# ndming/GS-2M

Hardware: AMD Instinct MI355X
Metric: train views/s (fwd+bwd raster) at 1M Gaussians 1080p (higher is better)
Workload: dtype f32; 1 GPU; BASELINE configs[2] (c3): 1000000 synthetic Gaussians (SH deg 3), 1 camera 1920x1080 per GPU, feature_count=9, fwd+bwd at the op boundary; gaussians=1000000, visible=844909, num_rendered=2709460, width=1920, height=1080, feature_count=9, parallelism=view-parallel x1, views_per_rank=1

## Files before the change

### gs-2m_amd/csrc/api.hip

```cpp
#include "common.h"
#include <atomic>
#include <mutex>
#include <chrono>
#include <dlfcn.h>

#define HIP_TRY(expr)                          \
    do {                                       \
        hipError_t e_ = (expr);                \
        if (e_ != hipSuccess) return GS2M_ERR_HIP; \
    } while (0)

namespace {

uint32_t higher_msb(uint32_t n) {
    uint32_t msb = sizeof(n) * 4;
    uint32_t step = msb;
    while (step > 1) {
        step /= 2;
        if (n >> msb) msb += step; else msb -= step;
    }
    if (n >> msb) msb++;
    return msb;
}

constexpr int kLandSlots = 64, kLandWords = 16;
struct LandRing {
    uint32_t* host = nullptr;
    uint32_t* dev = nullptr;
    std::atomic<uint32_t> next{0};
    std::atomic<uint32_t> gen[kLandSlots];
};
LandRing g_land[64];
std::mutex g_land_mutex;
thread_local uint64_t t_last_token = 0;
thread_local long long t_rows_hint = -1;
thread_local long long t_units_hint = -1, t_units_from_token = -1;

static_assert(GS2M_NUM_STAGES == 10, "stage table");
enum Stage { ST_PREPROCESS = 0, ST_UNUSED1, ST_SCAN, ST_EMIT, ST_TILE_SORT, ST_LISTS, ST_BLEND_FWD, ST_UNUSED7,
             ST_BLEND_BWD, ST_GAUSSIAN_BWD, ST_COUNT };
constexpr int kMaxRecords = 8192;
struct Prof {
    std::atomic<int> mode{0};
    int n = 0;
    hipEvent_t ev[kMaxRecords][2];
    int stage[kMaxRecords];
    int created = 0;
    int every = 1;
    int seen3 = 0;
};
Prof g_prof;
std::mutex g_prof_mutex;
std::atomic<int> g_reference_binning{0};
std::atomic<int> g_spin_wait{1};
std::atomic<int> g_debug{0};
std::atomic<int> g_markers{0};

const char* const kStageNames[ST_COUNT] = {"preprocess", "-", "scan", "emit", "tile_sort", "depth_order+quad_lists", "blend_fwd", "-", "blend_bwd", "gaussian_bwd"};

struct Roctx {
    int (*push)(const char*) = nullptr;
    int (*pop)() = nullptr;
    bool tried = false;
    void load() {
        if (tried) return;
        tried = true;
        void* h = dlopen("libroctx64.so", RTLD_NOW | RTLD_GLOBAL);
        if (!h) h = dlopen("libroctx64.so.4", RTLD_NOW | RTLD_GLOBAL);
        if (!h) return;
        push = (int (*)(const char*))dlsym(h, "roctxRangePushA");
        pop = (int (*)())dlsym(h, "roctxRangePop");
    }
};
Roctx g_roctx;

struct StageTimer {
    hipStream_t s;
    int slot = -1;
    int stage;
    int* failed;
    bool marked = false;
    StageTimer(int stage_, hipStream_t s_, int* failed_ = nullptr) : s(s_), stage(stage_), failed(failed_) {
        if (g_markers.load(std::memory_order_relaxed)) {
            g_roctx.load();
            if (g_roctx.push) { g_roctx.push(kStageNames[stage]); marked = true; }
        }
        const bool blend = stage == ST_BLEND_FWD || stage == ST_BLEND_BWD;
        if (g_prof.mode.load(std::memory_order_relaxed) == 0) return;
        {
            std::lock_guard<std::mutex> lock(g_prof_mutex);
            if (g_prof.mode == 0 || (g_prof.mode == 1 && !blend) || (g_prof.mode == 3 && stage != ST_BLEND_BWD) || g_prof.n >= kMaxRecords) return;
            if (g_prof.mode == 3 && (g_prof.seen3++ % g_prof.every) != 0) return;
            slot = g_prof.n++;
            if (slot >= g_prof.created) {
                (void)hipEventCreate(&g_prof.ev[slot][0]);
                (void)hipEventCreate(&g_prof.ev[slot][1]);
                g_prof.created = slot + 1;
            }
            g_prof.stage[slot] = stage;
        }
        (void)hipEventRecord(g_prof.ev[slot][0], s);
    }
    ~StageTimer() {
        if (slot >= 0) (void)hipEventRecord(g_prof.ev[slot][1], s);
        if (failed && g_debug.load(std::memory_order_relaxed) && *failed == 0) {
            hipError_t e = hipGetLastError();
            if (e == hipSuccess) e = hipStreamSynchronize(s);
            if (e != hipSuccess) *failed = stage + 1;
        }
        if (marked && g_roctx.pop) g_roctx.pop();
    }
};
#define DEBUG_CHECK()                                        \
    do {                                                     \
        if (failed_stage) return GS2M_ERR_STAGE(failed_stage - 1); \
    } while (0)

}

extern "C" {

char* gs2m_prealloc_alloc(size_t bytes, void* user) {
    gs2m_prealloc* p = static_cast<gs2m_prealloc*>(user);
    if (!p) return nullptr;
    p->requested = bytes;
    if (p->ptr && bytes <= p->capacity) return p->ptr;
    p->used_fallback = 1;
    return p->fallback ? p->fallback(bytes, p->fallback_user) : nullptr;
}

const char* gs2m_version(void) { return "gs2m_raster 0.5 (gfx950, round 5)"; }

static int forward_impl(gs2m_alloc_fn geometry_alloc, void* geometry_user, gs2m_alloc_fn binning_alloc,
                        void* binning_user, gs2m_alloc_fn image_alloc, void* image_user, int P, int D, int M,
                        const float* background, int width, int height, const float* means3D, const float* shs, const float* shs_rest,
                        const float* colors_precomp, const float* opacities, const float* scales, float scale_modifier,
                        const float* rotations, const float* cov3D_precomp, const float* features,
                        const float* viewmatrix, const float* projmatrix, const float* cam_pos, float tan_fovx,
                        float tan_fovy, int prefiltered, int feature_count, float* out_color, int* out_radii,
                        int* out_observe, float* out_buffer, void* stream_) {
    hipStream_t s = (hipStream_t)stream_;
    const int reference_binning = g_reference_binning.load(), spin_wait = g_spin_wait.load();
    int failed_stage = 0;
    if (P < 0 || width <= 0 || height <= 0 || feature_count < 0 || feature_count > GS2M_NUM_FEATURES) return GS2M_ERR_INVALID_ARG;
    if (!geometry_alloc || !binning_alloc || !image_alloc || !out_color || !out_buffer || !background) return GS2M_ERR_INVALID_ARG;
    if (P > 0 && (!means3D || !opacities || !out_radii || !out_observe || !viewmatrix || !projmatrix)) return GS2M_ERR_INVALID_ARG;
    if (P > 0 && ((shs == nullptr) == (colors_precomp == nullptr))) return GS2M_ERR_INVALID_ARG;
    if (P > 0 && (((scales == nullptr) || (rotations == nullptr)) == (cov3D_precomp == nullptr))) return GS2M_ERR_INVALID_ARG;
    if (P > 0 && shs && (D < 0 || D > 3 || M < (D + 1) * (D + 1) || !cam_pos)) return GS2M_ERR_INVALID_ARG;
    if (shs_rest && (!shs || M != 16 || (((uintptr_t)shs_rest) & 15))) return GS2M_ERR_UNSUPPORTED;
    if (P > 0 && feature_count > 0 && !features) return GS2M_ERR_INVALID_ARG;
    if (width > 16 * 65535 || height > 16 * 65535) return GS2M_ERR_UNSUPPORTED;
    if ((size_t)((width + GS2M_TILE - 1) / GS2M_TILE) * (size_t)((height + GS2M_TILE - 1) / GS2M_TILE) > ((size_t)1 << 28)) return GS2M_ERR_UNSUPPORTED;
    if (P >= (1 << GS2M_GID_BITS)) return GS2M_ERR_UNSUPPORTED;

    const int tiles_x = (width + GS2M_TILE - 1) / GS2M_TILE, tiles_y = (height + GS2M_TILE - 1) / GS2M_TILE;
    const size_t tiles = (size_t)tiles_x * tiles_y, N = (size_t)width * height;
    const float focal_y = height / (2.0f * tan_fovy);
    const float focal_x = width / (2.0f * tan_fovx);

    const size_t Pn = P > 0 ? (size_t)P : 1;
    GeomState gsz = gs2m_carve_geom(nullptr, Pn);
    char* gbase = geometry_alloc(gsz.total_bytes, geometry_user);
    if (!gbase) return GS2M_ERR_ALLOC;
    GeomState g = gs2m_carve_geom(gbase, Pn);

    ImageState isz = gs2m_carve_image(nullptr, N, tiles);
    char* ibase = image_alloc(isz.total_bytes, image_user);
    if (!ibase) return GS2M_ERR_ALLOC;
    ImageState im = gs2m_carve_image(ibase, N, tiles);

    int dev_id = 0;
    HIP_TRY(hipGetDevice(&dev_id));
    if (dev_id < 0 || dev_id >= 64) return GS2M_ERR_UNSUPPORTED;
    LandRing& ring = g_land[dev_id];
    if (!ring.host) {
        std::lock_guard<std::mutex> lock(g_land_mutex);
        if (!ring.host) {
            uint32_t* h = nullptr;
            HIP_TRY(hipHostMalloc((void**)&h, kLandSlots * kLandWords * sizeof(uint32_t), hipHostMallocMapped | hipHostMallocPortable));
            HIP_TRY(hipHostGetDevicePointer((void**)&ring.dev, h, 0));
            for (int k = 0; k < kLandSlots; k++) ring.gen[k] = 0;
            ring.host = h;
        }
    }
    const uint32_t seq = ring.next.fetch_add(1), slot = seq % kLandSlots;
    const uint32_t generation = ring.gen[slot].fetch_add(1) + 1;
    volatile uint32_t* land = ring.host + slot * kLandWords;
    uint32_t* land_dev = ring.dev + slot * kLandWords;
    land[GS2M_LAND_R] = 0xFFFFFFFFu;
    land[GS2M_LAND_HUNITS] = 0xFFFFFFFFu;
    land[GS2M_LAND_PREFILTERED] = 0u;
    land[GS2M_LAND_ROWS] = 0u;
    t_last_token = ((uint64_t)(dev_id + 1) << 40) | ((uint64_t)(generation & 0xFFFFFFFFu) << 8) | slot;

    int R = 0;
    uint32_t U = 0, crowded = GS2M_CROWDED_WAVE;
    if (P > 0) {
        {
            StageTimer t(ST_PREPROCESS, s, &failed_stage);
            ZeroJobs zj = {{g.tile_hist, nullptr, nullptr}, {(size_t)GS2M_HIST_COPIES * GS2M_HIST_COPY_WORDS, 0, 0}};
            gs2m_launch_preprocess(P, D, M, means3D, scales, scale_modifier, rotations, opacities, shs, shs_rest, cov3D_precomp,
                                   colors_precomp, features, viewmatrix, projmatrix, cam_pos, width, height, tan_fovx,
                                   tan_fovy, focal_x, focal_y, tiles_x, tiles_y, out_radii, out_observe, g,
                                   reference_binning ? 0 : 1, zj, s);
        }
        if (prefiltered) gs2m_launch_prefiltered_check(P, means3D, viewmatrix, land_dev + GS2M_LAND_PREFILTERED, s);
        {
            StageTimer t(ST_SCAN, s, &failed_stage);
            gs2m_launch_blockscan(P, g, land_dev, s);
        }
        HIP_TRY(hipGetLastError());
        DEBUG_CHECK();
        if (spin_wait) {
            const auto t0 = std::chrono::steady_clock::now();
            uint32_t spins = 0;
            while (land[GS2M_LAND_R] == 0xFFFFFFFFu || land[GS2M_LAND_HUNITS] == 0xFFFFFFFFu) {
                __builtin_ia32_pause();
                if ((++spins & 0xFFFFu) == 0u && std::chrono::steady_clock::now() - t0 > std::chrono::seconds(2)) break;
            }
        }
        if (land[GS2M_LAND_R] == 0xFFFFFFFFu || land[GS2M_LAND_HUNITS] == 0xFFFFFFFFu) HIP_TRY(hipStreamSynchronize(s));
        if (prefiltered && land[GS2M_LAND_PREFILTERED] != 0u) {
            HIP_TRY(hipStreamSynchronize(s));
            return GS2M_ERR_PREFILTERED;
        }
        if (land[GS2M_LAND_R] >= (1u << 29)) return GS2M_ERR_UNSUPPORTED;
        R = (int)land[GS2M_LAND_R];
        U = land[GS2M_LAND_HUNITS];
        if ((size_t)U * 4 * GS2M_UNIT > (size_t)6 * (size_t)R + 65536) {
            crowded = GS2M_CROWDED_OFF;
            land[GS2M_LAND_R] = 0xFFFFFFFFu;
            land[GS2M_LAND_HUNITS] = 0xFFFFFFFFu;
            gs2m_launch_recount_heavy(P, g, s);
            gs2m_launch_blockscan(P, g, land_dev, s);
            HIP_TRY(hipGetLastError());
            HIP_TRY(hipStreamSynchronize(s));
            if (land[GS2M_LAND_R] != (uint32_t)R) return GS2M_ERR_STAGE(ST_SCAN);
            U = land[GS2M_LAND_HUNITS];
        }
        if (U >= (1u << 22)) return GS2M_ERR_UNSUPPORTED;
    }

    const int tile_bits = (int)higher_msb((uint32_t)tiles);
    const size_t Rn = R > 0 ? (size_t)R : 1;
    const size_t btemp = gs2m_binning_temp_bytes(Rn, tile_bits);
    BinningState bsz = gs2m_carve_binning(nullptr, Rn, btemp, U);
    char* bbase = binning_alloc(bsz.total_bytes, binning_user);
    if (!bbase) return GS2M_ERR_ALLOC;
    BinningState b = gs2m_carve_binning(bbase, Rn, btemp, U);

    if (R > 0) {
        {
            StageTimer t(ST_EMIT, s, &failed_stage);
            ZeroJobs zj = {{nullptr, im.ranges_raw, nullptr}, {0, tiles * 2, 0}};
            gs2m_radix_zero_region(b.temp, (size_t)R, tile_bits, &zj.p[0], &zj.words[0]);
            gs2m_launch_emit(P, width, height, tiles_x, tile_bits, g, b, U, crowded, land_dev, zj, s);
        }
        if (g_debug.load(std::memory_order_relaxed)) {
            uint32_t total = 0;
            HIP_TRY(hipStreamSynchronize(s));
            HIP_TRY(hipMemcpy(&total, g.counters, sizeof(total), hipMemcpyDeviceToHost));
            if (total != (uint32_t)R) return GS2M_ERR_STAGE(ST_EMIT);
        }
        {
            StageTimer t(ST_TILE_SORT, s, &failed_stage);
            HIP_TRY(gs2m_radix_sort_pairs(b.temp, b.temp_bytes, b.keys_unsorted, nullptr, b.sort_keyA, b.sort_valA, b.tile_keys, b.slot_sorted,
                                          (size_t)R, tile_bits, true, s, im.ranges_raw, g.tile_hist));
        }
    } else {
        HIP_TRY(gs2m_zero_async(im.ranges_raw, tiles * 2 * sizeof(uint32_t), s));
        land[GS2M_LAND_ROWS] = 1u;
        if (land[GS2M_LAND_HUNITS] == 0xFFFFFFFFu) land[GS2M_LAND_HUNITS] = 0u;
    }
    DEBUG_CHECK();
    {
        StageTimer t(ST_LISTS, s, &failed_stage);
        gs2m_launch_tile_sort(tiles, tiles_x, tiles_y, (size_t)(R > 0 ? R : 0), b, im, g, s);
    }
    {
        StageTimer t(ST_BLEND_FWD, s, &failed_stage);
        gs2m_launch_blend_fwd_q(width, height, tiles_x, tiles_y, feature_count, background, g, b, im, out_color, out_buffer, out_observe, s);
    }
    DEBUG_CHECK();
    HIP_TRY(hipGetLastError());
    return R;
}

static int backward_impl(int P, int D, int M, int R, const float* background, int width, int height,
                         const float* means3D, const float* shs, const float* shs_rest, const float* colors_precomp, const float* scales,
                         float scale_modifier, const float* rotations, const float* cov3D_precomp,
                         const float* features, const float* viewmatrix, const float* projmatrix, const float* campos,
                         float tan_fovx, float tan_fovy, const int* radii, const float* buffer, char* geom_buffer,
                         char* binning_buffer, char* image_buffer, int feature_count, const float* grad_colors,
                         const float* grad_buffer, float* dL_dmeans2D, float* dL_dconics, float* dL_dopacities,
                         float* dL_dcolors, float* dL_dmeans3D, float* dL_dcov3D, float* dL_dshs, float* dL_dshs_rest, float* dL_dscales,
                         float* dL_drots, float* dL_dfeatures, gs2m_alloc_fn scratch_alloc, void* scratch_user,
                         void* stream_) {
    (void)buffer; (void)features;
    hipStream_t s = (hipStream_t)stream_;
    int failed_stage = 0;
    if (P == 0) return GS2M_OK;
    if (P >= (1 << GS2M_GID_BITS)) return GS2M_ERR_UNSUPPORTED;
    if (P < 0 || R < 0 || width <= 0 || height <= 0 || feature_count < 0 || feature_count > GS2M_NUM_FEATURES) return GS2M_ERR_INVALID_ARG;
    if (!geom_buffer || !binning_buffer || !image_buffer || !scratch_alloc || !grad_colors || !radii) return GS2M_ERR_INVALID_ARG;
    if (feature_count > 0 && !grad_buffer) return GS2M_ERR_INVALID_ARG;
    if (!dL_dmeans2D || !dL_dopacities || !dL_dmeans3D || !dL_dscales || !dL_drots || !dL_dfeatures) return GS2M_ERR_INVALID_ARG;
    if ((colors_precomp && !dL_dcolors) || (cov3D_precomp && !dL_dcov3D)) return GS2M_ERR_INVALID_ARG;
    if (shs_rest && (M != 16 || ((dL_dshs == nullptr) != (dL_dshs_rest == nullptr)) || ((((uintptr_t)shs_rest) | ((uintptr_t)dL_dshs_rest)) & 15))) return GS2M_ERR_UNSUPPORTED;

    const int tiles_x = (width + GS2M_TILE - 1) / GS2M_TILE, tiles_y = (height + GS2M_TILE - 1) / GS2M_TILE;
    const size_t tiles = (size_t)tiles_x * tiles_y, N = (size_t)width * height;
    const size_t Rn = R > 0 ? (size_t)R : 1;
    GeomState g = gs2m_carve_geom(geom_buffer, (size_t)P);
    BinningState b = gs2m_carve_binning(binning_buffer, Rn, gs2m_binning_temp_bytes(Rn, (int)higher_msb((uint32_t)tiles)), 0);
    ImageState im = gs2m_carve_image(image_buffer, N, tiles);

    const int rowf = gs2m_row_floats(feature_count);
    const long long hint = t_rows_hint;
    long long units = hint >= 0 ? t_units_hint : -1;
    t_rows_hint = -1;
    t_units_hint = -1;
    size_t nrows = 0;
    if (hint >= 0 && (size_t)hint <= Rn * 10 + 256) {
        nrows = (size_t)hint;
    } else if (R > 0) {
        uint32_t c[2] = {0u, 0u};
        HIP_TRY(hipStreamSynchronize(s));
        HIP_TRY(hipMemcpy(c, g.counters + GS2M_CNT_ROWS, sizeof(c), hipMemcpyDeviceToHost));
        nrows = c[0];
        units = c[1];
    }
    const size_t rows_bytes = gs2m_align_up((nrows > 0 ? nrows : 1) * (size_t)rowf * sizeof(float));
    char* sbase = scratch_alloc(rows_bytes + 2 * GS2M_ALIGN, scratch_user);
    if (!sbase) return GS2M_ERR_ALLOC;
    float* rows = (float*)gs2m_align_up((size_t)(uintptr_t)sbase);

    if (R > 0) {
        StageTimer t(ST_BLEND_BWD, s, &failed_stage);
        gs2m_launch_blend_bwd_q(width, height, tiles_x, tiles_y, feature_count, background, g, b, im, grad_colors,
                                grad_buffer, rows, s);
    }
    DEBUG_CHECK();
    {
        StageTimer tg(ST_GAUSSIAN_BWD, s, &failed_stage);
        if (R > 0) gs2m_launch_heavy_reduce(rows, rowf, b, g, units, s);
        gs2m_launch_gaussian_bwd(P, D, M, means3D, shs, shs_rest, colors_precomp, scales, scale_modifier, rotations, cov3D_precomp,
                                 viewmatrix, projmatrix, campos, width, height, tan_fovx, tan_fovy, radii, feature_count, g,
                                 rows, rowf, R > 0, dL_dmeans2D, dL_dconics, dL_dopacities, dL_dcolors, dL_dmeans3D,
                                 dL_dcov3D, dL_dshs, dL_dshs_rest, dL_dscales, dL_drots, dL_dfeatures, s);
    }
    DEBUG_CHECK();
    HIP_TRY(hipGetLastError());
    return GS2M_OK;
}

int gs2m_raster_forward(gs2m_alloc_fn geometry_alloc, void* geometry_user, gs2m_alloc_fn binning_alloc,
                        void* binning_user, gs2m_alloc_fn image_alloc, void* image_user, int P, int D, int M,
                        const float* background, int width, int height, const float* means3D, const float* shs,
                        const float* colors_precomp, const float* opacities, const float* scales, float scale_modifier,
                        const float* rotations, const float* cov3D_precomp, const float* features,
                        const float* viewmatrix, const float* projmatrix, const float* cam_pos, float tan_fovx,
                        float tan_fovy, int prefiltered, int feature_count, float* out_color, int* out_radii,
                        int* out_observe, float* out_buffer, void* stream_) {
    return forward_impl(geometry_alloc, geometry_user, binning_alloc, binning_user, image_alloc, image_user, P, D, M, background, width, height, means3D, shs, nullptr, colors_precomp, opacities, scales, scale_modifier, rotations, cov3D_precomp, features, viewmatrix, projmatrix, cam_pos, tan_fovx, tan_fovy, prefiltered, feature_count, out_color, out_radii, out_observe, out_buffer, stream_);
}

int gs2m_raster_forward_split_sh(gs2m_alloc_fn geometry_alloc, void* geometry_user, gs2m_alloc_fn binning_alloc,
                        void* binning_user, gs2m_alloc_fn image_alloc, void* image_user, int P, int D, int M,
                        const float* background, int width, int height, const float* means3D, const float* sh_dc, const float* sh_rest,
                        const float* colors_precomp, const float* opacities, const float* scales, float scale_modifier,
                        const float* rotations, const float* cov3D_precomp, const float* features,
                        const float* viewmatrix, const float* projmatrix, const float* cam_pos, float tan_fovx,
                        float tan_fovy, int prefiltered, int feature_count, float* out_color, int* out_radii,
                        int* out_observe, float* out_buffer, void* stream_) {
    if (!sh_dc || !sh_rest) return GS2M_ERR_INVALID_ARG;
    return forward_impl(geometry_alloc, geometry_user, binning_alloc, binning_user, image_alloc, image_user, P, D, M, background, width, height, means3D, sh_dc, sh_rest, colors_precomp, opacities, scales, scale_modifier, rotations, cov3D_precomp, features, viewmatrix, projmatrix, cam_pos, tan_fovx, tan_fovy, prefiltered, feature_count, out_color, out_radii, out_observe, out_buffer, stream_);
}

int gs2m_raster_backward(int P, int D, int M, int R, const float* background, int width, int height,
                         const float* means3D, const float* shs, const float* colors_precomp, const float* scales,
                         float scale_modifier, const float* rotations, const float* cov3D_precomp,
                         const float* features, const float* viewmatrix, const float* projmatrix, const float* campos,
                         float tan_fovx, float tan_fovy, const int* radii, const float* buffer, char* geom_buffer,
                         char* binning_buffer, char* image_buffer, int feature_count, const float* grad_colors,
                         const float* grad_buffer, float* dL_dmeans2D, float* dL_dconics, float* dL_dopacities,
                         float* dL_dcolors, float* dL_dmeans3D, float* dL_dcov3D, float* dL_dshs, float* dL_dscales,
                         float* dL_drots, float* dL_dfeatures, gs2m_alloc_fn scratch_alloc, void* scratch_user,
                         void* stream_) {
    return backward_impl(P, D, M, R, background, width, height, means3D, shs, nullptr, colors_precomp, scales, scale_modifier, rotations, cov3D_precomp, features, viewmatrix, projmatrix, campos, tan_fovx, tan_fovy, radii, buffer, geom_buffer, binning_buffer, image_buffer, feature_count, grad_colors, grad_buffer, dL_dmeans2D, dL_dconics, dL_dopacities, dL_dcolors, dL_dmeans3D, dL_dcov3D, dL_dshs, nullptr, dL_dscales, dL_drots, dL_dfeatures, scratch_alloc, scratch_user, stream_);
}

int gs2m_raster_backward_split_sh(int P, int D, int M, int R, const float* background, int width, int height,
                         const float* means3D, const float* sh_dc, const float* sh_rest, const float* colors_precomp, const float* scales,
                         float scale_modifier, const float* rotations, const float* cov3D_precomp,
                         const float* features, const float* viewmatrix, const float* projmatrix, const float* campos,
                         float tan_fovx, float tan_fovy, const int* radii, const float* buffer, char* geom_buffer,
                         char* binning_buffer, char* image_buffer, int feature_count, const float* grad_colors,
                         const float* grad_buffer, float* dL_dmeans2D, float* dL_dconics, float* dL_dopacities,
                         float* dL_dcolors, float* dL_dmeans3D, float* dL_dcov3D, float* dL_dsh_dc, float* dL_dsh_rest, float* dL_dscales,
                         float* dL_drots, float* dL_dfeatures, gs2m_alloc_fn scratch_alloc, void* scratch_user,
                         void* stream_) {
    if (!sh_dc || !sh_rest) return GS2M_ERR_INVALID_ARG;
    return backward_impl(P, D, M, R, background, width, height, means3D, sh_dc, sh_rest, colors_precomp, scales, scale_modifier, rotations, cov3D_precomp, features, viewmatrix, projmatrix, campos, tan_fovx, tan_fovy, radii, buffer, geom_buffer, binning_buffer, image_buffer, feature_count, grad_colors, grad_buffer, dL_dmeans2D, dL_dconics, dL_dopacities, dL_dcolors, dL_dmeans3D, dL_dcov3D, dL_dsh_dc, dL_dsh_rest, dL_dscales, dL_drots, dL_dfeatures, scratch_alloc, scratch_user, stream_);
}

int gs2m_raster_mark_visible(int P, const float* means3D, const float* viewmatrix, const float* projmatrix,
                             uint8_t* present, void* stream_) {
    (void)projmatrix;
    if (P < 0) return GS2M_ERR_INVALID_ARG;
    if (P == 0) return GS2M_OK;
    if (!means3D || !viewmatrix || !present) return GS2M_ERR_INVALID_ARG;
    gs2m_launch_mark_visible(P, means3D, viewmatrix, present, (hipStream_t)stream_);
    HIP_TRY(hipGetLastError());
    return GS2M_OK;
}

int gs2m_set_reference_binning(int on) {
    g_reference_binning = on ? 1 : 0;
    return GS2M_OK;
}

int gs2m_set_tile_sort_policy(int policy) {
    if (policy < 0 || policy > 3) return GS2M_ERR_INVALID_ARG;
    gs2m_set_tile_sort_policy_impl(policy);
    return GS2M_OK;
}

int gs2m_set_debug(int on) {
    g_debug = on ? 1 : 0;
    return GS2M_OK;
}

int gs2m_set_markers(int on) {
    g_markers = on ? 1 : 0;
    if (on) {
        g_roctx.load();
        if (!g_roctx.push || !g_roctx.pop) return GS2M_ERR_UNSUPPORTED;
    }
    return GS2M_OK;
}

const char* gs2m_stage_name(int stage) { return stage >= 0 && stage < ST_COUNT ? kStageNames[stage] : "?"; }

int gs2m_set_spin_wait(int on) {
    g_spin_wait = on ? 1 : 0;
    return GS2M_OK;
}

int gs2m_profile_mode(int mode) {
    if (mode < 0 || mode > 3) return GS2M_ERR_INVALID_ARG;
    std::lock_guard<std::mutex> lock(g_prof_mutex);
    g_prof.mode = mode;
    g_prof.n = 0;
    g_prof.seen3 = 0;
    return GS2M_OK;
}

int gs2m_profile_sampling(int every) {
    if (every < 1) return GS2M_ERR_INVALID_ARG;
    std::lock_guard<std::mutex> lock(g_prof_mutex);
    g_prof.every = every;
    return GS2M_OK;
}

int gs2m_profile_collect(float* stage_ms, int* stage_count, int n_stages) {
    if (!stage_ms || !stage_count || n_stages < GS2M_NUM_STAGES) return GS2M_ERR_INVALID_ARG;
    std::lock_guard<std::mutex> lock(g_prof_mutex);
    for (int i = 0; i < n_stages; i++) { stage_ms[i] = 0.f; stage_count[i] = 0; }
    for (int r = 0; r < g_prof.n; r++) {
        float ms = 0.f;
        HIP_TRY(hipEventSynchronize(g_prof.ev[r][1]));
        HIP_TRY(hipEventElapsedTime(&ms, g_prof.ev[r][0], g_prof.ev[r][1]));
        stage_ms[g_prof.stage[r]] += ms;
        stage_count[g_prof.stage[r]] += 1;
    }
    g_prof.n = 0;
    return GS2M_OK;
}

int gs2m_debug_layout(int P, int R, int width, int height, gs2m_layout* out) {
    if (!out || P < 0 || R < 0 || width <= 0 || height <= 0) return GS2M_ERR_INVALID_ARG;
    const int tiles_x = (width + GS2M_TILE - 1) / GS2M_TILE, tiles_y = (height + GS2M_TILE - 1) / GS2M_TILE;
    const size_t tiles = (size_t)tiles_x * tiles_y, N = (size_t)width * height;
    const size_t Pn = P > 0 ? (size_t)P : 1, Rn = R > 0 ? (size_t)R : 1;
    GeomState g = gs2m_carve_geom(nullptr, Pn);
    BinningState b = gs2m_carve_binning(nullptr, Rn, gs2m_binning_temp_bytes(Rn, (int)higher_msb((uint32_t)tiles)), 0);
    ImageState im = gs2m_carve_image(nullptr, N, tiles);
    out->geom_bytes = g.total_bytes;
    out->rec = (uint64_t)(uintptr_t)g.rec;
    out->tiles_touched = (uint64_t)(uintptr_t)g.tiles_touched;
    out->depth_key = (uint64_t)(uintptr_t)g.depth_key;
    out->rect = (uint64_t)(uintptr_t)g.rect;
    out->gauss_rows = (uint64_t)(uintptr_t)g.gauss_rows;
    out->clamped = (uint64_t)(uintptr_t)g.clamped;
    out->wave_rowbase = (uint64_t)(uintptr_t)g.wave_rowbase;
    out->counters = (uint64_t)(uintptr_t)g.counters;
    out->binning_bytes = b.total_bytes;
    out->point_list = (uint64_t)(uintptr_t)b.point_list;
    out->tile_keys = (uint64_t)(uintptr_t)b.tile_keys;
    out->qlist = (uint64_t)(uintptr_t)b.qlist;
    out->qrow = (uint64_t)(uintptr_t)b.qrow;
    out->image_bytes = im.total_bytes;
    out->final_T = (uint64_t)(uintptr_t)im.final_T;
    out->n_contrib = (uint64_t)(uintptr_t)im.n_contrib;
    out->ranges = (uint64_t)(uintptr_t)im.ranges;
    out->qcount = (uint64_t)(uintptr_t)im.qcount;
    return GS2M_OK;
}

unsigned long long gs2m_raster_forward_token(void) { return (unsigned long long)t_last_token; }

long long gs2m_raster_dense_rows(unsigned long long token) {
    if (token == 0ull) return -1;
    const int dev = (int)(token >> 40) - 1;
    const uint32_t slot = (uint32_t)(token & 0xFFull), generation = (uint32_t)((token >> 8) & 0xFFFFFFFFull);
    if (dev < 0 || dev >= 64 || slot >= (uint32_t)kLandSlots || !g_land[dev].host) return -1;
    LandRing& ring = g_land[dev];
    volatile uint32_t* land = ring.host + slot * kLandWords;
    const auto t0 = std::chrono::steady_clock::now();
    uint32_t spins = 0;
    for (;;) {
        if (ring.gen[slot].load() != generation) return -1;
        const uint32_t v = land[GS2M_LAND_ROWS];
        if (v != 0u) {
            t_units_from_token = (long long)land[GS2M_LAND_HUNITS];
            return ring.gen[slot].load() == generation ? (long long)v - 1 : -1;
        }
        __builtin_ia32_pause();
        if ((++spins & 0xFFFFu) == 0u && std::chrono::steady_clock::now() - t0 > std::chrono::seconds(2)) return -1;
    }
}

int gs2m_raster_backward_rows_hint(long long dense_rows) {
    t_rows_hint = dense_rows;
    t_units_hint = dense_rows >= 0 ? t_units_from_token : -1;
    t_units_from_token = -1;
    return GS2M_OK;
}

int gs2m_debug_tile_sort(int tiles, const unsigned* ranges_raw, unsigned* ranges, const unsigned* slot_sorted, const unsigned* e_rec,
                         const unsigned* wave_rowbase, unsigned* point_list, unsigned* row_tmp, unsigned* qlist,
                         unsigned* qrow, unsigned* qcount, void* stream_) {
    if (tiles < 0 || !ranges_raw || !ranges || !slot_sorted || !e_rec || !wave_rowbase || !point_list || !row_tmp || !qlist || !qrow || !qcount) return GS2M_ERR_INVALID_ARG;
    BinningState b = {};
    b.slot_sorted = const_cast<uint32_t*>(slot_sorted); b.e_rec = reinterpret_cast<uint4*>(const_cast<unsigned*>(e_rec));
    b.point_list = point_list; b.sort_valA = row_tmp; b.qlist = reinterpret_cast<uint2*>(qlist); b.qrow = qrow;
    ImageState im = {};
    im.ranges_raw = const_cast<uint32_t*>(ranges_raw);
    im.ranges = reinterpret_cast<uint2*>(ranges);
    im.qcount = qcount;
    GeomState g = {};
    g.wave_rowbase = const_cast<uint32_t*>(wave_rowbase);
    static uint32_t* dbg_counters[64] = {nullptr};
    int dev = 0;
    HIP_TRY(hipGetDevice(&dev));
    if (dev < 0 || dev >= 64) return GS2M_ERR_UNSUPPORTED;
    if (dbg_counters[dev] == nullptr) HIP_TRY(hipMalloc(&dbg_counters[dev], 64 * sizeof(uint32_t)));
    HIP_TRY(hipMemsetAsync(dbg_counters[dev], 0, 64 * sizeof(uint32_t), (hipStream_t)stream_));
    g.counters = dbg_counters[dev];
    gs2m_launch_tile_sort((size_t)tiles, tiles, 1, SIZE_MAX, b, im, g, (hipStream_t)stream_);
    HIP_TRY(hipGetLastError());
    return GS2M_OK;
}

}
```

### gs-2m_amd/csrc/binning.hip

```cpp
#include "common.h"

GeomState gs2m_carve_geom(char* base, size_t P) {
    GeomState g;
    size_t off = base ? (gs2m_align_up((size_t)(uintptr_t)base) - (size_t)(uintptr_t)base) : 0;
    auto take = [&](size_t bytes) {
        char* p = (char*)((uintptr_t)base + off);
        off = gs2m_align_up(off + bytes);
        return p;
    };
    const size_t nb = (P + 255) / 256 + 1, nw = (P + 63) / 64 + 1;
    g.rec = (float4*)take(P * REC_Q * sizeof(float4));
    g.tiles_touched = (uint32_t*)take(P * 4);
    g.rect = (uint2*)take(P * sizeof(uint2));
    g.depth_key = (uint32_t*)take(P * 4);
    g.clamped = (uint8_t*)take(P);
    g.sh_dir = (float*)take(P * 9 * sizeof(float));
    g.counters = (uint32_t*)take(64 * 4);
    g.gauss_rows = (uint32_t*)take(P * 4);
    g.block_tt = (uint32_t*)take(nb * 4);
    g.block_pref = (uint32_t*)take(nb * 4);
    g.block_hu = (uint32_t*)take(nb * 4);
    g.block_hupref = (uint32_t*)take(nb * 4);
    g.wave_rows = (uint32_t*)take(nw * 4);
    g.wave_rowbase = (uint32_t*)take(nw * 4);
    g.tile_hist = (uint32_t*)take(GS2M_HIST_COPIES * GS2M_HIST_COPY_WORDS * 4);
    g.total_bytes = off + GS2M_ALIGN;
    return g;
}

BinningState gs2m_carve_binning(char* base, size_t R, size_t temp_bytes, size_t heavy_units) {
    BinningState b;
    size_t off = base ? (gs2m_align_up((size_t)(uintptr_t)base) - (size_t)(uintptr_t)base) : 0;
    auto take = [&](size_t bytes) {
        char* p = (char*)((uintptr_t)base + off);
        off = gs2m_align_up(off + bytes);
        return p;
    };
    b.keys_unsorted = (uint32_t*)take(R * 4);
    b.e_rec = (uint4*)take(R * sizeof(uint4));
    b.sort_keyA = (uint32_t*)take(R * 4);
    b.sort_valA = (uint32_t*)take(R * 4);
    b.tile_keys = (uint32_t*)take(R * 4);
    b.slot_sorted = (uint32_t*)take(R * 4);
    b.point_list = (uint32_t*)take(R * 4);
    b.qlist = (uint2*)take(R * 4 * sizeof(uint2));
    b.qrow = (uint32_t*)take(R * 4 * 4);
    b.temp = take(temp_bytes);
    b.temp_bytes = temp_bytes;
    b.hrec = (HeavyUnit*)take(heavy_units * sizeof(HeavyUnit));
    b.total_bytes = off + GS2M_ALIGN;
    return b;
}

size_t gs2m_binning_temp_bytes(size_t R, int tile_bits) { return gs2m_align_up(gs2m_radix_temp_bytes(R, tile_bits)) + GS2M_ALIGN; }

ImageState gs2m_carve_image(char* base, size_t N, size_t tiles) {
    ImageState im;
    size_t off = base ? (gs2m_align_up((size_t)(uintptr_t)base) - (size_t)(uintptr_t)base) : 0;
    auto take = [&](size_t bytes) {
        char* p = (char*)((uintptr_t)base + off);
        off = gs2m_align_up(off + bytes);
        return p;
    };
    im.final_T = (float*)take(N * 4);
    im.n_contrib = (uint32_t*)take(N * 4);
    im.ranges = (uint2*)take(tiles * sizeof(uint2));
    im.ranges_raw = (uint32_t*)take(tiles * 2 * sizeof(uint32_t));
    im.qcount = (uint32_t*)take(tiles * 4 * sizeof(uint32_t));
    im.qlast = (uint32_t*)take(tiles * 4 * sizeof(uint32_t));
    im.total_bytes = off + GS2M_ALIGN;
    return im;
}

namespace {

__device__ __forceinline__ void publish(uint32_t* landing, int word, uint32_t v) {
    __hip_atomic_store(landing + word, v, __ATOMIC_RELAXED, __HIP_MEMORY_SCOPE_SYSTEM);
}

__device__ __forceinline__ unsigned long long block_sum_u64(unsigned long long v, unsigned long long* s_part ) {
    const int lane = threadIdx.x & 63, wave = threadIdx.x >> 6, nw = blockDim.x >> 6;
#pragma unroll
    for (int d = 32; d > 0; d >>= 1) v += __shfl_xor(v, d, 64);
    gs2m_sync();
    if (lane == 0) s_part[wave] = v;
    gs2m_sync();
    unsigned long long t = 0;
    for (int w = 0; w < nw; w++) t += s_part[w];
    return t;
}

template <typename F>
__device__ __forceinline__ unsigned long long scan_1024_per_block(const uint32_t* __restrict__ in, size_t n, uint32_t* s_w ,
                                                                  unsigned long long* s_part , F emit) {
    const size_t first = (size_t)blockIdx.x * 1024;
    unsigned long long before = 0;
    for (size_t base = 0; base < first; base += 16 * 1024) {
        uint32_t v[16];
#pragma unroll
        for (int k = 0; k < 16; k++) {
            const size_t i = base + (size_t)k * 1024 + threadIdx.x;
            v[k] = i < first ? in[i] : 0u;
        }
#pragma unroll
        for (int k = 0; k < 16; k++) before += v[k];
    }
    const size_t i = first + threadIdx.x;
    const uint32_t mine = i < n ? in[i] : 0u;
    before = block_sum_u64(before, s_part);
    const int lane = threadIdx.x & 63, wave = threadIdx.x >> 6;
    const uint32_t incl = wave_inclusive_scan_u32(mine, lane);
    if (lane == 63) s_w[wave] = incl;
    gs2m_sync();
    uint32_t run = incl - mine, total = 0;
    for (int w = 0; w < 16; w++) {
        if (w < wave) run += s_w[w];
        total += s_w[w];
    }
    if (i < n) emit(i, (uint32_t)before + run, mine);
    return before + total;
}

template <typename F>
__device__ __forceinline__ void scan2_1024_per_block(const uint32_t* __restrict__ in0, const uint32_t* __restrict__ in1, size_t n, uint32_t* s_w ,
                                                     unsigned long long* s_part , F emit, unsigned long long& total0, unsigned long long& total1) {
    const size_t first = (size_t)blockIdx.x * 1024;
    unsigned long long b0 = 0, b1 = 0;
    for (size_t base = 0; base < first; base += 8 * 1024) {
        uint32_t v[8], w[8];
#pragma unroll
        for (int k = 0; k < 8; k++) {
            const size_t i = base + (size_t)k * 1024 + threadIdx.x;
            v[k] = i < first ? in0[i] : 0u;
            w[k] = i < first ? in1[i] : 0u;
        }
#pragma unroll
        for (int k = 0; k < 8; k++) { b0 += v[k]; b1 += w[k]; }
    }
    const size_t i = first + threadIdx.x;
    const uint32_t m0 = i < n ? in0[i] : 0u, m1 = i < n ? in1[i] : 0u;
    const int lane = threadIdx.x & 63, wave = threadIdx.x >> 6;
#pragma unroll
    for (int d = 32; d > 0; d >>= 1) { b0 += __shfl_xor(b0, d, 64); b1 += __shfl_xor(b1, d, 64); }
    const uint32_t i0 = wave_inclusive_scan_u32(m0, lane), i1 = wave_inclusive_scan_u32(m1, lane);
    if (lane == 0) { s_part[wave] = b0; s_part[16 + wave] = b1; }
    if (lane == 63) { s_w[wave] = i0; s_w[16 + wave] = i1; }
    gs2m_sync();
    unsigned long long f0 = 0, f1 = 0;
    uint32_t r0 = i0 - m0, r1 = i1 - m1, t0 = 0, t1 = 0;
    for (int w = 0; w < 16; w++) {
        f0 += s_part[w]; f1 += s_part[16 + w];
        if (w < wave) { r0 += s_w[w]; r1 += s_w[16 + w]; }
        t0 += s_w[w]; t1 += s_w[16 + w];
    }
    if (i < n) emit(i, (uint32_t)f0 + r0, (uint32_t)f1 + r1);
    total0 = f0 + t0;
    total1 = f1 + t1;
}

__global__ void __launch_bounds__(1024) blockscan_kernel(const uint32_t* __restrict__ block_tt, const uint32_t* __restrict__ block_hu, size_t nblocks,
                                                         uint32_t* __restrict__ block_pref, uint32_t* __restrict__ block_hupref,
                                                         uint32_t* __restrict__ counters, uint32_t* landing) {
    __shared__ uint32_t s_w[32];
    __shared__ unsigned long long s_part[32];
    unsigned long long t = 0, u = 0;
    scan2_1024_per_block(block_tt, block_hu, nblocks, s_w, s_part, [&](size_t b, uint32_t e0, uint32_t e1) { block_pref[b] = e0; block_hupref[b] = e1; }, t, u);
    if (blockIdx.x == gridDim.x - 1 && threadIdx.x == 0) {
        const uint32_t r32 = t > 0xFFFFFFFEull ? 0xFFFFFFFEu : (uint32_t)t, u32 = u > 0xFFFFFFFEull ? 0xFFFFFFFEu : (uint32_t)u;
        __hip_atomic_store(reinterpret_cast<unsigned long long*>(landing + GS2M_LAND_R), (unsigned long long)r32 | ((unsigned long long)u32 << 32),
                           __ATOMIC_RELAXED, __HIP_MEMORY_SCOPE_SYSTEM);
        counters[1] = r32;
        counters[GS2M_CNT_HUNITS] = u32;
        counters[GS2M_CNT_SPAN_MID] = 0u;
        counters[GS2M_CNT_SPAN_LONG] = 0u;
    }
}

__global__ void __launch_bounds__(1024) rowscan_kernel(const uint32_t* __restrict__ wave_rows, size_t nwaves, uint32_t* __restrict__ wave_rowbase,
                                                       uint32_t* __restrict__ counters, uint32_t* landing) {
    __shared__ uint32_t s_w[16];
    __shared__ unsigned long long s_part[16];
    const uint32_t heavy_rows = 4u * GS2M_UNIT * counters[GS2M_CNT_HUNITS];
    const unsigned long long total = heavy_rows + scan_1024_per_block(wave_rows, nwaves, s_w, s_part, [&](size_t w, uint32_t excl, uint32_t) { wave_rowbase[w] = heavy_rows + excl; });
    if (blockIdx.x == gridDim.x - 1 && threadIdx.x == 0) {
        counters[GS2M_CNT_ROWS] = (uint32_t)total;
        publish(landing, GS2M_LAND_ROWS, (uint32_t)total + 1u);
    }
}


__device__ __forceinline__ uint2 expand_instance(uint32_t rmin, uint32_t rwid, uint32_t t, const float4 a , const float2 ct ,
                                                 int W, int H, int tiles_x) {
    const uint32_t ry = t / rwid, rx = t - ry * rwid;
    const uint32_t tx = (rmin & 0xFFFFu) + rx, ty = (rmin >> 16) + ry;
    const int px0 = (int)tx * GS2M_TILE, py0 = (int)ty * GS2M_TILE;
    uint32_t mask = gs2m_reaches_quads(a.x, a.y, a.z, a.w, ct.x, ct.y, (float)px0, (float)py0);
    if (px0 + 8 >= W) mask &= 0x5u;
    if (py0 + 8 >= H) mask &= 0x3u;
    return make_uint2(ty * (uint32_t)tiles_x + tx, mask);
}

__global__ void __launch_bounds__(256) emit_kernel(int P, int W, int H, int tiles_x, const uint2* __restrict__ rect,
                                                   const uint32_t* __restrict__ block_pref, const uint32_t* __restrict__ block_hupref,
                                                   const float4* __restrict__ rec,
                                                   const uint32_t* __restrict__ depth_key, uint32_t* __restrict__ keys_out, uint4* __restrict__ e_rec,
                                                   HeavyUnit* __restrict__ hrec,
                                                   uint32_t* __restrict__ gauss_rows, uint32_t* __restrict__ wave_rows,
                                                   uint32_t* __restrict__ counters, uint32_t* __restrict__ tile_hist, int npass, int4 hbits,
                                                   int4 hshift, uint32_t crowded, ZeroJobs zero) {
    __shared__ uint32_t s_th[4][256];
    __shared__ uint32_t s_pref[4][GS2M_WAVE];
    __shared__ uint32_t s_rmin[4][GS2M_WAVE];
    __shared__ uint32_t s_rw[4][GS2M_WAVE];
    __shared__ uint32_t s_off[4][GS2M_WAVE];
    __shared__ uint32_t s_depth[4][GS2M_WAVE];
    __shared__ float4 s_geo[4][GS2M_WAVE];
    __shared__ float2 s_ct[4][GS2M_WAVE];
    __shared__ uint32_t s_rc[4][GS2M_WAVE];
    __shared__ uint32_t s_wtot[4], s_whu[4];
    const int i = blockIdx.x * 256 + threadIdx.x;
    const int wave = threadIdx.x >> 6, lane = threadIdx.x & 63;
    gs2m_zero_jobs(zero, (size_t)i, (size_t)gridDim.x * 256);
#pragma unroll
    for (int p = 0; p < 4; p++) s_th[p][threadIdx.x] = 0u;
    const int hb[4] = {hbits.x, hbits.y, hbits.z, hbits.w}, hs[4] = {hshift.x, hshift.y, hshift.z, hshift.w};
    uint32_t cnt = 0, rmin = 0, rw = 1;
    if (i < P) {
        const uint2 r = rect[i];
        rmin = r.x;
        rw = r.y & 0xFFFFu;
        cnt = rw * (r.y >> 16);
        if (rw == 0u) rw = 1u;
    }
    const bool heavy = gs2m_heavy(cnt, crowded);
    const uint32_t hu = heavy ? (cnt + GS2M_UNIT - 1u) / GS2M_UNIT : 0u;
    const uint32_t incl_all = wave_inclusive_scan_u32(cnt, lane), incl_hu = wave_inclusive_scan_u32(hu, lane);
    if (lane == 63) { s_wtot[wave] = incl_all; s_whu[wave] = incl_hu; }
    const uint32_t lcnt = heavy ? 0u : cnt;
    if (lcnt > 0) {
        const float4* r = rec + (size_t)i * REC_Q;
        s_geo[wave][lane] = r[REC_GEO0];
        s_ct[wave][lane] = make_float2(r[REC_GEO1].x, r[REC_BIN].w);
        s_depth[wave][lane] = depth_key[i];
    }
    const uint32_t incl = wave_inclusive_scan_u32(lcnt, lane);
    const uint32_t total = __shfl(incl, 63, 64);
    s_pref[wave][lane] = incl - lcnt;
    s_rmin[wave][lane] = rmin;
    s_rw[wave][lane] = rw;
    s_rc[wave][lane] = 0u;
    gs2m_sync();
    uint32_t off = block_pref[blockIdx.x], ustart = block_hupref[blockIdx.x];
#pragma unroll
    for (int w = 0; w < 4; w++)
        if (w < wave) { off += s_wtot[w]; ustart += s_whu[w]; }
    off += incl_all - cnt;
    ustart += incl_hu - hu;
    s_off[wave][lane] = off;
    if (blockIdx.x == gridDim.x - 1 && threadIdx.x == 255) counters[0] = off + cnt;
    if (heavy) {
        gauss_rows[i] = GS2M_ROWS_BIG | ustart;
        for (uint32_t j = 0; j < hu; j++) {
            hrec[ustart + j].gid = (uint32_t)i;
            hrec[ustart + j].off = off;
        }
    }
    const uint32_t gid0 = (uint32_t)blockIdx.x * 256u;
    uint32_t rows_run = 0;
    for (uint32_t k = 0; k < total; k += GS2M_WAVE) {
        const uint32_t j = k + lane;
        uint32_t pc = 0, slot = 0, mask = 0;
        int lo = 0;
        if (j < total) {
#pragma unroll
            for (int step = 32; step > 0; step >>= 1)
                if (s_pref[wave][lo + step] <= j) lo += step;
            const uint32_t t = j - s_pref[wave][lo];
            slot = s_off[wave][lo] + t;
            const uint2 km = expand_instance(s_rmin[wave][lo], s_rw[wave][lo], t, s_geo[wave][lo], s_ct[wave][lo], W, H, tiles_x);
            mask = km.y;
            keys_out[slot] = km.x;
            for (int p = 0; p < npass; p++) atomicAdd(&s_th[p][(km.x >> hs[p]) & ((1u << hb[p]) - 1u)], 1u);
            pc = (uint32_t)__popc(mask);
            if (pc) atomicAdd(&s_rc[wave][lo], pc);
        }
        const uint32_t pin = wave_inclusive_scan_u32(pc, lane);
        if (j < total) e_rec[slot] = make_uint4((gid0 + (uint32_t)(wave * GS2M_WAVE + lo)) | (mask << GS2M_GID_BITS), rows_run + pin - pc, s_depth[wave][lo], 0u);
        rows_run += __shfl(pin, 63, 64);
    }
    if (i < P && !heavy) gauss_rows[i] = s_rc[wave][lane];
    const size_t wave_id = (size_t)blockIdx.x * 4 + wave;
    if (lane == 0 && (size_t)wave_id * GS2M_WAVE < (size_t)P) wave_rows[wave_id] = rows_run;
    gs2m_sync();
    uint32_t* dst = tile_hist + (blockIdx.x & (GS2M_HIST_COPIES - 1)) * GS2M_HIST_COPY_WORDS;
    for (int p = 0; p < npass; p++) {
        const uint32_t c = s_th[p][threadIdx.x];
        if (c) atomicAdd(&dst[p * 256 + threadIdx.x], c);
    }
}

__global__ void __launch_bounds__(256) recount_heavy_kernel(int P, const uint2* __restrict__ rect, uint32_t* __restrict__ block_hu) {
    __shared__ uint32_t s_hu[4];
    const int i = blockIdx.x * 256 + threadIdx.x;
    uint32_t cnt = 0;
    if (i < P) {
        const uint2 r = rect[i];
        cnt = (r.y & 0xFFFFu) * (r.y >> 16);
    }
    uint32_t hu = gs2m_heavy(cnt, GS2M_CROWDED_OFF) ? (cnt + GS2M_UNIT - 1u) / GS2M_UNIT : 0u;
#pragma unroll
    for (int d = 32; d > 0; d >>= 1) hu += (uint32_t)__shfl_xor((int)hu, d, 64);
    if ((threadIdx.x & 63) == 0) s_hu[threadIdx.x >> 6] = hu;
    gs2m_sync();
    if (threadIdx.x == 0) block_hu[blockIdx.x] = s_hu[0] + s_hu[1] + s_hu[2] + s_hu[3];
}

__global__ void __launch_bounds__(256) emit_heavy_kernel(uint32_t units, int W, int H, int tiles_x, const uint2* __restrict__ rect, const float4* __restrict__ rec,
                                                         const uint32_t* __restrict__ depth_key, const uint32_t* __restrict__ gauss_rows,
                                                         uint32_t* __restrict__ keys_out, uint4* __restrict__ e_rec, HeavyUnit* __restrict__ hrec,
                                                         uint32_t* __restrict__ tile_hist, int npass, int4 hbits, int4 hshift) {
    __shared__ uint32_t s_th[4][256];
#pragma unroll
    for (int p = 0; p < 4; p++) s_th[p][threadIdx.x] = 0u;
    gs2m_sync();
    const int hb[4] = {hbits.x, hbits.y, hbits.z, hbits.w}, hs[4] = {hshift.x, hshift.y, hshift.z, hshift.w};
    const int wave = threadIdx.x >> 6, lane = threadIdx.x & 63;
    const uint32_t u = blockIdx.x * 4u + (uint32_t)wave;
    if (u < units) {
        const uint32_t gid = hrec[u].gid, off = hrec[u].off;
        const uint32_t ustart = gauss_rows[gid] & ~GS2M_ROWS_BIG;
        const uint2 r = rect[gid];
        const uint32_t rw = r.y & 0xFFFFu, cnt = rw * (r.y >> 16);
        const float4* rq = rec + (size_t)gid * REC_Q;
        const float4 geo = rq[REC_GEO0];
        const float2 ct = make_float2(rq[REC_GEO1].x, rq[REC_BIN].w);
        const uint32_t dk = depth_key[gid];
        const uint32_t t = (u - ustart) * GS2M_UNIT + (uint32_t)lane;
        uint32_t pc = 0;
        if (t < cnt) {
            const uint2 km = expand_instance(r.x, rw, t, geo, ct, W, H, tiles_x);
            keys_out[off + t] = km.x;
            for (int p = 0; p < npass; p++) atomicAdd(&s_th[p][(km.x >> hs[p]) & ((1u << hb[p]) - 1u)], 1u);
            e_rec[off + t] = make_uint4(gid | (km.y << GS2M_GID_BITS), GS2M_ROWS_BIG | (4u * (u * GS2M_UNIT + (uint32_t)lane)), dk, 0u);
            pc = (uint32_t)__popc(km.y);
        }
        hrec[u].pop[lane] = (uint8_t)pc;
    }
    gs2m_sync();
    uint32_t* dst = tile_hist + (blockIdx.x & (GS2M_HIST_COPIES - 1)) * GS2M_HIST_COPY_WORDS;
    for (int p = 0; p < npass; p++) {
        const uint32_t c = s_th[p][threadIdx.x];
        if (c) atomicAdd(&dst[p * 256 + threadIdx.x], c);
    }
}

}

void gs2m_launch_blockscan(int P, const GeomState& g, uint32_t* landing, hipStream_t s) {
    const size_t nb = (size_t)(P + 255) / 256;
    blockscan_kernel<<<(unsigned)((nb + 1023) / 1024 > 0 ? (nb + 1023) / 1024 : 1), 1024, 0, s>>>(g.block_tt, g.block_hu, nb, g.block_pref, g.block_hupref, g.counters,
                                                                                                  landing);
}

void gs2m_launch_recount_heavy(int P, const GeomState& g, hipStream_t s) {
    recount_heavy_kernel<<<(P + 255) / 256, 256, 0, s>>>(P, g.rect, g.block_hu);
}

void gs2m_launch_emit(int P, int W, int H, int tiles_x, int tile_bits, const GeomState& g, const BinningState& b, uint32_t heavy_units, uint32_t crowded,
                      uint32_t* landing, const ZeroJobs& zero, hipStream_t s) {
    int npass = 0, bits[4], shift[4];
    gs2m_radix_plan(tile_bits, &npass, bits, shift);
    const int4 hbits = make_int4(bits[0], bits[1], bits[2], bits[3]), hshift = make_int4(shift[0], shift[1], shift[2], shift[3]);
    emit_kernel<<<(P + 255) / 256, 256, 0, s>>>(P, W, H, tiles_x, g.rect, g.block_pref, g.block_hupref, g.rec, g.depth_key, b.keys_unsorted, b.e_rec, b.hrec,
                                                g.gauss_rows, g.wave_rows, g.counters, g.tile_hist, npass, hbits, hshift, crowded, zero);
    if (heavy_units > 0u)
        emit_heavy_kernel<<<(heavy_units + 3u) / 4u, 256, 0, s>>>(heavy_units, W, H, tiles_x, g.rect, g.rec, g.depth_key, g.gauss_rows, b.keys_unsorted, b.e_rec,
                                                                  b.hrec, g.tile_hist, npass, hbits, hshift);
    const size_t nw = (size_t)(P + 63) / 64;
    rowscan_kernel<<<(unsigned)((nw + 1023) / 1024 > 0 ? (nw + 1023) / 1024 : 1), 1024, 0, s>>>(g.wave_rows, nw, g.wave_rowbase, g.counters, landing);
}

__global__ void zero_kernel(uint32_t* __restrict__ p, size_t words) {
    const size_t i = (size_t)blockIdx.x * blockDim.x + threadIdx.x;
    const size_t head = (4 - (((uintptr_t)p >> 2) & 3)) & 3;
    const size_t quads = words > head ? (words - head) >> 2 : 0;
    if (i < quads) reinterpret_cast<uint4*>(p + head)[i] = make_uint4(0u, 0u, 0u, 0u);
    if (i < head && i < words) p[i] = 0u;
    const size_t tail = head + 4 * quads;
    if (i < words - min(words, tail)) p[tail + i] = 0u;
}
hipError_t gs2m_zero_async(void* p, size_t bytes, hipStream_t s) {
    if (bytes == 0) return hipSuccess;
    if ((bytes & 3) || ((uintptr_t)p & 3)) return hipMemsetAsync(p, 0, bytes, s);
    const size_t words = bytes >> 2, threads = (words >> 2) + 4;
    zero_kernel<<<(unsigned)((threads + 255) / 256), 256, 0, s>>>((uint32_t*)p, words);
    return hipGetLastError();
}
```

### gs-2m_amd/csrc/common.h

```cpp
#pragma once
#include <hip/hip_runtime.h>
#include <stdint.h>
#include <stddef.h>
#include "../../include/gs2m_raster.h"

typedef float gs2m_v4f __attribute__((ext_vector_type(4)));
template <typename T> __device__ __forceinline__ T gs2m_ldnt(const T* p) { return __builtin_nontemporal_load(p); }
__device__ __forceinline__ float4 gs2m_ldnt(const float4* p) {
    const gs2m_v4f t = __builtin_nontemporal_load(reinterpret_cast<const gs2m_v4f*>(p));
    return make_float4(t.x, t.y, t.z, t.w);
}
template <typename T> __device__ __forceinline__ void gs2m_stnt(T* p, T v) { __builtin_nontemporal_store(v, p); }
__device__ __forceinline__ void gs2m_stnt(float4* p, float4 v) {
    const gs2m_v4f t = {v.x, v.y, v.z, v.w};
    __builtin_nontemporal_store(t, reinterpret_cast<gs2m_v4f*>(p));
}

#define GS2M_ALIGN 256
#define GS2M_WAVE 64

#define REC_Q 8
#define REC_GEO0 0
#define REC_GEO1 1
#define REC_BIN 2
#define REC_CH 3
#define REC_AUX 7
#define GS2M_GID_BITS 28
#define GS2M_GID_MASK 0x0FFFFFFFu
#define GS2M_HEAVY_TILES 40u
#define GS2M_HEAVY_TILES_CROWDED 8u
#define GS2M_CROWDED_WAVE 320u
#define GS2M_ROWS_BIG 0x80000000u
#define GS2M_UNIT 64u
struct HeavyUnit {
    uint32_t gid;
    uint32_t off;
    uint32_t pad[2];
    uint8_t pop[GS2M_UNIT];
};

#define ROW_GEOM 8
#define ROW_COL 8
#define ROW_FEAT 11

static inline size_t gs2m_align_up(size_t x, size_t a = GS2M_ALIGN) { return (x + a - 1) & ~(a - 1); }
static inline int gs2m_status(hipError_t e) { return e == hipSuccess ? GS2M_OK : GS2M_ERR_HIP; }

struct GeomState {
    float4* rec;
    uint32_t* tiles_touched;
    uint2* rect;
    uint32_t* depth_key;
    uint8_t* clamped;
    float* sh_dir;
    uint32_t* counters;
    uint32_t* gauss_rows;
    uint32_t* block_tt;
    uint32_t* block_pref;
    uint32_t* block_hu;
    uint32_t* block_hupref;
    uint32_t* wave_rows;
    uint32_t* wave_rowbase;
    uint32_t* tile_hist;
    size_t total_bytes;
};
struct BinningState {
    uint32_t* keys_unsorted;
    uint4* e_rec;
    uint32_t* sort_keyA;
    uint32_t* sort_valA;
    uint32_t* tile_keys;
    uint32_t* slot_sorted;
    uint32_t* point_list;
    uint2* qlist;
    uint32_t* qrow;
    char* temp;
    size_t temp_bytes;
    HeavyUnit* hrec;
    size_t total_bytes;
};
struct ImageState {
    float* final_T;
    uint32_t* n_contrib;
    uint2* ranges;
    uint32_t* ranges_raw;
    uint32_t* qcount;
    uint32_t* qlast;
    size_t total_bytes;
};

struct ZeroJobs {
    uint32_t* p[3];
    size_t words[3];
};
#ifdef __HIPCC__
__device__ __forceinline__ void gs2m_zero_jobs(const ZeroJobs& z, size_t thread, size_t threads) {
#pragma unroll
    for (int k = 0; k < 3; k++)
        for (size_t i = thread; i < z.words[k]; i += threads) z.p[k][i] = 0u;
}
#endif

#ifdef __HIPCC__
__device__ __forceinline__ void gs2m_stage_sh(const float* __restrict__ shs, const float* __restrict__ rest, int P,
                                              float* __restrict__ s_sh) {
    const int tid = threadIdx.x;
    if (rest == nullptr) {
        const size_t base4 = (size_t)blockIdx.x * 256 * 12, lim4 = (size_t)P * 12;
        const float4* g4 = reinterpret_cast<const float4*>(shs);
        float4 t[12];
#pragma unroll
        for (int i = 0; i < 12; i++) {
            const size_t k = base4 + tid + 256 * i;
            t[i] = k < lim4 ? gs2m_ldnt(g4 + k) : make_float4(0.f, 0.f, 0.f, 0.f);
        }
#pragma unroll
        for (int i = 0; i < 12; i++) {
            const int e = 4 * (tid + 256 * i);
            const int row = e / 48, col = e - row * 48;
            float* d = s_sh + row * 49 + col;
            d[0] = t[i].x; d[1] = t[i].y; d[2] = t[i].z; d[3] = t[i].w;
        }
    } else {
        const size_t dbase = (size_t)blockIdx.x * 768, dlim = (size_t)P * 3;
#pragma unroll
        for (int i = 0; i < 3; i++) {
            const int e = tid + 256 * i;
            const float v = dbase + e < dlim ? shs[dbase + e] : 0.f;
            s_sh[(e / 3) * 49 + (e % 3)] = v;
        }
        const size_t rbase = (size_t)blockIdx.x * 11520, rlim = (size_t)P * 45;
        const bool full = rbase + 11520 <= rlim;
        float4 t[12];
        if (full) {
            const float4* g4 = reinterpret_cast<const float4*>(rest + rbase);
#pragma unroll
            for (int i = 0; i < 11; i++) t[i] = gs2m_ldnt(g4 + tid + 256 * i);
            t[11] = tid < 64 ? gs2m_ldnt(g4 + tid + 2816) : make_float4(0.f, 0.f, 0.f, 0.f);
        } else {
#pragma unroll
            for (int i = 0; i < 12; i++) {
                const int k4 = tid + 256 * i;
                const size_t ge = rbase + 4 * (size_t)k4;
                t[i] = make_float4(0.f, 0.f, 0.f, 0.f);
                if (k4 < 2880) {
                    if (ge + 3 < rlim) {
                        t[i] = *reinterpret_cast<const float4*>(rest + ge);
                    } else {
                        if (ge < rlim) t[i].x = rest[ge];
                        if (ge + 1 < rlim) t[i].y = rest[ge + 1];
                        if (ge + 2 < rlim) t[i].z = rest[ge + 2];
                    }
                }
            }
        }
        int row = (4 * tid) / 45, col = 4 * tid - 45 * row;
#pragma unroll
        for (int i = 0; i < 12; i++) {
            if (i < 11 || tid < 64) {
                const float v[4] = {t[i].x, t[i].y, t[i].z, t[i].w};
                int a = row * 49 + 3 + col, left = 45 - col;
#pragma unroll
                for (int c = 0; c < 4; c++) s_sh[a + c + (c >= left ? 4 : 0)] = v[c];
            }
            row += 22; col += 34;
            if (col >= 45) { col -= 45; row += 1; }
        }
    }
}
#endif

GeomState gs2m_carve_geom(char* base, size_t P);
BinningState gs2m_carve_binning(char* base, size_t R, size_t temp_bytes, size_t heavy_units);
size_t gs2m_binning_temp_bytes(size_t R, int tile_bits);
ImageState gs2m_carve_image(char* base, size_t N, size_t tiles);

size_t gs2m_radix_temp_bytes(size_t n, int total_bits);
hipError_t gs2m_radix_sort_pairs(void* temp, size_t temp_bytes, const uint32_t* kin, const uint32_t* vin, uint32_t* kA,
                                 uint32_t* vA, uint32_t* kB, uint32_t* vB, size_t n, int total_bits, bool prezeroed, hipStream_t s,
                                 uint32_t* range_raw = nullptr, const uint32_t* ext_hist = nullptr);
#define GS2M_HIST_COPIES 8
#define GS2M_HIST_COPY_WORDS 1024
void gs2m_radix_plan(int total_bits, int* npass, int bits[4], int shift[4]);
void gs2m_radix_zero_region(void* temp, size_t n, int total_bits, uint32_t** ptr, size_t* words);

#define GS2M_LAND_R 0
#define GS2M_LAND_HUNITS 1
#define GS2M_LAND_PREFILTERED 2
#define GS2M_LAND_ROWS 3
#define GS2M_CNT_ROWS 2
#define GS2M_CNT_HUNITS 3
#define GS2M_CNT_SPAN_MID 4
#define GS2M_CNT_SPAN_LONG 5

void gs2m_launch_preprocess(int P, int D, int M, const float* means3D, const float* scales, float scale_modifier,
                            const float* rotations, const float* opacities, const float* shs, const float* shs_rest,
                            const float* cov3D_precomp, const float* colors_precomp, const float* features,
                            const float* viewmatrix, const float* projmatrix, const float* cam_pos, int W, int H,
                            float tan_fovx, float tan_fovy, float focal_x, float focal_y, int tiles_x, int tiles_y,
                            int* radii, int* observe_zero, const GeomState& g, int shrink, const ZeroJobs& zero, hipStream_t s);
void gs2m_launch_blockscan(int P, const GeomState& g, uint32_t* landing, hipStream_t s);
void gs2m_launch_emit(int P, int W, int H, int tiles_x, int tile_bits, const GeomState& g, const BinningState& b, uint32_t heavy_units,
                      uint32_t crowded, uint32_t* landing, const ZeroJobs& zero, hipStream_t s);
void gs2m_launch_recount_heavy(int P, const GeomState& g, hipStream_t s);
void gs2m_launch_heavy_reduce(float* rows, int rowf, const BinningState& b, const GeomState& g, long long heavy_units, hipStream_t s);
void gs2m_set_tile_sort_policy_impl(int policy);
void gs2m_launch_tile_sort(size_t tiles, int tiles_x, int tiles_y, size_t R, const BinningState& b, const ImageState& im, const GeomState& g, hipStream_t s);
hipError_t gs2m_zero_async(void* p, size_t bytes, hipStream_t s);

void gs2m_launch_blend_fwd_q(int W, int H, int tiles_x, int tiles_y, int fc, const float* bg, const GeomState& g,
                             const BinningState& b, const ImageState& im, float* out_color, float* out_buffer,
                             int* out_observe, hipStream_t s);
void gs2m_launch_blend_bwd_q(int W, int H, int tiles_x, int tiles_y, int fc, const float* bg, const GeomState& g,
                             const BinningState& b, const ImageState& im, const float* grad_color,
                             const float* grad_buffer, float* rows, hipStream_t s);
int gs2m_row_floats(int fc);
void gs2m_launch_gaussian_bwd(int P, int D, int M, const float* means3D, const float* shs, const float* shs_rest,
                              const float* colors_precomp,
                              const float* scales, float scale_modifier, const float* rotations,
                              const float* cov3D_precomp, const float* viewmatrix, const float* projmatrix,
                              const float* campos, int W, int H, float tan_fovx, float tan_fovy, const int* radii,
                              int fc, const GeomState& g, const float* rows, int rowf, bool have_rows,
                              float* dL_dmeans2D, float* dL_dconics, float* dL_dopacities, float* dL_dcolors,
                              float* dL_dmeans3D, float* dL_dcov3D, float* dL_dshs, float* dL_dshs_rest, float* dL_dscales,
                              float* dL_drots, float* dL_dfeatures, hipStream_t s);
void gs2m_launch_prefiltered_check(int P, const float* means3D, const float* viewmatrix, uint32_t* flag, hipStream_t s);
void gs2m_launch_mark_visible(int P, const float* means3D, const float* viewmatrix, uint8_t* present, hipStream_t s);

#ifdef __HIPCC__
__device__ __forceinline__ float u2f(uint32_t u) { return __uint_as_float(u); }
__device__ __forceinline__ uint32_t f2u(float f) { return __float_as_uint(f); }

#define DPP_QUAD_PERM(a, b, c, d) ((a) | ((b) << 2) | ((c) << 4) | ((d) << 6))
#define DPP_ROW_HALF_MIRROR 0x141
#define DPP_ROW_MIRROR 0x140

__device__ __forceinline__ void gs2m_sync() {
    asm volatile("s_waitcnt lgkmcnt(0)" ::: "memory");
    __syncthreads();
}
__device__ __forceinline__ int gs2m_sync_or(bool pred) {
    asm volatile("s_waitcnt lgkmcnt(0)" ::: "memory");
    return __syncthreads_or(pred);
}

#define GS2M_CROWDED_OFF 0xFFFFFFFFu
__device__ __forceinline__ bool gs2m_heavy(uint32_t cnt, uint32_t crowded) {
    uint32_t light = cnt < GS2M_HEAVY_TILES ? cnt : 0u;
#pragma unroll
    for (int d = 32; d > 0; d >>= 1) light += (uint32_t)__shfl_xor((int)light, d, 64);
    return cnt >= (light > crowded ? GS2M_HEAVY_TILES_CROWDED : GS2M_HEAVY_TILES) && cnt < (1u << 29);
}

template <typename T>
__device__ __forceinline__ T gs2m_wave_inclusive_scan(T v, int lane) {
#pragma unroll
    for (int d = 1; d < 64; d <<= 1) {
        const T t = __shfl_up(v, d, 64);
        if (lane >= d) v += t;
    }
    return v;
}
__device__ __forceinline__ uint32_t wave_inclusive_scan_u32(uint32_t v, int lane) { return gs2m_wave_inclusive_scan(v, lane); }

template <typename T>
__device__ __forceinline__ T gs2m_wg_exclusive_scan(T v, T* s_w, T* total) {
    const int lane = threadIdx.x & 63, w = threadIdx.x >> 6;
    const T inc = gs2m_wave_inclusive_scan(v, lane);
    if (lane == 63) s_w[w] = inc;
    __syncthreads();
    T off = 0, tot = 0;
#pragma unroll
    for (int k = 0; k < 4; k++) {
        const T x = s_w[k];
        off += k < w ? x : T(0);
        tot += x;
    }
    __syncthreads();
    *total = tot;
    return off + inc - v;
}

#define GS2M_LOG2E 1.4426950408889634f
__device__ __forceinline__ float gs2m_power(float dx, float dy, float A, float B, float C) {
    const float t1 = (A * dx) * dx;
    const float t2 = (C * dy) * dy;
    const float t3 = (B * dx) * dy;
    return (-0.5f * (t1 + t2)) - t3;
}
__device__ __forceinline__ uint32_t gs2m_reaches_quads(float gx, float gy, float A, float B, float C, float t2, float x0, float y0) {
    const float b2 = B + B;
    const float nhrC = -0.5f * __builtin_amdgcn_rcpf(C), nhrA = -0.5f * __builtin_amdgcn_rcpf(A);
    float xl[4], yl[4], blx[4], bly[4], basex[4], basey[4], mx[4], my[4];
#pragma unroll
    for (int i = 0; i < 4; i++) {
        const float o = (float)((i >> 1) * 8 + (i & 1) * 7);
        xl[i] = (x0 + o) - gx; yl[i] = (y0 + o) - gy;
        blx[i] = b2 * xl[i]; bly[i] = b2 * yl[i];
        basex[i] = (A * xl[i]) * xl[i]; basey[i] = (C * yl[i]) * yl[i];
        mx[i] = blx[i] * nhrC;
        my[i] = bly[i] * nhrA;
    }
    uint32_t mask = 0;
#pragma unroll
    for (int q = 0; q < 4; q++) {
        const int qx = q & 1, qy = q >> 1;
        const float lx = xl[2 * qx], ux = xl[2 * qx + 1], ly = yl[2 * qy], uy = yl[2 * qy + 1];
        const bool inside = lx <= 0.f && ux >= 0.f && ly <= 0.f && uy >= 0.f;
        float qe[2];
#pragma unroll
        for (int e = 0; e < 2; e++) {
            const int i = 2 * qx + e;
            const float fm = __builtin_amdgcn_fmed3f(mx[i], ly, uy);
            qe[e] = __builtin_fmaf(__builtin_fmaf(C, fm, blx[i]), fm, basex[i]);
        }
        const float qv = fminf(qe[0], qe[1]);
#pragma unroll
        for (int e = 0; e < 2; e++) {
            const int k = 2 * qy + e;
            const float fm = __builtin_amdgcn_fmed3f(my[k], lx, ux);
            qe[e] = __builtin_fmaf(__builtin_fmaf(A, fm, bly[k]), fm, basey[k]);
        }
        const float qmin = fminf(qv, fminf(qe[0], qe[1]));
        const bool hit = !(t2 < 3.0e38f) || inside || qmin <= __builtin_fmaf(1.0e-3f, fabsf(qmin), t2);
        mask |= hit ? (1u << q) : 0u;
    }
    return mask;
}

__device__ __forceinline__ float gs2m_exp(float x) { return __builtin_amdgcn_exp2f(x * GS2M_LOG2E); }
#endif
```

### gs-2m_amd/csrc/radix_sort.hip

```cpp
#include "common.h"
#include <stdlib.h>
#include <atomic>

static std::atomic<int> g_sort_tickets{0};
extern "C" int gs2m_set_sort_tickets(int on) {
    g_sort_tickets = on ? 1 : 0;
    return GS2M_OK;
}

namespace {
constexpr int RS_LB2_WIN = 16;
constexpr int RS_THREADS = 256;
constexpr int RS_ITEMS = 16;
constexpr int RS_TILE = RS_THREADS * RS_ITEMS;
constexpr int RS_MAXPASS = 4;
int resident_tiles() {
    static int cached[64] = {0};
    int dev = 0;
    if (hipGetDevice(&dev) != hipSuccess || dev < 0 || dev >= 64) return 0;
    if (cached[dev] == 0) {
        int cus = 0;
        cached[dev] = hipDeviceGetAttribute(&cus, hipDeviceAttributeMultiprocessorCount, dev) == hipSuccess && cus > 0 ? 4 * cus : -1;
    }
    return cached[dev] > 0 ? cached[dev] : 0;
}
constexpr uint32_t FLAG_AGG = 1u << 30, FLAG_PFX = 2u << 30, VAL_MASK = (1u << 30) - 1;

struct SortPlan {
    int npass;
    int bits[RS_MAXPASS];
    int shift[RS_MAXPASS];
};

SortPlan make_plan(int total_bits) {
    SortPlan p;
    if (total_bits < 1) total_bits = 1;
    p.npass = total_bits <= 16 ? 2 : 4;
    const int per = (total_bits + p.npass - 1) / p.npass;
    int s = 0;
    for (int i = 0; i < p.npass; i++) {
        int b = total_bits - s;
        if (b > per) b = per;
        if (b < 0) b = 0;
        p.bits[i] = b;
        p.shift[i] = s;
        s += b;
    }
    return p;
}

constexpr int RS_HIST_WGS = 512;
constexpr int RS_HIST_REP = 16;
__global__ void __launch_bounds__(RS_THREADS) rs_hist_kernel(const uint32_t* __restrict__ keys, uint32_t n, int npass,
                                                             int4 bits, int4 shift, uint32_t* __restrict__ ghist, int tiles,
                                                             int workers) {
    __shared__ uint32_t s_h[RS_MAXPASS][256][RS_HIST_REP];
    const int tid = threadIdx.x, lane = tid & 63;
    for (int i = tid; i < RS_MAXPASS * 256 * RS_HIST_REP; i += RS_THREADS) (&s_h[0][0][0])[i] = 0;
    gs2m_sync();
    const int b[4] = {bits.x, bits.y, bits.z, bits.w}, sh[4] = {shift.x, shift.y, shift.z, shift.w};
    const int rep = lane & (RS_HIST_REP - 1);
    for (int tile = blockIdx.x; tile < tiles; tile += workers) {
        const uint32_t base = (uint32_t)tile * RS_TILE;
        uint32_t key[RS_ITEMS];
#pragma unroll
        for (int k = 0; k < RS_ITEMS; k++) {
            const uint32_t i = base + k * RS_THREADS + tid;
            key[k] = i < n ? keys[i] : 0u;
        }
#pragma unroll
        for (int k = 0; k < RS_ITEMS; k++) {
            const uint32_t i = base + k * RS_THREADS + tid;
            if (i < n)
                for (int p = 0; p < npass; p++) atomicAdd(&s_h[p][(key[k] >> sh[p]) & ((1u << b[p]) - 1u)][rep], 1u);
        }
    }
    gs2m_sync();
    for (int p = 0; p < npass; p++) {
        const uint4* r4 = reinterpret_cast<const uint4*>(&s_h[p][tid][0]);
        uint32_t c = 0;
#pragma unroll
        for (int q = 0; q < RS_HIST_REP / 4; q++) {
            const uint4 v = r4[q];
            c += v.x + v.y + v.z + v.w;
        }
        if (c) atomicAdd(&ghist[p * 256 + tid], c);
    }
}

template <int BITS>
__global__ void __launch_bounds__(RS_THREADS) rs_onesweep_kernel(
    const uint32_t* __restrict__ keys_in, const uint32_t* __restrict__ vals_in, uint32_t* __restrict__ keys_out,
    uint32_t* __restrict__ vals_out, uint32_t n, int shift, const uint32_t* __restrict__ ghist, uint32_t* ticket,
    uint32_t* status , uint32_t* range_raw, int hist_copies ) {
    constexpr int BINS = 1 << BITS;
    __shared__ uint32_t s_cnt[4][BINS];
    __shared__ uint32_t s_gbase[256];
    __shared__ uint32_t s_w[2][4];
    __shared__ uint32_t s_tile;
    __shared__ uint32_t s_key[RS_TILE], s_val[RS_TILE];
    const int tid = threadIdx.x, wave = tid >> 6, lane = tid & 63;
    if (tid == 0) s_tile = ticket != nullptr ? atomicAdd(ticket, 1u) : blockIdx.x;
    for (int i = tid; i < 4 * BINS; i += RS_THREADS) (&s_cnt[0][0])[i] = 0;
    gs2m_sync();
    const uint32_t tile = s_tile;
    const uint32_t tile_base = tile * RS_TILE;
    const uint32_t tile_count = min((uint32_t)RS_TILE, n - tile_base);
    const uint32_t segbase = tile_base + wave * (64 * RS_ITEMS);

    uint32_t key[RS_ITEMS], val[RS_ITEMS], rank[RS_ITEMS];
#pragma unroll
    for (int k = 0; k < RS_ITEMS; k++) {
        const uint32_t i = segbase + k * 64 + lane;
        key[k] = i < n ? keys_in[i] : 0xFFFFFFFFu;
        val[k] = i < n ? (vals_in ? vals_in[i] : i) : 0u;
    }
    const unsigned long long lt = (1ull << lane) - 1ull;
#pragma unroll
    for (int k = 0; k < RS_ITEMS; k++) {
        const bool valid = segbase + k * 64 + lane < n;
        const uint32_t d = (key[k] >> shift) & (BINS - 1);
        unsigned long long peers = __builtin_amdgcn_ballot_w64(valid);
#pragma unroll
        for (int b = 0; b < BITS; b++) {
            const bool bit = (d >> b) & 1u;
            const unsigned long long bal = __builtin_amdgcn_ballot_w64(bit);
            peers &= bit ? bal : ~bal;
        }
        const uint32_t old = s_cnt[wave][d];
        const unsigned long long below = peers & lt;
        rank[k] = old + (uint32_t)__popcll(below);
        if (valid && below == 0ull) s_cnt[wave][d] = old + (uint32_t)__popcll(peers);
    }
    gs2m_sync();

    uint32_t tot = 0, c0 = 0, c1 = 0, c2 = 0, gh = 0;
    if (tid < BINS) {
        c0 = s_cnt[0][tid]; c1 = s_cnt[1][tid]; c2 = s_cnt[2][tid];
        tot = c0 + c1 + c2 + s_cnt[3][tid];
        for (int c = 0; c < hist_copies; c++) gh += ghist[c * GS2M_HIST_COPY_WORDS + tid];
    }
    const uint32_t inclA = wave_inclusive_scan_u32(tot, lane), inclB = wave_inclusive_scan_u32(gh, lane);
    if (lane == 63) {
        s_w[0][wave] = inclA;
        s_w[1][wave] = inclB;
    }
    gs2m_sync();
    uint32_t tile_excl = inclA - tot, digit_base = inclB - gh;
#pragma unroll
    for (int w = 0; w < 4; w++)
        if (w < wave) {
            tile_excl += s_w[0][w];
            digit_base += s_w[1][w];
        }
    if (tid < BINS) {
        __hip_atomic_store(status + (size_t)tile * 256 + tid, FLAG_AGG | tot, __ATOMIC_RELAXED, __HIP_MEMORY_SCOPE_AGENT);
        s_cnt[0][tid] = tile_excl;
        s_cnt[1][tid] = tile_excl + c0;
        s_cnt[2][tid] = tile_excl + c0 + c1;
        s_cnt[3][tid] = tile_excl + c0 + c1 + c2;
    }
    gs2m_sync();
#pragma unroll
    for (int k = 0; k < RS_ITEMS; k++) {
        if (segbase + k * 64 + lane < n) {
            const uint32_t d = (key[k] >> shift) & (BINS - 1);
            const uint32_t lp = s_cnt[wave][d] + rank[k];
            s_key[lp] = key[k];
            s_val[lp] = val[k];
        }
    }
    if (tid < BINS) {
        const uint32_t grp = tile >> 5, r = tile & 31u;
        uint32_t* const lvl2 = status + (size_t)gridDim.x * 256;
        const bool leader = r == 31u;
        uint32_t insum = 0;
#pragma unroll
        for (int h = 0; h < 2; h++) {
            uint32_t w[16];
#pragma unroll
            for (int k = 0; k < 16; k++) {
                const uint32_t back = (uint32_t)(16 * h + k) + 1u;
                w[k] = back <= r ? __hip_atomic_load(status + (size_t)(tile - back) * 256 + tid, __ATOMIC_RELAXED, __HIP_MEMORY_SCOPE_AGENT) : FLAG_AGG;
            }
#pragma unroll
            for (int k = 0; k < 16; k++) {
                const uint32_t back = (uint32_t)(16 * h + k) + 1u;
                while ((w[k] & ~VAL_MASK) == 0u) {
                    __builtin_amdgcn_s_sleep(1);
                    w[k] = __hip_atomic_load(status + (size_t)(tile - back) * 256 + tid, __ATOMIC_RELAXED, __HIP_MEMORY_SCOPE_AGENT);
                }
                insum += w[k] & VAL_MASK;
            }
        }
        uint32_t* const my2 = lvl2 + (size_t)grp * 256 + tid;
        const uint32_t gagg = insum + tot;
        if (leader) __hip_atomic_store(my2, (grp == 0 ? FLAG_PFX : FLAG_AGG) | gagg, __ATOMIC_RELAXED, __HIP_MEMORY_SCOPE_AGENT);
        uint32_t excl2 = 0;
        {
            int p = (int)grp - 1;
            bool found = p < 0;
            while (!found) {
                uint32_t w[RS_LB2_WIN];
#pragma unroll
                for (int k = 0; k < RS_LB2_WIN; k++)
                    w[k] = p - k >= 0 ? __hip_atomic_load(lvl2 + (size_t)(p - k) * 256 + tid, __ATOMIC_RELAXED, __HIP_MEMORY_SCOPE_AGENT)
                                      : FLAG_PFX;
                bool stalled = false;
#pragma unroll
                for (int k = 0; k < RS_LB2_WIN; k++) {
                    const uint32_t f = w[k] & ~VAL_MASK;
                    if (!found && !stalled) {
                        if (f == 0u) {
                            stalled = true;
                        } else {
                            excl2 += w[k] & VAL_MASK;
                            p--;
                            found = f == FLAG_PFX;
                        }
                    }
                }
                if (stalled) __builtin_amdgcn_s_sleep(1);
            }
        }
        if (leader && grp > 0) __hip_atomic_store(my2, FLAG_PFX | (excl2 + gagg), __ATOMIC_RELAXED, __HIP_MEMORY_SCOPE_AGENT);
        const uint32_t excl = excl2 + insum;
        s_gbase[tid] = digit_base + excl - tile_excl;
    }
    gs2m_sync();
#pragma unroll
    for (int k = 0; k < RS_ITEMS; k++) {
        const uint32_t i = k * RS_THREADS + tid;
        if (i < tile_count) {
            const uint32_t kk = s_key[i];
            const uint32_t pos = s_gbase[(kk >> shift) & (BINS - 1)] + i;
            keys_out[pos] = kk;
            vals_out[pos] = s_val[i];
            if (range_raw != nullptr) {
                if (i == 0 || s_key[i - 1] != kk) atomicMax(&range_raw[2 * kk], ~pos);
                if (i + 1 == tile_count || s_key[i + 1] != kk) atomicMax(&range_raw[2 * kk + 1], pos + 1u);
            }
        }
    }
}

template <int BITS>
void launch_pass(const uint32_t* ki, const uint32_t* vi, uint32_t* ko, uint32_t* vo, uint32_t n, int shift,
                 const uint32_t* ghist, uint32_t* ticket, uint32_t* status, int tiles, hipStream_t s, uint32_t* range_raw, int hist_copies) {
    static const bool env_tickets = getenv("GS2M_SORT_TICKETS") && atoi(getenv("GS2M_SORT_TICKETS")) != 0;
    const bool force_tickets = env_tickets || g_sort_tickets.load(std::memory_order_relaxed) != 0;
    rs_onesweep_kernel<BITS><<<tiles, RS_THREADS, 0, s>>>(ki, vi, ko, vo, n, shift, ghist,
                                                          (!force_tickets && tiles <= resident_tiles()) ? nullptr : ticket, status, range_raw, hist_copies);
}

}

void gs2m_radix_plan(int total_bits, int* npass, int bits[4], int shift[4]) {
    const SortPlan p = make_plan(total_bits);
    *npass = p.npass;
    for (int i = 0; i < RS_MAXPASS; i++) { bits[i] = i < p.npass ? p.bits[i] : 0; shift[i] = i < p.npass ? p.shift[i] : 0; }
}

static size_t status_rows(size_t tiles) { return tiles + (tiles + 31) / 32; }
size_t gs2m_radix_temp_bytes(size_t n, int total_bits) {
    const SortPlan p = make_plan(total_bits);
    const size_t tiles = (n + RS_TILE - 1) / RS_TILE;
    return gs2m_align_up(RS_MAXPASS * 256 * 4) + GS2M_ALIGN + (size_t)p.npass * status_rows(tiles) * 256 * 4 + 2 * GS2M_ALIGN;
}

void gs2m_radix_zero_region(void* temp, size_t n, int total_bits, uint32_t** ptr, size_t* words) {
    const SortPlan p = make_plan(total_bits);
    const size_t tiles = (n + RS_TILE - 1) / RS_TILE;
    *ptr = (uint32_t*)gs2m_align_up((size_t)(uintptr_t)temp);
    *words = (gs2m_align_up(RS_MAXPASS * 256 * 4) + GS2M_ALIGN + (size_t)p.npass * status_rows(tiles) * 256 * 4) / 4;
}

hipError_t gs2m_radix_sort_pairs(void* temp, size_t temp_bytes, const uint32_t* kin, const uint32_t* vin, uint32_t* kA,
                                 uint32_t* vA, uint32_t* kB, uint32_t* vB, size_t n, int total_bits, bool prezeroed, hipStream_t s,
                                 uint32_t* range_raw, const uint32_t* ext_hist) {
    if (n == 0) return hipSuccess;
    const SortPlan p = make_plan(total_bits);
    const int tiles = (int)((n + RS_TILE - 1) / RS_TILE);
    if (temp_bytes < gs2m_radix_temp_bytes(n, total_bits)) return hipErrorInvalidValue;
    char* base = (char*)gs2m_align_up((size_t)(uintptr_t)temp);
    uint32_t* ghist = (uint32_t*)base;
    uint32_t* tickets = (uint32_t*)(base + gs2m_align_up(RS_MAXPASS * 256 * 4));
    uint32_t* status = (uint32_t*)(base + gs2m_align_up(RS_MAXPASS * 256 * 4) + GS2M_ALIGN);
    const size_t zero_bytes = gs2m_align_up(RS_MAXPASS * 256 * 4) + GS2M_ALIGN + (size_t)p.npass * status_rows((size_t)tiles) * 256 * 4;
    hipError_t e = prezeroed ? hipSuccess : gs2m_zero_async(base, zero_bytes, s);
    if (e != hipSuccess) return e;
    const int workers = tiles < RS_HIST_WGS ? tiles : RS_HIST_WGS;
    if (ext_hist == nullptr)
        rs_hist_kernel<<<workers, RS_THREADS, 0, s>>>(kin, (uint32_t)n, p.npass, make_int4(p.bits[0], p.bits[1], p.bits[2], p.bits[3]),
                                                      make_int4(p.shift[0], p.shift[1], p.shift[2], p.shift[3]), ghist, tiles, workers);
    const uint32_t *ki = kin, *vi = vin;
    for (int i = 0; i < p.npass; i++) {
        uint32_t* ko = (i & 1) ? kB : kA;
        uint32_t* vo = (i & 1) ? vB : vA;
        uint32_t* st = status + (size_t)i * status_rows((size_t)tiles) * 256;
        const uint32_t* gh = (ext_hist ? ext_hist : ghist) + i * 256;
        const int hc = ext_hist ? GS2M_HIST_COPIES : 1;
        uint32_t* const rr = i == p.npass - 1 ? range_raw : nullptr;
        switch (p.bits[i]) {
#define RS_CASE(B) case B: launch_pass<B>(ki, vi, ko, vo, (uint32_t)n, p.shift[i], gh, tickets + i, st, tiles, s, rr, hc); break;
            RS_CASE(1) RS_CASE(2) RS_CASE(3) RS_CASE(4) RS_CASE(5) RS_CASE(6) RS_CASE(7) RS_CASE(8)
#undef RS_CASE
            default: launch_pass<1>(ki, vi, ko, vo, (uint32_t)n, 31, gh, tickets + i, st, tiles, s, rr, hc); break;
        }
        ki = ko;
        vi = vo;
    }
    return hipGetLastError();
}
```

### gs-2m_amd/csrc/tile_sort.hip

```cpp
#include "common.h"
#include <atomic>
#include <cstdlib>
#include <type_traits>

namespace {

template <int CTRL, int ROW_MASK = 0xF, int BANK_MASK = 0xF>
__device__ __forceinline__ uint32_t dpp_u32(uint32_t old, uint32_t v) {
    return (uint32_t)__builtin_amdgcn_update_dpp((int)old, (int)v, CTRL, ROW_MASK, BANK_MASK, false);
}
template <int CTRL>
__device__ __forceinline__ uint32_t dpp_perm(uint32_t v) {
    return (uint32_t)__builtin_amdgcn_update_dpp(0, (int)v, CTRL, 0xF, 0xF, true);
}
template <int B>
__device__ __forceinline__ uint32_t lane_xor(uint32_t v, int lane) {
    if constexpr (B == 0) return dpp_perm<DPP_QUAD_PERM(1, 0, 3, 2)>(v);
    else if constexpr (B == 1) return dpp_perm<DPP_QUAD_PERM(2, 3, 0, 1)>(v);
    else if constexpr (B == 2) {
        const uint32_t t = dpp_u32<0x104 , 0xF, 0x5>(v, v);
        return dpp_u32<0x114 , 0xF, 0xA>(t, v);
    } else if constexpr (B == 3) return dpp_perm<0x128 >(v);
    else return (uint32_t)__builtin_amdgcn_ds_bpermute((lane ^ (1 << B)) << 2, (int)v);
}
template <int T>
__device__ __forceinline__ uint32_t lane_flip(uint32_t v, int lane) {
    if constexpr (T == 1) return dpp_perm<DPP_QUAD_PERM(1, 0, 3, 2)>(v);
    else if constexpr (T == 2) return dpp_perm<DPP_QUAD_PERM(3, 2, 1, 0)>(v);
    else if constexpr (T == 3) return dpp_perm<DPP_ROW_HALF_MIRROR>(v);
    else if constexpr (T == 4) return dpp_perm<DPP_ROW_MIRROR>(v);
    else return (uint32_t)__builtin_amdgcn_ds_bpermute((lane ^ ((1 << T) - 1)) << 2, (int)v);
}

template <int I, int N, typename F>
__device__ __forceinline__ void static_for(F&& f) {
    if constexpr (I < N) {
        f(std::integral_constant<int, I>{});
        static_for<I + 1, N>(f);
    }
}
template <int E, int a, int b>
__device__ __forceinline__ void ce(uint32_t (&k)[E], uint32_t (&x)[E]) {
    const bool sw = k[b] < k[a];
    const uint32_t mn = min(k[a], k[b]), mx = max(k[a], k[b]);
    const uint32_t xa = sw ? x[b] : x[a], xb = sw ? x[a] : x[b];
    k[a] = mn; k[b] = mx; x[a] = xa; x[b] = xb;
}
template <int E, int KB>
__device__ __forceinline__ void inlane_flip(uint32_t (&k)[E], uint32_t (&x)[E]) {
    static_for<0, E>([&](auto ec) {
        constexpr int e = decltype(ec)::value;
        if constexpr (((e >> (KB - 1)) & 1) == 0) ce<E, e, (e ^ ((1 << KB) - 1))>(k, x);
    });
}
template <int E, int JB>
__device__ __forceinline__ void inlane_xor(uint32_t (&k)[E], uint32_t (&x)[E]) {
    static_for<0, E>([&](auto ec) {
        constexpr int e = decltype(ec)::value;
        if constexpr (((e >> JB) & 1) == 0) ce<E, e, (e | (1 << JB))>(k, x);
    });
}
template <int E, int T>
__device__ __forceinline__ void cross_flip(uint32_t (&k)[E], uint32_t (&x)[E], int lane) {
    const bool lower = ((lane >> (T - 1)) & 1) == 0;
    uint32_t nk[E], nx[E];
#pragma unroll
    for (int e = 0; e < E; e++) {
        const uint32_t ok = lane_flip<T>(k[E - 1 - e], lane), ox = lane_flip<T>(x[E - 1 - e], lane);
        const uint32_t mn = min(k[e], ok), mx = max(k[e], ok);
        nk[e] = lower ? mn : mx;
        nx[e] = nk[e] == k[e] ? x[e] : ox;
    }
#pragma unroll
    for (int e = 0; e < E; e++) { k[e] = nk[e]; x[e] = nx[e]; }
}
template <int E, int B>
__device__ __forceinline__ void cross_xor(uint32_t (&k)[E], uint32_t (&x)[E], int lane) {
    const bool lower = ((lane >> B) & 1) == 0;
#pragma unroll
    for (int e = 0; e < E; e++) {
        const uint32_t ok = lane_xor<B>(k[e], lane), ox = lane_xor<B>(x[e], lane);
        const uint32_t mn = min(k[e], ok), mx = max(k[e], ok);
        const uint32_t nk = lower ? mn : mx;
        x[e] = nk == k[e] ? x[e] : ox;
        k[e] = nk;
    }
}
template <int E, int LE, int JB>
__device__ __forceinline__ void xor_steps(uint32_t (&k)[E], uint32_t (&x)[E], int lane) {
    if constexpr (JB >= 0) {
        if constexpr (JB >= LE) cross_xor<E, JB - LE>(k, x, lane);
        else inlane_xor<E, JB>(k, x);
        xor_steps<E, LE, JB - 1>(k, x, lane);
    }
}
template <int E, int LE, int KB>
__device__ __forceinline__ void levels(uint32_t (&k)[E], uint32_t (&x)[E], int lane, uint32_t n) {
    if constexpr (KB <= LE + 6) {
        if (n > (1u << (KB - 1))) {
            if constexpr (KB <= LE) inlane_flip<E, KB>(k, x);
            else cross_flip<E, KB - LE>(k, x, lane);
            xor_steps<E, LE, KB - 2>(k, x, lane);
        }
        levels<E, LE, KB + 1>(k, x, lane, n);
    }
}

__device__ __forceinline__ int skew(int p) { return p + (p >> 5); }

template <int E>
__device__ __forceinline__ void tie_positions(const uint32_t (&key)[E], const uint32_t (&idx)[E], uint32_t (&pos)[E], const int t, const uint32_t n,
                                              const uint32_t* s_k, const uint32_t* s_i) {
#pragma unroll
    for (int e = 0; e < E; e++) {
        const uint32_t i = (uint32_t)(t * E + e);
        pos[e] = i;
        if (i >= n) continue;
        const uint32_t K = key[e], X = idx[e];
        uint32_t a = i, cnt = 0;
        for (uint32_t j = i; j > 0u;) {
            j--;
            if (s_k[skew((int)j)] != K) break;
            a = j;
            cnt += s_i[skew((int)j)] < X ? 1u : 0u;
        }
        for (uint32_t j = i + 1u; j < n; j++) {
            if (s_k[skew((int)j)] != K) break;
            cnt += s_i[skew((int)j)] < X ? 1u : 0u;
        }
        pos[e] = a + cnt;
    }
}

template <int E, int LE>
__device__ __forceinline__ void sort_tile_wave(const int tile, const uint32_t start, const uint32_t n, const uint32_t* __restrict__ slot_sorted,
                                               const uint4* __restrict__ e_rec, const uint32_t* __restrict__ wave_rowbase,
                                               uint32_t* __restrict__ point_list, uint2* __restrict__ qlist, uint32_t* __restrict__ qrow,
                                               uint32_t* __restrict__ qcount, uint32_t* s_v, uint32_t* s_r, const int lane) {
    uint32_t key[E], idx[E], rb[E];
    static_for<0, E / 8>([&](auto bc) {
        constexpr int e0 = 8 * decltype(bc)::value;
        uint32_t slot[8];
#pragma unroll
        for (int e = 0; e < 8; e++) {
            const uint32_t p = (uint32_t)((e0 + e) * GS2M_WAVE + lane);
            slot[e] = p < n ? slot_sorted[start + p] : 0u;
        }
        uint4 rc[8];
#pragma unroll
        for (int e = 0; e < 8; e++) rc[e] = (uint32_t)((e0 + e) * GS2M_WAVE + lane) < n ? e_rec[slot[e]] : make_uint4(0u, 0u, 0xFFFFFFFFu, 0u);
        static_for<0, 8>([&](auto ec) {
            constexpr int e = decltype(ec)::value;
            const uint32_t p = (uint32_t)((e0 + e) * GS2M_WAVE + lane);
            key[e0 + e] = rc[e].z;
            idx[e0 + e] = p;
            s_v[skew((int)p)] = rc[e].x;
            s_r[skew((int)p)] = rc[e].y & ~GS2M_ROWS_BIG;
            rb[e0 + e] = p < n && (rc[e].y & GS2M_ROWS_BIG) == 0u ? wave_rowbase[(rc[e].x & GS2M_GID_MASK) >> 6] : 0u;
        });
        asm volatile("" ::: "memory");
    });
    levels<E, LE, 1>(key, idx, lane, 0xFFFFFFFFu);
#pragma unroll
    for (int e = 0; e < E; e++) s_r[skew(e * GS2M_WAVE + lane)] += rb[e];
    asm volatile("s_waitcnt lgkmcnt(0)" ::: "memory");
    uint32_t sv[E], sr[E];
    auto pick_up = [&]() {
#pragma unroll
        for (int e = 0; e < E; e++) {
            const bool real = (uint32_t)(lane * E + e) < n;
            sv[e] = real ? s_v[skew((int)idx[e])] : 0u;
            sr[e] = real ? s_r[skew((int)idx[e])] : 0u;
        }
        asm volatile("s_waitcnt lgkmcnt(0)" ::: "memory");
    };
    auto park = [&]() {
#pragma unroll
        for (int e = 0; e < E; e++) {
            s_v[skew(lane * E + e)] = sv[e];
            s_r[skew(lane * E + e)] = sr[e];
        }
    };
    pick_up();
    bool tie = false;
#pragma unroll
    for (int e = 0; e + 1 < E; e++) tie |= (uint32_t)(lane * E + e + 1) < n && key[e] == key[e + 1];
    {
        const uint32_t nxt = (uint32_t)__shfl_down((int)key[0], 1, 64);
        tie |= lane < 63 && (uint32_t)(lane * E + E) < n && key[E - 1] == nxt;
    }
    if (__builtin_amdgcn_ballot_w64(tie) != 0ull) {
#pragma unroll
        for (int e = 0; e < E; e++) {
            s_v[skew(lane * E + e)] = key[e];
            s_r[skew(lane * E + e)] = idx[e];
        }
        asm volatile("s_waitcnt lgkmcnt(0)" ::: "memory");
        uint32_t pos[E];
        tie_positions<E>(key, idx, pos, lane, n, s_v, s_r);
        asm volatile("s_waitcnt lgkmcnt(0)" ::: "memory");
#pragma unroll
        for (int e = 0; e < E; e++) {
            s_v[skew((int)pos[e])] = sv[e];
            s_r[skew((int)pos[e])] = sr[e];
        }
    } else {
        park();
    }
    asm volatile("s_waitcnt lgkmcnt(0)" ::: "memory");
    uint2* out = qlist + (size_t)4 * start;
    uint32_t* orow = qrow + (size_t)4 * start;
    uint32_t run[4] = {0u, 0u, 0u, 0u};
    const unsigned long long lt = lane == 0 ? 0ull : (~0ull >> (64 - lane));
    for (uint32_t base = 0; base < n; base += GS2M_WAVE) {
        const uint32_t k = base + (uint32_t)lane;
        uint32_t v = 0, r = 0;
        if (k < n) {
            v = s_v[skew((int)k)];
            r = s_r[skew((int)k)];
            point_list[start + k] = v;
        }
        const uint32_t mask = v >> GS2M_GID_BITS;
#pragma unroll
        for (int q = 0; q < 4; q++) {
            const bool hit = ((mask >> q) & 1u) != 0u;
            const unsigned long long m = __builtin_amdgcn_ballot_w64(hit);
            if (hit) {
                const size_t o = (size_t)q * n + run[q] + (uint32_t)__popcll(m & lt);
                out[o] = make_uint2(v, k);
                orow[o] = r + (uint32_t)__popc(mask & ((1u << q) - 1u));
            }
            run[q] += (uint32_t)__popcll(m);
        }
    }
    if (lane < 4) qcount[tile * 4 + lane] = lane == 0 ? run[0] : (lane == 1 ? run[1] : (lane == 2 ? run[2] : run[3]));
    asm volatile("s_waitcnt lgkmcnt(0)" ::: "memory");
}

#ifndef GS2M_TS_SUPER_LOG
#define GS2M_TS_SUPER_LOG 2
#endif
__device__ __forceinline__ int tile_of_block(int b, int tiles_x, int tiles_y) {
    constexpr int L = GS2M_TS_SUPER_LOG, SIDE = 1 << L, PER = SIDE * SIDE;
    const int xcd = b & 7, j = b >> 3, sub = j & (PER - 1);
    const int stx = (tiles_x + SIDE - 1) >> L, nsuper = stx * ((tiles_y + SIDE - 1) >> L);
    const int S = (j >> (2 * L)) * 8 + xcd;
    if (S >= nsuper) return -1;
    const int tx = SIDE * (S % stx) + (sub & (SIDE - 1)), ty = SIDE * (S / stx) + (sub >> L);
    if (tx >= tiles_x || ty >= tiles_y) return -1;
    return ty * tiles_x + tx;
}
__host__ __device__ inline unsigned tile_grid(int tiles_x, int tiles_y) {
    constexpr int L = GS2M_TS_SUPER_LOG, SIDE = 1 << L;
    const size_t nsuper = (size_t)((tiles_x + SIDE - 1) >> L) * ((tiles_y + SIDE - 1) >> L);
    return (unsigned)(((nsuper + 7) / 8) * 8 * SIDE * SIDE);
}

__device__ __forceinline__ uint2 tile_range(const uint32_t* __restrict__ ranges_raw, uint2* __restrict__ ranges, int tile, int lane) {
    const uint2 raw = reinterpret_cast<const uint2*>(ranges_raw)[tile];
    const uint2 range = raw.y != 0u ? make_uint2(~raw.x, raw.y) : make_uint2(0u, 0u);
    if (lane == 0) ranges[tile] = range;
    return range;
}

__global__ void __launch_bounds__(64) tile_sort_wave_kernel(const uint32_t* __restrict__ ranges_raw, uint2* __restrict__ ranges,
                                                            const uint32_t* __restrict__ slot_sorted, const uint4* __restrict__ e_rec,
                                                            const uint32_t* __restrict__ wave_rowbase,
                                                            uint32_t* __restrict__ point_list, uint2* __restrict__ qlist,
                                                            uint32_t* __restrict__ qrow, uint32_t* __restrict__ qcount, int tiles_x, int tiles_y,
                                                            uint32_t wave_max , uint32_t* __restrict__ counters) {
    constexpr int M = 64 * 8;
    __shared__ uint32_t s_v[M + M / 32], s_r[M + M / 32];
    const int lane = threadIdx.x;
    const int tile = tile_of_block(blockIdx.x, tiles_x, tiles_y);
    if (tile < 0) return;
    const uint2 range = tile_range(ranges_raw, ranges, tile, lane);
    const uint32_t n = range.y - range.x;
    if (n == 0u) {
        if (lane < 4) qcount[tile * 4 + lane] = 0u;
    } else if (n <= wave_max) {
        sort_tile_wave<8, 3>(tile, range.x, n, slot_sorted, e_rec, wave_rowbase, point_list, qlist, qrow, qcount, s_v, s_r, lane);
    } else if (lane == 0) {
        counters[n <= 1024u ? GS2M_CNT_SPAN_MID : GS2M_CNT_SPAN_LONG] = 1u;
    }
}

__global__ void __launch_bounds__(64) __attribute__((amdgpu_waves_per_eu(4, 8)))
tile_sort_wave16_kernel(const uint32_t* __restrict__ ranges_raw, const uint32_t* __restrict__ slot_sorted, const uint4* __restrict__ e_rec,
                        const uint32_t* __restrict__ wave_rowbase, uint32_t* __restrict__ point_list, uint2* __restrict__ qlist,
                        uint32_t* __restrict__ qrow, uint32_t* __restrict__ qcount, int tiles_x, int tiles_y, const uint32_t* __restrict__ counters) {
    constexpr int M16 = 64 * 16, W16 = M16 + M16 / 32;
    __shared__ uint32_t s_v[W16], s_r[W16];
    if (counters[GS2M_CNT_SPAN_MID] == 0u) return;
    const int lane = threadIdx.x;
    const int tile = tile_of_block(blockIdx.x, tiles_x, tiles_y);
    if (tile < 0) return;
    const uint2 raw = reinterpret_cast<const uint2*>(ranges_raw)[tile];
    const uint32_t start = ~raw.x, n = raw.y != 0u ? raw.y - start : 0u;
    if (n <= 512u || n > 1024u) return;
    sort_tile_wave<16, 4>(tile, start, n, slot_sorted, e_rec, wave_rowbase, point_list, qlist, qrow, qcount, s_v, s_r, lane);
}

template <int E>
__device__ __forceinline__ void cross_wave(uint32_t (&k)[E], uint32_t (&x)[E], const int tid, const int partner, const bool mirrored, const bool lower,
                                           uint32_t* s_x) {
    uint32_t ok[E], ox[E];
#pragma unroll
    for (int e = 0; e < E; e++) s_x[skew(tid * E + e)] = k[e];
    gs2m_sync();
#pragma unroll
    for (int e = 0; e < E; e++) ok[e] = s_x[skew(partner * E + (mirrored ? E - 1 - e : e))];
    gs2m_sync();
#pragma unroll
    for (int e = 0; e < E; e++) s_x[skew(tid * E + e)] = x[e];
    gs2m_sync();
#pragma unroll
    for (int e = 0; e < E; e++) ox[e] = s_x[skew(partner * E + (mirrored ? E - 1 - e : e))];
    gs2m_sync();
#pragma unroll
    for (int e = 0; e < E; e++) {
        const uint32_t mn = min(k[e], ok[e]), mx = max(k[e], ok[e]);
        const uint32_t nk = lower ? mn : mx;
        x[e] = nk == k[e] ? x[e] : ox[e];
        k[e] = nk;
    }
}
template <int E, int LE>
__device__ __forceinline__ void network_wg(uint32_t (&k)[E], uint32_t (&x)[E], const int tid, uint32_t* s_x) {
    const int lane = tid & 63, wave = tid >> 6;
    levels<E, LE, 1>(k, x, lane, 0xFFFFFFFFu);
    cross_wave<E>(k, x, tid, tid ^ 127, true, (wave & 1) == 0, s_x);
    xor_steps<E, LE, LE + 5>(k, x, lane);
    cross_wave<E>(k, x, tid, tid ^ 255, true, wave < 2, s_x);
    cross_wave<E>(k, x, tid, tid ^ 64, false, (wave & 1) == 0, s_x);
    xor_steps<E, LE, LE + 5>(k, x, lane);
}

constexpr int WG_MAX = 4096;
template <int E, int LE>
__device__ __forceinline__ void sort_tile_wg(const int tile, const uint32_t start, const uint32_t n, const uint32_t* __restrict__ slot_sorted,
                                             const uint4* __restrict__ e_rec, const uint32_t* __restrict__ wave_rowbase,
                                             uint32_t* __restrict__ point_list, uint2* __restrict__ qlist, uint32_t* __restrict__ qrow,
                                             uint32_t* __restrict__ qcount, uint32_t* s_v, uint32_t* s_r, uint32_t* s_x, const int tid,
                                             uint32_t* __restrict__ clk = nullptr) {
    const int lane = tid & 63, wave = tid >> 6;
#ifdef GS2M_TS_CLOCK
    const unsigned long long c0 = wall_clock64();
    int cphase = 0;
#define TS_CLK() do { if (tid == 0 && clk) clk[16 * tile + (cphase++)] = (uint32_t)(wall_clock64() - c0); } while (0)
#else
#define TS_CLK() do {} while (0)
#endif
    uint32_t key[E], idx[E], rb[E];
    constexpr int BATCH = E < 8 ? E : 8;
    static_for<0, E / BATCH>([&](auto bc) {
        constexpr int e0 = BATCH * decltype(bc)::value;
        uint32_t slot[BATCH];
#pragma unroll
        for (int e = 0; e < BATCH; e++) {
            const uint32_t p = (uint32_t)((e0 + e) * 256 + tid);
            slot[e] = p < n ? slot_sorted[start + p] : 0u;
        }
        uint4 rc[BATCH];
#pragma unroll
        for (int e = 0; e < BATCH; e++) rc[e] = (uint32_t)((e0 + e) * 256 + tid) < n ? e_rec[slot[e]] : make_uint4(0u, 0u, 0xFFFFFFFFu, 0u);
        static_for<0, BATCH>([&](auto ec) {
            constexpr int e = decltype(ec)::value;
            const uint32_t p = (uint32_t)((e0 + e) * 256 + tid);
            key[e0 + e] = rc[e].z;
            idx[e0 + e] = p;
            s_v[skew((int)p)] = rc[e].x;
            s_r[skew((int)p)] = rc[e].y & ~GS2M_ROWS_BIG;
            rb[e0 + e] = p < n && (rc[e].y & GS2M_ROWS_BIG) == 0u ? wave_rowbase[(rc[e].x & GS2M_GID_MASK) >> 6] : 0u;
        });
        asm volatile("" ::: "memory");
    });
    TS_CLK();
    network_wg<E, LE>(key, idx, tid, s_x);
    TS_CLK();
#pragma unroll
    for (int e = 0; e < E; e++) s_r[skew(e * 256 + tid)] += rb[e];
    uint32_t sv[E], sr[E];
    auto pick_up = [&]() {
#pragma unroll
        for (int e = 0; e < E; e++) {
            const bool real = (uint32_t)(tid * E + e) < n;
            sv[e] = real ? s_v[skew((int)idx[e])] : 0u;
            sr[e] = real ? s_r[skew((int)idx[e])] : 0u;
        }
    };
    auto park = [&]() {
#pragma unroll
        for (int e = 0; e < E; e++) {
            s_v[skew(tid * E + e)] = sv[e];
            s_r[skew(tid * E + e)] = sr[e];
        }
    };
    gs2m_sync();
    pick_up();
    bool tie = false;
#pragma unroll
    for (int e = 0; e + 1 < E; e++) tie |= (uint32_t)(tid * E + e + 1) < n && key[e] == key[e + 1];
    s_x[tid] = key[0];
    gs2m_sync();
    tie |= tid < 255 && (uint32_t)(tid * E + E) < n && key[E - 1] == s_x[tid + 1];
    if (gs2m_sync_or(tie) != 0) {
#pragma unroll
        for (int e = 0; e < E; e++) {
            s_v[skew(tid * E + e)] = key[e];
            s_r[skew(tid * E + e)] = idx[e];
        }
        gs2m_sync();
        uint32_t pos[E];
        tie_positions<E>(key, idx, pos, tid, n, s_v, s_r);
        gs2m_sync();
#pragma unroll
        for (int e = 0; e < E; e++) {
            s_v[skew((int)pos[e])] = sv[e];
            s_r[skew((int)pos[e])] = sr[e];
        }
    } else {
        park();
    }
    TS_CLK();
    gs2m_sync();
    TS_CLK();
    for (uint32_t k = (uint32_t)tid; k < n; k += 256) point_list[start + k] = s_v[skew((int)k)];
    const int q = wave;
    uint2* out = qlist + (size_t)4 * start + (size_t)q * n;
    uint32_t* orow = qrow + (size_t)4 * start + (size_t)q * n;
    uint32_t run = 0;
    const unsigned long long lt = lane == 0 ? 0ull : (~0ull >> (64 - lane));
    for (uint32_t base = 0; base < n; base += GS2M_WAVE) {
        const uint32_t k = base + (uint32_t)lane;
        uint32_t v = 0, r = 0;
        if (k < n) { v = s_v[skew((int)k)]; r = s_r[skew((int)k)]; }
        const uint32_t mask = v >> GS2M_GID_BITS;
        const bool hit = ((mask >> q) & 1u) != 0u;
        const unsigned long long m = __builtin_amdgcn_ballot_w64(hit);
        if (hit) {
            const uint32_t o = run + (uint32_t)__popcll(m & lt);
            out[o] = make_uint2(v, k);
            orow[o] = r + (uint32_t)__popc(mask & ((1u << q) - 1u));
        }
        run += (uint32_t)__popcll(m);
    }
    if (lane == 0) qcount[tile * 4 + q] = run;
    TS_CLK();
#ifdef GS2M_TS_CLOCK
    if (tid == 0 && clk) { clk[16 * tile + 14] = n; clk[16 * tile + 15] = (uint32_t)(c0 & 0xFFFFFFFFull); }
#endif
}

constexpr int BIG_CHUNK = 4096;
__device__ __forceinline__ void sort_tile_big(const int tile, const uint32_t start, const uint32_t n, const uint32_t* __restrict__ slot_sorted,
                                              const uint4* __restrict__ e_rec, const uint32_t* __restrict__ wave_rowbase, uint32_t* __restrict__ point_list,
                                              uint32_t* __restrict__ row_tmp ,
                                              uint2* __restrict__ qlist, uint32_t* __restrict__ qrow, uint32_t* __restrict__ qcount,
                                              uint32_t* s_x ) {
    const int tid = threadIdx.x, wave = tid >> 6, lane = tid & 63;
    uint32_t* const K = reinterpret_cast<uint32_t*>(qlist + (size_t)4 * start);
    uint32_t* const I = K + n;
    auto barrier = [&]() {
        __threadfence_block();
        gs2m_sync();
    };
    constexpr int E = 16, LE = 4;
    for (uint32_t base = 0; base < n; base += BIG_CHUNK) {
        uint32_t key[E], idx[E];
        static_for<0, E / 8>([&](auto bc) {
            constexpr int e0 = 8 * decltype(bc)::value;
            uint32_t slot[8];
#pragma unroll
            for (int e = 0; e < 8; e++) {
                const uint32_t p = base + (uint32_t)((e0 + e) * 256 + tid);
                slot[e] = p < n ? slot_sorted[start + p] : 0u;
            }
            static_for<0, 8>([&](auto ec) {
                constexpr int e = decltype(ec)::value;
                const uint32_t p = base + (uint32_t)((e0 + e) * 256 + tid);
                key[e0 + e] = p < n ? e_rec[slot[e]].z : 0xFFFFFFFFu;
                idx[e0 + e] = p;
            });
        });
        network_wg<E, LE>(key, idx, tid, s_x);
#pragma unroll
        for (int e = 0; e < E; e++) {
            const uint32_t i = base + (uint32_t)(tid * E + e);
            if (i < n) { K[i] = key[e]; I[i] = idx[e]; }
        }
    }
    barrier();
    auto cex = [&](uint32_t i, uint32_t p) {
        const uint32_t a = K[i], b = K[p];
        if (b < a) {
            const uint32_t xa = I[i], xb = I[p];
            K[i] = b; K[p] = a; I[i] = xb; I[p] = xa;
        }
    };
    for (int kb = 13; (1u << (kb - 1)) < n; kb++) {
        const uint32_t half = 1u << (kb - 1), mask = (1u << kb) - 1u;
        for (uint32_t q = tid;; q += 256) {
            const uint32_t i = ((q >> (kb - 1)) << kb) | (q & (half - 1u));
            if (i >= n) break;
            const uint32_t p = i ^ mask;
            if (p < n) cex(i, p);
        }
        barrier();
        for (int jb = kb - 2; jb >= 12; jb--) {
            const uint32_t j = 1u << jb;
            for (uint32_t q = tid;; q += 256) {
                const uint32_t i = ((q >> jb) << (jb + 1)) | (q & (j - 1u));
                if (i >= n) break;
                const uint32_t p = i | j;
                if (p < n) cex(i, p);
            }
            barrier();
        }
        for (uint32_t base = 0; base < n; base += BIG_CHUNK) {
            uint32_t key[E], idx[E];
#pragma unroll
            for (int e = 0; e < E; e++) {
                const uint32_t i = base + (uint32_t)(tid * E + e);
                key[e] = i < n ? K[i] : 0xFFFFFFFFu;
                idx[e] = i < n ? I[i] : i;
            }
            cross_wave<E>(key, idx, tid, tid ^ 128, false, (wave & 2) == 0, s_x);
            cross_wave<E>(key, idx, tid, tid ^ 64, false, (wave & 1) == 0, s_x);
            xor_steps<E, LE, LE + 5>(key, idx, lane);
#pragma unroll
            for (int e = 0; e < E; e++) {
                const uint32_t i = base + (uint32_t)(tid * E + e);
                if (i < n) { K[i] = key[e]; I[i] = idx[e]; }
            }
        }
        barrier();
    }
    uint32_t* const I2 = I + n;
    for (uint32_t p = tid; p < n; p += 256) {
        const uint32_t Kp = K[p], X = I[p];
        uint32_t a = p, cnt = 0;
        for (uint32_t j = p; j > 0u;) {
            j--;
            if (K[j] != Kp) break;
            a = j;
            cnt += I[j] < X ? 1u : 0u;
        }
        for (uint32_t j = p + 1u; j < n; j++) {
            if (K[j] != Kp) break;
            cnt += I[j] < X ? 1u : 0u;
        }
        I2[a + cnt] = X;
    }
    barrier();
    for (uint32_t p = tid; p < n; p += 256) {
        const uint4 rc = e_rec[slot_sorted[start + I2[p]]];
        point_list[start + p] = rc.x;
        row_tmp[start + p] = (rc.y & GS2M_ROWS_BIG) != 0u ? (rc.y & ~GS2M_ROWS_BIG) : rc.y + wave_rowbase[(rc.x & GS2M_GID_MASK) >> 6];
    }
    barrier();
    const int q = wave;
    uint2* out = qlist + (size_t)4 * start + (size_t)q * n;
    uint32_t* orow = qrow + (size_t)4 * start + (size_t)q * n;
    uint32_t run = 0;
    const unsigned long long lt = lane == 0 ? 0ull : (~0ull >> (64 - lane));
    for (uint32_t base = 0; base < n; base += GS2M_WAVE) {
        const uint32_t k = base + (uint32_t)lane;
        uint32_t v = 0, r = 0;
        if (k < n) { v = point_list[start + k]; r = row_tmp[start + k]; }
        const uint32_t mask = v >> GS2M_GID_BITS;
        const bool hit = ((mask >> q) & 1u) != 0u;
        const unsigned long long m = __builtin_amdgcn_ballot_w64(hit);
        if (hit) {
            const uint32_t o = run + (uint32_t)__popcll(m & lt);
            out[o] = make_uint2(v, k);
            orow[o] = r + (uint32_t)__popc(mask & ((1u << q) - 1u));
        }
        run += (uint32_t)__popcll(m);
    }
    if (lane == 0) qcount[tile * 4 + q] = run;
}

#ifndef GS2M_TS_WG_OCC
#define GS2M_TS_WG_OCC 6
#endif
template <int MAXE>
struct WgCfg {
    static constexpr int kMax = 256 * MAXE, kWords = kMax + kMax / 32;
    static constexpr int kLds = 3 * kWords;
};
template <int MAXE>
__global__ void __launch_bounds__(256) __attribute__((amdgpu_waves_per_eu(MAXE >= 8 ? 3 : GS2M_TS_WG_OCC, 8)))
tile_sort_wg_kernel(const uint32_t* __restrict__ ranges_raw, uint2* __restrict__ ranges, const uint32_t* __restrict__ slot_sorted,
                    const uint4* __restrict__ e_rec, const uint32_t* __restrict__ wave_rowbase, uint32_t* __restrict__ point_list,
                    uint32_t* __restrict__ row_tmp, uint2* __restrict__ qlist, uint32_t* __restrict__ qrow, uint32_t* __restrict__ qcount,
                    int tiles_x, int tiles_y, uint32_t nblocks, uint32_t* __restrict__ counters, int take_mid) {
    constexpr int WORDS = WgCfg<MAXE>::kWords;
    __shared__ uint32_t s_all[WgCfg<MAXE>::kLds];
    if constexpr (MAXE >= 8) {
        if (counters[GS2M_CNT_SPAN_LONG] == 0u && !(take_mid && counters[GS2M_CNT_SPAN_MID] != 0u)) return;
    }
    uint32_t* const s_v = s_all, * const s_r = s_all + WORDS, * const s_x = s_all + 2 * WORDS;
    const int tid = threadIdx.x;
    for (uint32_t blk = blockIdx.x; blk < nblocks; blk += gridDim.x) {
        const int tile = tile_of_block((int)blk, tiles_x, tiles_y);
        if (tile < 0) continue;
        const uint2 raw = reinterpret_cast<const uint2*>(ranges_raw)[tile];
        const uint32_t start = raw.y != 0u ? ~raw.x : 0u, n = raw.y != 0u ? raw.y - start : 0u;
        if constexpr (MAXE < 8) {
            if (ranges != nullptr) {
                if (tid == 0) ranges[tile] = raw.y != 0u ? make_uint2(start, raw.y) : make_uint2(0u, 0u);
                if (n == 0u && tid < 4) qcount[tile * 4 + tid] = 0u;
            }
            if (n > 1024u && tid == 0) counters[GS2M_CNT_SPAN_LONG] = 1u;
            if (n == 0u || n > 1024u) continue;
            if (n <= 256u) sort_tile_wg<1, 0>(tile, start, n, slot_sorted, e_rec, wave_rowbase, point_list, qlist, qrow, qcount, s_v, s_r, s_x, tid, row_tmp);
            else if (n <= 512u) sort_tile_wg<2, 1>(tile, start, n, slot_sorted, e_rec, wave_rowbase, point_list, qlist, qrow, qcount, s_v, s_r, s_x, tid, row_tmp);
            else sort_tile_wg<4, 2>(tile, start, n, slot_sorted, e_rec, wave_rowbase, point_list, qlist, qrow, qcount, s_v, s_r, s_x, tid, row_tmp);
        } else {
            if (n <= 512u || (n <= 1024u && !take_mid)) continue;
            if (n <= 1024u) sort_tile_wg<4, 2>(tile, start, n, slot_sorted, e_rec, wave_rowbase, point_list, qlist, qrow, qcount, s_v, s_r, s_x, tid, row_tmp);
            else if (n <= 2048u) sort_tile_wg<8, 3>(tile, start, n, slot_sorted, e_rec, wave_rowbase, point_list, qlist, qrow, qcount, s_v, s_r, s_x, tid, row_tmp);
            else if (n <= (uint32_t)WG_MAX) sort_tile_wg<16, 4>(tile, start, n, slot_sorted, e_rec, wave_rowbase, point_list, qlist, qrow, qcount, s_v, s_r, s_x, tid, row_tmp);
            else sort_tile_big(tile, start, n, slot_sorted, e_rec, wave_rowbase, point_list, row_tmp, qlist, qrow, qcount, s_all);
        }
        gs2m_sync();
    }
}

}

static std::atomic<int> g_ts_policy{0};
void gs2m_set_tile_sort_policy_impl(int policy) { g_ts_policy = policy; }

void gs2m_launch_tile_sort(size_t tiles, int tiles_x, int tiles_y, size_t R , const BinningState& b, const ImageState& im,
                           const GeomState& g, hipStream_t s) {
    if (tiles == 0) return;
    const unsigned grid = tile_grid(tiles_x, tiles_y);
    static const int env_policy = getenv("GS2M_TS_POLICY") ? atoi(getenv("GS2M_TS_POLICY")) : 0;
    const int set_policy = g_ts_policy.load(std::memory_order_relaxed), policy = set_policy != 0 ? set_policy : env_policy;
    const bool waves = policy == 2 || policy == 3 || (policy == 0 && tiles >= 2560);
    const bool mid_own_kernel = policy != 3 && (R == SIZE_MAX || R > (size_t)400 * tiles);
    const unsigned wg_grid = grid < 2048u ? grid : 2048u;
    if (waves) {
        tile_sort_wave_kernel<<<grid, 64, 0, s>>>(im.ranges_raw, im.ranges, b.slot_sorted, b.e_rec, g.wave_rowbase, b.point_list, b.qlist, b.qrow, im.qcount,
                                                  tiles_x, tiles_y, 512u, g.counters);
        if (mid_own_kernel)
            tile_sort_wave16_kernel<<<grid, 64, 0, s>>>(im.ranges_raw, b.slot_sorted, b.e_rec, g.wave_rowbase, b.point_list, b.qlist, b.qrow, im.qcount, tiles_x, tiles_y, g.counters);
    } else {
        tile_sort_wg_kernel<4><<<wg_grid, 256, 0, s>>>(im.ranges_raw, im.ranges, b.slot_sorted, b.e_rec, g.wave_rowbase, b.point_list, b.sort_valA, b.qlist, b.qrow,
                                                       im.qcount, tiles_x, tiles_y, grid, g.counters, 0);
    }
    tile_sort_wg_kernel<16><<<wg_grid < 768u ? wg_grid : 768u , 256, 0, s>>>(im.ranges_raw, nullptr, b.slot_sorted, b.e_rec, g.wave_rowbase, b.point_list, b.sort_valA,
                                                                             b.qlist, b.qrow, im.qcount, tiles_x, tiles_y, grid, g.counters, waves && !mid_own_kernel ? 1 : 0);
}
```

### gs-2m_amd/diff_gaussian_rasterization/__init__.py

```python
from typing import NamedTuple

import ctypes as C
import functools
import os
import threading

import torch
import torch.nn as nn

import gs2m_arena as _arena
import gs2m_native as _native

NUM_CHANNELS = 3
NUM_FEATURES = 10


_ptr = _native.ptr
_f32c = functools.partial(_native.f32, who="gs2m rasterizer", optional=True)


class _Alloc:

    def __init__(self, device):
        self.device = device
        self.tensor = None
        self.cb = _native.ALLOC_FN(self._alloc)

    _pool = threading.local()

    @classmethod
    def three(cls, device):
        pool = cls._pool.__dict__.setdefault("by_device", {})
        key = torch.device(device).index
        a = pool.get(key)
        if a is None:
            a = pool[key] = (cls(device), cls(device), cls(device))
        for x in a:
            x.tensor = None
        return a

    def take(self):
        t, self.tensor = self.tensor, None
        return t if t is not None else torch.empty(0, dtype=torch.uint8, device=self.device)

    def _alloc(self, nbytes, _user):
        try:
            self.tensor = torch.empty(int(nbytes), dtype=torch.uint8, device=self.device)
            return self.tensor.data_ptr()
        except Exception:
            return 0


class _ScratchCache(_Alloc):
    SHRINK_AFTER = 32
    _cache = {}
    _cache_lock = threading.Lock()

    @classmethod
    def get(cls, device, stream):
        key = (torch.device(device).index, stream)
        with cls._cache_lock:
            a = cls._cache.get(key)
            if a is None:
                a = cls._cache[key] = cls(device)
        return a

    @classmethod
    def release(cls):
        with cls._cache_lock:
            cls._cache.clear()

    recent_max = 0
    window = 0

    def _alloc(self, nbytes, _user):
        nbytes = int(nbytes)
        self.recent_max = max(self.recent_max, nbytes)
        self.window += 1
        if self.window >= self.SHRINK_AFTER:
            if self.tensor is not None and self.tensor.numel() > 2 * self.recent_max + (1 << 20):
                self.tensor = None
            self.recent_max, self.window = nbytes, 0
        if self.tensor is not None and self.tensor.numel() >= nbytes:
            return self.tensor.data_ptr()
        self.tensor = None
        return super()._alloc(nbytes + nbytes // 10, _user)


BINNING_CACHE_STATS = {"calls": 0, "busy": 0, "grown": 0}


class _BinningLease:

    def __init__(self):
        self.node = None
        self.ended = False

    def attach(self, ctx):
        import weakref
        self.node = weakref.ref(ctx)

    def over(self):
        if self.ended:
            return True
        if self.node is None:
            return False
        ctx = self.node()
        if ctx is None:
            return True
        try:
            ctx.saved_tensors
        except RuntimeError:
            return True
        except Exception:
            return False
        return False


class _BinningCache:
    _cache = {}
    _lock = threading.RLock()
    SHRINK_AFTER = 32

    def __init__(self):
        self.tensor = None
        self.owner = None
        self.recent_max = 0
        self.window = 0

    @classmethod
    def acquire(cls, device, stream):
        key = (torch.device(device).index, stream)
        lease = _BinningLease()
        with cls._lock:
            e = cls._cache.get(key)
            if e is None:
                e = cls._cache[key] = cls()
            if e.owner is not None and not e.owner.over():
                return e, None
            e.owner = lease
        return e, lease

    def note_request(self, nbytes):
        self.recent_max = max(self.recent_max, int(nbytes))
        self.window += 1
        if self.window >= self.SHRINK_AFTER:
            if self.tensor is not None and self.tensor.numel() > 2 * max(self.recent_max, 1) + 8192:
                self.tensor = None
            self.recent_max, self.window = 0, 0

    @classmethod
    def release(cls):
        with cls._lock:
            cls._cache.clear()


class _CModule:
    _prealloc_cb = None

    @staticmethod
    def rasterize_gaussians(background, means3D, colors, opacities, scales, rotations, scale_modifier, cov3D_precomp,
                            features, viewmatrix, projmatrix, tan_fovx, tan_fovy, image_height, image_width, sh, degree,
                            campos, prefiltered, featureCount, sh_rest=None, _cached_binning=False, _lease_out=None):
        if means3D.dim() != 2 or means3D.size(1) != 3:
            raise RuntimeError("means3D must have dimensions (num_points, 3)")
        means3D = _f32c(means3D, "means3D")
        device = means3D.device
        background = _f32c(background, "bg"); colors = _f32c(colors, "colors_precomp")
        opacities = _f32c(opacities, "opacities"); scales = _f32c(scales, "scales")
        rotations = _f32c(rotations, "rotations"); cov3D_precomp = _f32c(cov3D_precomp, "cov3D_precomp")
        features = _f32c(features, "features"); viewmatrix = _f32c(viewmatrix, "viewmatrix")
        projmatrix = _f32c(projmatrix, "projmatrix"); sh = _f32c(sh, "shs"); campos = _f32c(campos, "campos")
        P, H, W = means3D.size(0), int(image_height), int(image_width)
        M = sh.size(1) if (sh is not None and sh.numel() != 0) else 0
        split = sh_rest is not None and sh_rest.numel() != 0
        if split:
            sh_rest = _f32c(sh_rest, "shs_rest")
            if sh_rest.data_ptr() % 16:
                sh_rest = sh_rest.clone()
            M = 1 + sh_rest.size(1)
        out_color = torch.empty((NUM_CHANNELS, H, W), dtype=torch.float32, device=device)
        out_buffer = torch.empty((NUM_FEATURES, H, W), dtype=torch.float32, device=device)
        radii = torch.empty((P,), dtype=torch.int32, device=device)
        observe = torch.empty((P,), dtype=torch.int32, device=device)
        geom, binning, img = _Alloc.three(device)
        cache, lease = _BinningCache.acquire(device, _native.stream_ptr(device)) if _cached_binning else (None, None)
        pre = None
        if lease is not None and cache.tensor is not None:
            pre = _native.Prealloc(cache.tensor.data_ptr(), cache.tensor.numel(), binning.cb, None, 0, 0)
            if _CModule._prealloc_cb is None:
                _CModule._prealloc_cb = C.cast(_native.lib().gs2m_prealloc_alloc, _native.ALLOC_FN)
            bin_cb, bin_user = _CModule._prealloc_cb, C.byref(pre)
        else:
            bin_cb, bin_user = binning.cb, None
        sh_args = (_ptr(sh), _ptr(sh_rest)) if split else (_ptr(sh),)
        rendered = _native.launch(
            "gs2m_raster_forward_split_sh" if split else "gs2m_raster_forward", device,
            geom.cb, None, bin_cb, bin_user, img.cb, None, P, int(degree), int(M), _ptr(background), W, H,
            _ptr(means3D), *sh_args, _ptr(colors), _ptr(opacities), _ptr(scales), float(scale_modifier),
            _ptr(rotations), _ptr(cov3D_precomp), _ptr(features), _ptr(viewmatrix), _ptr(projmatrix), _ptr(campos),
            float(tan_fovx), float(tan_fovy), int(bool(prefiltered)), int(featureCount), _ptr(out_color),
            _ptr(radii), _ptr(observe), _ptr(out_buffer))
        if _cached_binning:
            BINNING_CACHE_STATS["calls"] += 1
            if lease is None:
                BINNING_CACHE_STATS["busy"] += 1
            elif pre is None or pre.used_fallback:
                BINNING_CACHE_STATS["grown"] += 1
        if pre is not None and not pre.used_fallback:
            bin_tensor = cache.tensor
            cache.note_request(pre.requested)
            if _lease_out is not None:
                _lease_out.append(lease)
            else:
                lease.ended = True
        else:
            bin_tensor = binning.take()
            if lease is not None:
                cache.tensor = torch.empty(int(bin_tensor.numel() * 1.25) + 4096, dtype=torch.uint8, device=device)
                cache.recent_max, cache.window = 0, 0
                lease.ended = True
        return rendered, out_color, radii, observe, out_buffer, geom.take(), bin_tensor, img.take()

    @staticmethod
    def rasterize_gaussians_backward(background, means3D, radii, buffer, colors, scales, rotations, scale_modifier,
                                     cov3D_precomp, features, viewmatrix, projmatrix, tan_fovx, tan_fovy, grad_colors,
                                     grad_buffer, sh, degree, campos, geomBuffer, R, binningBuffer, imageBuffer,
                                     featureCount, return_conics=False, sh_rest=None, unused_input_grads=True, want_sh_grad=True):
        device = means3D.device
        means3D = _f32c(means3D, "means3D")
        P = means3D.size(0)
        H, W = grad_colors.size(1), grad_colors.size(2)
        M = sh.size(1) if (sh is not None and sh.numel() != 0) else 0
        split = sh_rest is not None and sh_rest.numel() != 0
        if split:
            sh_rest = _f32c(sh_rest, "shs_rest")
            if sh_rest.data_ptr() % 16:
                sh_rest = sh_rest.clone()
            M = 1 + sh_rest.size(1)
        grad_colors = _f32c(grad_colors, "grad_colors"); grad_buffer = _f32c(grad_buffer, "grad_buffer")
        background = _f32c(background, "bg"); colors = _f32c(colors, "colors_precomp")
        scales = _f32c(scales, "scales"); rotations = _f32c(rotations, "rotations")
        cov3D_precomp = _f32c(cov3D_precomp, "cov3D_precomp"); features = _f32c(features, "features")
        viewmatrix = _f32c(viewmatrix, "viewmatrix"); projmatrix = _f32c(projmatrix, "projmatrix")
        sh = _f32c(sh, "shs"); campos = _f32c(campos, "campos"); buffer = _f32c(buffer, "buffer")
        radii = radii.contiguous()
        entries = [("means3D", (P, 3)), ("opacities", (P, 1)), ("scales", (P, 3)), ("rotations", (P, 4)),
                   ("features", (P, NUM_FEATURES))]
        if want_sh_grad:
            entries.append(("shs", (P, 1 if split else M, 3)))
            if split:
                entries.append(("shs_rest", (P, M - 1, 3)))
        want_colors = unused_input_grads or (colors is not None and colors.numel() != 0)
        want_cov3D = unused_input_grads or (cov3D_precomp is not None and cov3D_precomp.numel() != 0)
        entries += [("means2D", (P, 4))] + ([("colors", (P, NUM_CHANNELS))] if want_colors else []) + ([("cov3D", (P, 6))] if want_cov3D else [])
        if return_conics:
            entries.append(("conics", (P, 2, 2)))
        arena = _arena.GradArena(device, entries, zero=(P == 0), key="rasterizer")
        dL_dmeans3D = arena["means3D"]; dL_dmeans2D = arena["means2D"]; dL_dcolors = arena.get("colors")
        dL_dfeatures = arena["features"]; dL_dopacities = arena["opacities"]; dL_dcov3D = arena.get("cov3D")
        dL_dshs = arena.get("shs"); dL_dscales = arena["scales"]; dL_drotations = arena["rotations"]
        dL_dshs_rest = arena.get("shs_rest")
        dL_dconics = arena.get("conics")
        scratch = _ScratchCache.get(device, _native.stream_ptr(device))
        sh_args = (_ptr(sh), _ptr(sh_rest)) if split else (_ptr(sh),)
        dsh_args = (_ptr(dL_dshs), _ptr(dL_dshs_rest)) if split else (_ptr(dL_dshs),)
        _native.launch(
            "gs2m_raster_backward_split_sh" if split else "gs2m_raster_backward", device,
            P, int(degree), int(M), int(R), _ptr(background), W, H, _ptr(means3D), *sh_args, _ptr(colors),
            _ptr(scales), float(scale_modifier), _ptr(rotations), _ptr(cov3D_precomp), _ptr(features),
            _ptr(viewmatrix), _ptr(projmatrix), _ptr(campos), float(tan_fovx), float(tan_fovy), _ptr(radii),
            _ptr(buffer), _ptr(geomBuffer), _ptr(binningBuffer), _ptr(imageBuffer), int(featureCount),
            _ptr(grad_colors), _ptr(grad_buffer), _ptr(dL_dmeans2D), _ptr(dL_dconics), _ptr(dL_dopacities),
            _ptr(dL_dcolors), _ptr(dL_dmeans3D), _ptr(dL_dcov3D), *dsh_args, _ptr(dL_dscales),
            _ptr(dL_drotations), _ptr(dL_dfeatures), scratch.cb, None)
        out = (dL_dmeans2D, dL_dcolors, dL_dopacities, dL_dmeans3D, dL_dcov3D, dL_dshs, dL_dscales, dL_drotations,
               dL_dfeatures)
        if split:
            out = out + (dL_dshs_rest,)
        return out + (dL_dconics,) if return_conics else out

    @staticmethod
    def mark_visible(means3D, viewmatrix, projmatrix):
        means3D = _f32c(means3D, "means3D")
        P = means3D.size(0)
        present = torch.zeros((P,), dtype=torch.bool, device=means3D.device)
        if P != 0:
            _native.launch("gs2m_raster_mark_visible", means3D.device, P, _ptr(means3D), _ptr(_f32c(viewmatrix, "viewmatrix")),
                           _ptr(_f32c(projmatrix, "projmatrix")), present.data_ptr())
        return present


_C = _CModule()


def release_scratch():
    _ScratchCache.release()
    _BinningCache.release()
    _arena.release()


def rasterize_gaussians(means3D, means2D, shs, colors_precomp, opacities, scales, rotations, cov3Ds_precomp, features,
                        raster_settings, shs_rest=None):
    if shs_rest is None:
        shs_rest = torch.Tensor([])
    return _RasterizeGaussians.apply(means3D, means2D, shs, colors_precomp, opacities, scales, rotations,
                                     cov3Ds_precomp, features, raster_settings, shs_rest)


_zero_image_cache = {}


def _zero_image(buffer):
    key = (buffer.device, buffer.shape[1], buffer.shape[2])
    z = _zero_image_cache.get(key)
    if z is None:
        if len(_zero_image_cache) > 8:
            _zero_image_cache.clear()
        z = _zero_image_cache[key] = torch.zeros((NUM_CHANNELS, buffer.shape[1], buffer.shape[2]), dtype=torch.float32, device=buffer.device)
    return z


class _RasterizeGaussians(torch.autograd.Function):
    @staticmethod
    def forward(ctx, means3D, means2D, shs, colors_precomp, opacities, scales, rotations, cov3Ds_precomp, features,
                raster_settings, shs_rest):
        args = (raster_settings.bg, means3D, colors_precomp, opacities, scales, rotations,
                raster_settings.scale_modifier, cov3Ds_precomp, features, raster_settings.viewmatrix,
                raster_settings.projmatrix, raster_settings.tanfovx, raster_settings.tanfovy,
                raster_settings.image_height, raster_settings.image_width, shs, raster_settings.sh_degree,
                raster_settings.campos, raster_settings.prefiltered, raster_settings.feature_count)
        lease = []
        num_rendered, color, radii, observe, buffer, geomBuffer, binningBuffer, imgBuffer = _C.rasterize_gaussians(
            *args, sh_rest=shs_rest, _cached_binning=True, _lease_out=lease)
        ctx.forward_token = _native.lib().gs2m_raster_forward_token()
        ctx.binning_lease = lease[0] if lease else None
        if lease:
            lease[0].attach(ctx)
        ctx.raster_settings = raster_settings
        ctx.num_rendered = num_rendered
        ctx.set_materialize_grads(False)
        ctx.save_for_backward(buffer, features, colors_precomp, means3D, scales, rotations, cov3Ds_precomp, radii, shs,
                              geomBuffer, binningBuffer, imgBuffer, shs_rest)
        ctx.mark_non_differentiable(radii, observe)
        return color, radii, observe, buffer

    @staticmethod
    def backward(ctx, grad_out_color, grad_out_radii, grad_out_observe, grad_out_buffer):
        num_rendered = ctx.num_rendered
        raster_settings = ctx.raster_settings
        (buffer, features, colors_precomp, means3D, scales, rotations, cov3Ds_precomp, radii, shs, geomBuffer,
         binningBuffer, imgBuffer, shs_rest) = ctx.saved_tensors
        color_dead = grad_out_color is None and os.environ.get("GS2M_KEEP_DEAD_SH") is None
        if grad_out_color is None:
            grad_out_color = _zero_image(buffer)
        if grad_out_buffer is None:
            grad_out_buffer = torch.zeros_like(buffer)
        args = (raster_settings.bg, means3D, radii, buffer, colors_precomp, scales, rotations,
                raster_settings.scale_modifier, cov3Ds_precomp, features, raster_settings.viewmatrix,
                raster_settings.projmatrix, raster_settings.tanfovx, raster_settings.tanfovy, grad_out_color,
                grad_out_buffer, shs, raster_settings.sh_degree, raster_settings.campos, geomBuffer, num_rendered,
                binningBuffer, imgBuffer, raster_settings.feature_count)
        L = _native.lib()
        dense_rows = L.gs2m_raster_dense_rows(ctx.forward_token)
        if dense_rows >= 0:
            L.gs2m_raster_backward_rows_hint(dense_rows)
        res = _C.rasterize_gaussians_backward(*args, sh_rest=shs_rest, unused_input_grads=False, want_sh_grad=not color_dead)
        (grad_means2D, grad_colors_precomp, grad_opacities, grad_means3D, grad_cov3Ds_precomp, grad_sh, grad_scales,
         grad_rotations, grad_features) = res[:9]
        grad_sh_rest = res[9] if len(res) > 9 else None

        def opt(g, x):
            return g if (x is not None and x.numel() != 0) else None

        return (grad_means3D, grad_means2D, opt(grad_sh, shs), opt(grad_colors_precomp, colors_precomp), grad_opacities,
                opt(grad_scales, scales), opt(grad_rotations, rotations), opt(grad_cov3Ds_precomp, cov3Ds_precomp),
                opt(grad_features, features), None, grad_sh_rest)


class GaussianRasterizationSettings(NamedTuple):
    image_height: int
    image_width: int
    tanfovx: float
    tanfovy: float
    bg: torch.Tensor
    scale_modifier: float
    viewmatrix: torch.Tensor
    projmatrix: torch.Tensor
    sh_degree: int
    campos: torch.Tensor
    prefiltered: bool
    feature_count: int


class GaussianRasterizer(nn.Module):
    def __init__(self, raster_settings):
        super().__init__()
        self.raster_settings = raster_settings

    def markVisible(self, positions):
        with torch.no_grad():
            raster_settings = self.raster_settings
            visible = _C.mark_visible(positions, raster_settings.viewmatrix, raster_settings.projmatrix)
        return visible

    def forward(self, means3D, means2D, opacities, shs=None, colors_precomp=None, scales=None, rotations=None,
                cov3D_precomp=None, features=None, shs_rest=None):
        raster_settings = self.raster_settings

        if (shs is None and colors_precomp is None) or (shs is not None and colors_precomp is not None):
            raise Exception('Please provide excatly one of either SHs or precomputed colors!')

        if ((scales is None or rotations is None) and cov3D_precomp is None) or \
                ((scales is not None or rotations is not None) and cov3D_precomp is not None):
            raise Exception('Please provide exactly one of either scale/rotation pair or precomputed 3D covariance!')

        if shs is None:
            shs = torch.Tensor([])
        if colors_precomp is None:
            colors_precomp = torch.Tensor([])
        if scales is None:
            scales = torch.Tensor([])
        if rotations is None:
            rotations = torch.Tensor([])
        if cov3D_precomp is None:
            cov3D_precomp = torch.Tensor([])
        if features is None:
            features = torch.Tensor([])

        return rasterize_gaussians(means3D, means2D, shs, colors_precomp, opacities, scales, rotations, cov3D_precomp,
                                   features, raster_settings, shs_rest=shs_rest)
```

### gs-2m_amd/gs2m_native.py

```python
import ctypes as C
import os
import subprocess

_HERE = os.path.dirname(os.path.abspath(__file__))
CSRC = os.path.join(_HERE, "csrc")
LIB_PATH = os.environ.get("GS2M_LIB", os.path.join(CSRC, "libgs2m_raster.so"))

ALLOC_FN = C.CFUNCTYPE(C.c_void_p, C.c_size_t, C.c_void_p)


class Prealloc(C.Structure):
    _fields_ = [("ptr", C.c_void_p), ("capacity", C.c_size_t), ("fallback", ALLOC_FN), ("fallback_user", C.c_void_p),
                ("used_fallback", C.c_int), ("requested", C.c_size_t)]


class Layout(C.Structure):
    _fields_ = [(n, C.c_uint64) for n in (
        "geom_bytes", "rec", "tiles_touched", "depth_key", "rect", "gauss_rows", "clamped", "wave_rowbase", "counters",
        "binning_bytes", "point_list", "tile_keys", "qlist", "qrow",
        "image_bytes", "final_T", "n_contrib", "ranges", "qcount")]


class STREAM(C.c_void_p):
    """`void* stream` as an entry point's LAST parameter: the function enqueues GPU work (call it through `launch`)."""


p, i, f, d, ll, ull, A, s = C.c_void_p, C.c_int, C.c_float, C.c_double, C.c_longlong, C.c_ulonglong, ALLOC_FN, STREAM
SIGNATURES = {
    "gs2m_raster_forward": (i, [A, p, A, p, A, p, i, i, i, p, i, i, p, p, p, p, p, f, p, p, p, p, p, p, f, f, i, i, p,
                                p, p, p, s]),
    "gs2m_raster_backward": (i, [i, i, i, i, p, i, i, p, p, p, p, f, p, p, p, p, p, p, f, f, p, p, p, p, p, i, p, p, p,
                                 p, p, p, p, p, p, p, p, p, A, p, s]),
    "gs2m_raster_mark_visible": (i, [i, p, p, p, p, s]),
    "gs2m_knn_dist2": (i, [i, p, p, A, p, s]),
    "gs2m_debug_layout": (i, [i, i, i, i, C.POINTER(Layout)]),
    "gs2m_set_reference_binning": (i, [i]),
    "gs2m_raster_forward_split_sh": (i, [A, p, A, p, A, p, i, i, i, p, i, i, p, p, p, p, p, p, f, p, p, p, p, p, p, f,
                                         f, i, i, p, p, p, p, s]),
    "gs2m_raster_backward_split_sh": (i, [i, i, i, i, p, i, i, p, p, p, p, p, f, p, p, p, p, p, p, f, f, p, p, p, p, p,
                                          i, p, p, p, p, p, p, p, p, p, p, p, p, p, A, p, s]),
    "gs2m_pack_features_forward": (i, [i, p, p, p, p, p, p, p, p, i, i, p, s]),
    "gs2m_pack_features_backward": (i, [i, p, p, p, p, p, i, i, p, p, p, p, p, p, s]),
    "gs2m_gbuffer_post_forward": (i, [i, i, p, p, p, i, p, p, p, s]),
    "gs2m_gbuffer_post_backward": (i, [i, i, p, p, p, i, p, p, p, s]),
    "gs2m_gbuffer_maps_backward": (i, [i, i, p, p, p, i, p, p, p, p, p, p, p, p, p, s]),
    "gs2m_sobel_normal_forward": (i, [i, i, p, p, p, p, f, f, f, f, p, s]),
    "gs2m_sobel_normal_backward": (i, [i, i, p, p, p, p, f, f, f, f, p, p, p, s]),
    "gs2m_activate_forward": (i, [i, p, p, p, p, p, p, p, p, p, p, p, p, s]),
    "gs2m_activate_backward": (i, [i, p, p, p, p, p, p, p, p, p, p, p, p, p, p, p, p, p, p, s]),
    "gs2m_set_spin_wait": (i, [i]),
    "gs2m_set_sort_tickets": (i, [i]),
    "gs2m_set_tile_sort_policy": (i, [i]),
    "gs2m_prealloc_alloc": (p, [C.c_size_t, p]),
    "gs2m_set_debug": (i, [i]),
    "gs2m_set_markers": (i, [i]),
    "gs2m_stage_name": (C.c_char_p, [i]),
    "gs2m_raster_forward_token": (ull, []),
    "gs2m_raster_dense_rows": (ll, [ull]),
    "gs2m_raster_backward_rows_hint": (i, [ll]),
    "gs2m_debug_tile_sort": (i, [i, p, p, p, p, p, p, p, p, p, p, s]),
    "gs2m_profile_mode": (i, [i]),
    "gs2m_profile_sampling": (i, [i]),
    "gs2m_profile_collect": (i, [C.POINTER(C.c_float), C.POINTER(C.c_int), i]),
    "gs2m_version": (C.c_char_p, []),
    "gs2m_texture_cube_forward": (i, [i, i, i, p, p, p, p, p, s]),
    "gs2m_texture_cube_backward": (i, [i, i, i, p, p, p, p, p, i, s]),
    "gs2m_texture_2d_clamp_forward": (i, [i, i, i, i, p, p, p, s]),
    "gs2m_texture_2d_clamp_backward": (i, [i, i, i, i, p, p, p, s]),
    "gs2m_diffuse_cubemap_forward": (i, [i, p, p, s]),
    "gs2m_diffuse_cubemap_backward": (i, [i, p, p, s]),
    "gs2m_cubemap_texel_table": (i, [i, p, s]),
    "gs2m_specular_cubemap_forward": (i, [i, f, f, p, p, p, s]),
    "gs2m_specular_cubemap_backward": (i, [i, f, f, p, p, p, s]),
    "gs2m_specular_cubemap_normalized_forward": (i, [i, f, f, p, p, p, p, s]),
    "gs2m_specular_cubemap_normalized_backward": (i, [i, f, f, p, p, p, p, p, s]),
    "gs2m_pbr_shade_forward": (i, [i, p, p, p, p, p, p, i, i, p, i, i, p, p, f, f, p, p, p, p, s]),
    "gs2m_pbr_shade_backward": (i, [i, p, p, p, p, p, p, i, i, p, i, i, p, p, f, f, p, p, p, p, p, i, s]),
    "gs2m_pbr_inputs_forward": (i, [i, i, p, p, p, p, p, f, f, p, p, p, p, s]),
    "gs2m_pbr_inputs_backward": (i, [i, i, p, p, p, s]),
    "gs2m_patch_ncc_forward": (i, [i, p, p, p, p, p, i, i, p, p, p, f, i, p, s]),
    "gs2m_patch_ncc_backward": (i, [i, p, p, p, p, p, i, i, p, p, p, f, i, p, p, p, s]),
    "gs2m_patch_ncc_roughness": (i, [i, p, p, p, p, p, i, i, p, p, p, f, i, p, p, p, s]),
    "gs2m_mvs_set_deterministic": (None, [i]),
    "gs2m_mvs_get_deterministic": (i, []),
    "gs2m_grid_sample_border_forward": (i, [i, i, i, i, p, p, p, s]),
    "gs2m_grid_sample_border_backward": (i, [i, i, i, i, p, p, p, p, p, s]),
    "gs2m_mv_geo_forward": (i, [i, i, i, i, p, p, p, p, p, p, p, p, p, p, f, p, p, p, s]),
    "gs2m_mv_geo_backward": (i, [i, i, i, i, p, p, p, p, p, p, p, p, p, p, f, p, p, p, p, p, p, s]),
    "gs2m_adam_step": (i, [i, p, d, d, d, s]),
    "gs2m_ssim_forward": (i, [i, i, i, i, f, f, p, p, p, p, p, p, s]),
    "gs2m_ssim_backward": (i, [i, i, i, i, p, p, p, p, p, p, p, s]),
    "gs2m_ssim_backward_uniform": (i, [i, i, i, i, p, p, p, f, f, p, p, p, p, s]),
    "gs2m_loss_workspace_bytes": (i, []),
    "gs2m_edge_gradient": (i, [i, i, p, p, p, p, s]),
    "gs2m_image_loss_forward": (i, [i, i, p, i, p, p, p, p, p, p, p, p, f, f, p, p, p, s]),
    "gs2m_image_loss_backward": (i, [i, i, p, i, p, p, p, p, p, p, p, f, f, p, p, p, p, p, s]),
    "gs2m_tv_loss_forward": (i, [i, i, i, p, p, p, i, f, p, p, s]),
    "gs2m_tv_loss_backward": (i, [i, i, i, p, p, p, i, f, p, p, s]),
    "gs2m_mv_geo_loss_forward": (i, [i, p, p, p, f, f, f, f, p, p, p, p, s]),
    "gs2m_mv_geo_loss_backward": (i, [i, p, p, p, f, f, f, f, p, p, p, p, s]),
    "gs2m_mv_take_forward": (i, [i, p, i, i, p, p, p, p, p, p, p, s]),
    "gs2m_mv_take_backward": (i, [i, p, i, i, p, p, p, p, s]),
    "gs2m_ncc_tail_forward": (i, [i, p, p, p, p, s]),
    "gs2m_ncc_tail_backward": (i, [i, p, p, p, p, p, s]),
    "gs2m_subset_thin": (i, [i, p, i, ull, p, i, p, p, s]),
    "gs2m_subset_remove": (i, [i, i, ull, p, p, s]),
    "gs2m_affine_mean": (i, [ll, p, f, f, p, p, s]),
    "gs2m_plane_loss_forward": (i, [i, p, i, p, f, p, p, s]),
    "gs2m_plane_loss_backward": (i, [i, p, i, p, f, p, p, p, s]),
    "gs2m_densification_stats": (i, [i, p, p, p, p, p, p, p, p, s]),
    "gs2m_tsdf_workspace_bytes": (i, [p, i, p, p]),
    "gs2m_tsdf_points_aabb": (i, [i, i, p, f, f, f, f, f, p, p, s]),
    "gs2m_tsdf_touch": (i, [p, f, f, i, i, p, f, f, f, f, f, p, i, p, p, p, p, p, p, s]),
    "gs2m_tsdf_integrate": (i, [f, f, i, i, p, p, f, f, f, f, f, p, i, p, p, p, p, p, s]),
    "gs2m_tsdf_mesh_count": (i, [p, i, p, p, p, p, p, p, s]),
    "gs2m_tsdf_mesh_emit": (i, [p, f, i, p, p, p, p, p, ll, ll, p, p, p, s]),
    "gs2m_tsdf_block_coords": (i, [i, p, p, s]),
    "gs2m_mesh_post_workspace_bytes": (i, [ll, ll, p, p]),
    "gs2m_mesh_cluster_triangles": (i, [ll, ll, p, p, p, p, p, s]),
    "gs2m_mesh_keep_clusters": (i, [ll, p, p, i, p, s]),
    "gs2m_mesh_compact": (i, [ll, ll, p, p, p, p, p, p, p, p, p, s]),
    "gs2m_eval_transform": (i, [ll, p, d, p, p, s]),
    "gs2m_eval_sample_workspace_bytes": (i, [ll, ll, p, p]),
    "gs2m_eval_sample_rows": (i, [ll, p, ll, p, d, p, p, s]),
    "gs2m_eval_sample_count": (i, [ll, ll, p, p, p, s]),
    "gs2m_eval_sample_emit": (i, [ll, p, ll, p, ll, p, p, ll, p, s]),
    "gs2m_eval_gather": (i, [ll, p, p, p, s]),
    "gs2m_eval_grid_bytes": (i, [ll, p, p]),
    "gs2m_eval_grid_build": (i, [ll, p, d, p, p, s]),
    "gs2m_eval_thin_workspace_bytes": (i, [ll, p]),
    "gs2m_eval_thin": (i, [ll, p, p, d, p, p, p, s]),
    "gs2m_eval_filter": (i, [ll, p, p, p, p, d, p, p, p, s]),
    "gs2m_eval_above_plane": (i, [ll, p, p, p, s]),
    "gs2m_eval_scan_workspace_bytes": (i, [ll, p]),
    "gs2m_eval_compact": (i, [ll, p, p, i, p, p, p, s]),
    "gs2m_eval_nearest": (i, [ll, p, ll, d, p, d, p, s]),
    "gs2m_eval_nearest_index": (i, [ll, p, ll, d, p, d, p, p, s]),
    "gs2m_eval_masked_mean": (i, [ll, p, d, p, p, p, s]),
    "gs2m_tnt_mesh_points": (i, [ll, p, ll, p, p, p, s]),
    "gs2m_tnt_transform": (i, [ll, p, p, p, s]),
    "gs2m_tnt_crop_flags": (i, [ll, p, i, d, d, i, p, p, s]),
    "gs2m_tnt_voxel_workspace_bytes": (i, [ll, p]),
    "gs2m_tnt_voxel_downsample": (i, [ll, p, d, p, p, p, s]),
    "gs2m_tnt_stride_gather": (i, [ll, p, ll, p, s]),
    "gs2m_tnt_icp_workspace_bytes": (i, [p]),
    "gs2m_tnt_icp_moments": (i, [ll, p, ll, p, p, p, p, p, s]),
    "gs2m_tnt_histogram": (i, [ll, p, i, p, p, s]),
}
del p, i, f, d, ll, ull, A, s
EXPORTS = tuple(SIGNATURES)

STAGES = ("preprocess", "unused1", "scan", "emit", "tile_sort", "lists", "blend_fwd", "unused7", "blend_bwd",
          "gaussian_bwd")

_lib = None


def build(jobs=8, force=False):
    cmd = ["make", "-C", CSRC, "-j", str(jobs)]
    if force:
        cmd.append("-B")
    subprocess.check_call(cmd, stdout=subprocess.DEVNULL)
    return LIB_PATH


def lib():
    global _lib
    if _lib is not None:
        return _lib
    if not os.path.exists(LIB_PATH):
        raise RuntimeError(
            f"gs2m: HIP extension not built: {LIB_PATH} is missing. Run `python -c 'import __graft_entry__ as g; "
            f"g.build()'` (needs hipcc, --offload-arch=gfx950). There is no CPU fallback.")
    L = C.CDLL(LIB_PATH)
    for name, (restype, argtypes) in SIGNATURES.items():
        fn = getattr(L, name)
        fn.restype, fn.argtypes = restype, argtypes
    _lib = L
    return L


ERRORS = {-1: "invalid argument", -2: "HIP runtime error", -3: "scratch allocation failed", -4: "unsupported size",
          -5: "Point culled! This point should have been prefiltered (prefiltered=True and a Gaussian has view z <= 0.2; the reference traps the device here, cuda_rasterizer/auxiliary.h:155-158)"}


class _NoGuard:
    def __enter__(self):
        return None

    def __exit__(self, *exc):
        return False


_NO_GUARD = _NoGuard()


def device_guard(device):
    import torch
    idx = device.index if hasattr(device, "index") else device
    if idx is None or idx == torch.cuda.current_device():
        return _NO_GUARD
    return torch.cuda.device(device)


def stream_ptr(device=None):
    import torch
    idx = None if device is None else (device.index if hasattr(device, "index") else device)
    if idx is None:
        idx = torch.cuda.current_device()
    return torch._C._cuda_getCurrentRawStream(idx)


def check(rc, what):
    if rc <= -100:
        raise RuntimeError(f"gs2m: {what} failed in stage `{lib().gs2m_stage_name(-100 - rc).decode()}` (debug mode)")
    if rc < 0:
        raise RuntimeError(f"gs2m: {what} failed: {ERRORS.get(rc, rc)}")
    return rc


def launch(name, device, *args):
    fn = getattr(lib(), name)
    if fn.argtypes[-1] is not STREAM:
        raise TypeError(f"gs2m: {name} takes no stream: call it as check(lib().{name}(...), ...)")
    with device_guard(device):
        return check(fn(*args, stream_ptr(device)), name)


def ptr(t):
    return None if t is None or t.numel() == 0 else t.data_ptr()


def f32(t, name, shape=None, *, who, optional=False):
    import torch
    if optional and (t is None or t.numel() == 0):
        return t
    if not isinstance(t, torch.Tensor) or not t.is_cuda:
        raise RuntimeError(f"{who}: `{name}` must be a CUDA tensor on a HIP device; there is no CPU path")
    if t.dtype != torch.float32:
        raise RuntimeError(f"{who}: `{name}` must be float32, got {t.dtype}")
    if shape is not None and tuple(t.shape) != tuple(shape):
        raise RuntimeError(f"{who}: `{name}` must have shape {tuple(shape)}, got {tuple(t.shape)}")
    return t.contiguous()


def set_debug(on):
    check(lib().gs2m_set_debug(int(bool(on))), "gs2m_set_debug")


def set_markers(on):
    check(lib().gs2m_set_markers(int(bool(on))), "gs2m_set_markers")


def reset_modes():
    L = lib()
    L.gs2m_set_reference_binning(0); L.gs2m_set_spin_wait(1); L.gs2m_set_debug(0); L.gs2m_set_sort_tickets(0); L.gs2m_set_tile_sort_policy(0)
    L.gs2m_set_markers(0); L.gs2m_profile_mode(0)


def debug_layout(P, R, W, H):
    lay = Layout()
    check(lib().gs2m_debug_layout(P, R, W, H, C.byref(lay)), "gs2m_debug_layout")
    return lay


def set_sort_tickets(on):
    check(lib().gs2m_set_sort_tickets(int(bool(on))), "gs2m_set_sort_tickets")


def set_tile_sort_policy(policy):
    check(lib().gs2m_set_tile_sort_policy(int(policy)), "gs2m_set_tile_sort_policy")


def set_spin_wait(on):
    check(lib().gs2m_set_spin_wait(int(bool(on))), "gs2m_set_spin_wait")


def profile_mode(mode, every=1):
    check(lib().gs2m_profile_sampling(int(every)), "gs2m_profile_sampling")
    check(lib().gs2m_profile_mode(int(mode)), "gs2m_profile_mode")


def profile_collect():
    n = len(STAGES)
    ms = (C.c_float * n)()
    cnt = (C.c_int * n)()
    check(lib().gs2m_profile_collect(ms, cnt, n), "gs2m_profile_collect")
    return {STAGES[k]: (float(ms[k]), int(cnt[k])) for k in range(n)}


def set_reference_binning(on):
    check(lib().gs2m_set_reference_binning(1 if on else 0), "gs2m_set_reference_binning")
```

### include/gs2m_raster.h

```cpp
#ifndef GS2M_RASTER_H
#define GS2M_RASTER_H

#include <stddef.h>
#include <stdint.h>

#ifdef __cplusplus
extern "C" {
#endif

#define GS2M_NUM_CHANNELS 3
#define GS2M_NUM_FEATURES 10
#define GS2M_TILE 16

#define GS2M_OK 0
#define GS2M_ERR_INVALID_ARG (-1)
#define GS2M_ERR_HIP (-2)
#define GS2M_ERR_ALLOC (-3)
#define GS2M_ERR_UNSUPPORTED (-4)
#define GS2M_ERR_PREFILTERED (-5)
#define GS2M_ERR_STAGE(st) (-100 - (st))

typedef char* (*gs2m_alloc_fn)(size_t bytes, void* user);

int gs2m_raster_forward(
    gs2m_alloc_fn geometry_alloc, void* geometry_user,
    gs2m_alloc_fn binning_alloc, void* binning_user,
    gs2m_alloc_fn image_alloc, void* image_user,
    int P, int D, int M,
    const float* background,
    int width, int height,
    const float* means3D,
    const float* shs,
    const float* colors_precomp,
    const float* opacities,
    const float* scales,
    float scale_modifier,
    const float* rotations,
    const float* cov3D_precomp,
    const float* features,
    const float* viewmatrix,
    const float* projmatrix,
    const float* cam_pos,
    float tan_fovx, float tan_fovy,
    int prefiltered,
    int feature_count,
    float* out_color,
    int* out_radii,
    int* out_observe,
    float* out_buffer,
    void* stream);

int gs2m_raster_backward(
    int P, int D, int M, int R,
    const float* background,
    int width, int height,
    const float* means3D,
    const float* shs,
    const float* colors_precomp,
    const float* scales,
    float scale_modifier,
    const float* rotations,
    const float* cov3D_precomp,
    const float* features,
    const float* viewmatrix,
    const float* projmatrix,
    const float* campos,
    float tan_fovx, float tan_fovy,
    const int* radii,
    const float* buffer,
    char* geom_buffer,
    char* binning_buffer,
    char* image_buffer,
    int feature_count,
    const float* grad_colors,
    const float* grad_buffer,
    float* dL_dmeans2D,
    float* dL_dconics,
    float* dL_dopacities,
    float* dL_dcolors,
    float* dL_dmeans3D,
    float* dL_dcov3D,
    float* dL_dshs,
    float* dL_dscales,
    float* dL_drots,
    float* dL_dfeatures,
    gs2m_alloc_fn scratch_alloc, void* scratch_user,
    void* stream);

int gs2m_raster_mark_visible(int P, const float* means3D, const float* viewmatrix,
                             const float* projmatrix, uint8_t* present, void* stream);

int gs2m_knn_dist2(int P, const float* points, float* mean_dists,
                   gs2m_alloc_fn scratch_alloc, void* scratch_user, void* stream);


typedef struct gs2m_layout {
    uint64_t geom_bytes;
    uint64_t rec;
    uint64_t tiles_touched;
    uint64_t depth_key;
    uint64_t rect;
    uint64_t gauss_rows;
    uint64_t clamped;
    uint64_t wave_rowbase;
    uint64_t counters;
    uint64_t binning_bytes;
    uint64_t point_list;
    uint64_t tile_keys;
    uint64_t qlist;
    uint64_t qrow;
    uint64_t image_bytes;
    uint64_t final_T;
    uint64_t n_contrib;
    uint64_t ranges;
    uint64_t qcount;
} gs2m_layout;

int gs2m_debug_layout(int P, int R, int width, int height, gs2m_layout* out);

int gs2m_set_reference_binning(int on);

int gs2m_raster_forward_split_sh(gs2m_alloc_fn geometry_alloc, void* geometry_user, gs2m_alloc_fn binning_alloc,
                        void* binning_user, gs2m_alloc_fn image_alloc, void* image_user, int P, int D, int M,
                        const float* background, int width, int height, const float* means3D, const float* sh_dc, const float* sh_rest,
                        const float* colors_precomp, const float* opacities, const float* scales, float scale_modifier,
                        const float* rotations, const float* cov3D_precomp, const float* features,
                        const float* viewmatrix, const float* projmatrix, const float* cam_pos, float tan_fovx,
                        float tan_fovy, int prefiltered, int feature_count, float* out_color, int* out_radii,
                        int* out_observe, float* out_buffer, void* stream_);
int gs2m_raster_backward_split_sh(int P, int D, int M, int R, const float* background, int width, int height,
                         const float* means3D, const float* sh_dc, const float* sh_rest, const float* colors_precomp, const float* scales,
                         float scale_modifier, const float* rotations, const float* cov3D_precomp,
                         const float* features, const float* viewmatrix, const float* projmatrix, const float* campos,
                         float tan_fovx, float tan_fovy, const int* radii, const float* buffer, char* geom_buffer,
                         char* binning_buffer, char* image_buffer, int feature_count, const float* grad_colors,
                         const float* grad_buffer, float* dL_dmeans2D, float* dL_dconics, float* dL_dopacities,
                         float* dL_dcolors, float* dL_dmeans3D, float* dL_dcov3D, float* dL_dsh_dc, float* dL_dsh_rest, float* dL_dscales,
                         float* dL_drots, float* dL_dfeatures, gs2m_alloc_fn scratch_alloc, void* scratch_user,
                         void* stream_);

int gs2m_pack_features_forward(int P, const float* xyz, const float* scales, const float* rotations, const float* albedo,
                               const float* roughness, const float* metallic, const float* campos, const float* view,
                               int z_depth, int blend_metallic, float* features, void* stream);
int gs2m_pack_features_backward(int P, const float* xyz, const float* scales, const float* rotations, const float* campos,
                                const float* view, int z_depth, int blend_metallic, const float* dL_dfeatures,
                                float* dL_dxyz, float* dL_drotations, float* dL_dalbedo, float* dL_droughness,
                                float* dL_dmetallic, void* stream);
int gs2m_gbuffer_post_forward(int width, int height, const float* buffer, const float* rays, const float* view, int z_depth,
                              uint8_t* normal_mask, float* local_normal_map, float* depth_map, void* stream);
int gs2m_gbuffer_post_backward(int width, int height, const float* buffer, const float* rays, const float* view,
                               int z_depth, const float* dL_dlocal_normal, const float* dL_ddepth, float* dL_dbuffer,
                               void* stream);

int gs2m_gbuffer_maps_backward(int width, int height, const float* buffer, const float* rays, const float* view,
                               int z_depth, const float* dL_dlocal_normal, const float* dL_ddepth, const float* dL_dalpha,
                               const float* dL_ddistance, const float* dL_dnormal, const float* dL_dalbedo,
                               const float* dL_droughness, const float* dL_dmetallic, float* dL_dbuffer, void* stream);

int gs2m_sobel_normal_forward(int width, int height, const float* depth, const float* alpha, const float* bg,
                              const float* view, float fx, float fy, float cx, float cy, float* sobel_map, void* stream);
int gs2m_sobel_normal_backward(int width, int height, const float* depth, const float* alpha, const float* bg,
                               const float* view, float fx, float fy, float cx, float cy, const float* dL_dsobel,
                               float* dL_ddepth, float* dL_dalpha, void* stream);

int gs2m_activate_forward(int P, const float* scaling, const float* rotation, const float* opacity, const float* albedo,
                          const float* roughness, const float* metallic, float* scales, float* rotations, float* opacities,
                          float* albedo_a, float* roughness_a, float* metallic_a, void* stream);
int gs2m_activate_backward(int P, const float* rotation, const float* scales, const float* opacities, const float* albedo_a,
                           const float* roughness_a, const float* metallic_a, const float* dL_dscales,
                           const float* dL_drotations, const float* dL_dopacities, const float* dL_dalbedo_a,
                           const float* dL_droughness_a, const float* dL_dmetallic_a, float* dL_dscaling, float* dL_drotation,
                           float* dL_dopacity, float* dL_dalbedo, float* dL_droughness, float* dL_dmetallic, void* stream);

int gs2m_set_spin_wait(int on);

int gs2m_set_sort_tickets(int on);

int gs2m_set_tile_sort_policy(int policy);

typedef struct gs2m_prealloc {
    char* ptr;
    size_t capacity;
    gs2m_alloc_fn fallback;
    void* fallback_user;
    int used_fallback;
    size_t requested;
} gs2m_prealloc;
char* gs2m_prealloc_alloc(size_t bytes, void* user);

int gs2m_set_debug(int on);
int gs2m_set_markers(int on);
const char* gs2m_stage_name(int stage);


unsigned long long gs2m_raster_forward_token(void);
long long gs2m_raster_dense_rows(unsigned long long token);
int gs2m_raster_backward_rows_hint(long long dense_rows);

int gs2m_debug_tile_sort(int tiles, const unsigned* ranges_raw, unsigned* ranges, const unsigned* slot_sorted, const unsigned* e_rec,
                         const unsigned* wave_rowbase, unsigned* point_list, unsigned* row_tmp,
                         unsigned* qlist, unsigned* qrow, unsigned* qcount, void* stream);

#define GS2M_NUM_STAGES 10
int gs2m_profile_mode(int mode);
int gs2m_profile_sampling(int every);
int gs2m_profile_collect(float* stage_ms, int* stage_count, int n_stages);

const char* gs2m_version(void);

#ifdef __cplusplus
}
#endif
#endif
```

Baseline: 853.2 views/s.

## Queue forward emit/sort/blend speculatively before host learns instance count

When a cached binning buffer is available, the forward pass sizes the binning layout from the cached capacity and enqueues emit, tile sort, list building and blending right after the scan. It does this before spinning on the host for the rendered-instance count. Device kernels check a spec-fail flag and read the count from device counters, so the GPU does not sit idle during the host round trip. If the guess overflows, the host falls back to the exact path using the fallback allocator. The backward pass gets a carve hint so it uses the same buffer layout. This adds device-side flag checks, oversized buffers and a costly rerun when the speculation fails.

```diff
diff --git a/gs-2m_amd/csrc/api.hip b/gs-2m_amd/csrc/api.hip
--- a/gs-2m_amd/csrc/api.hip
+++ b/gs-2m_amd/csrc/api.hip
@@ -35,6 +35,7 @@
 thread_local uint64_t t_last_token = 0;
 thread_local long long t_rows_hint = -1;
 thread_local long long t_units_hint = -1, t_units_from_token = -1;
+thread_local long long t_last_carved = 0, t_carve_hint = -1;
 
 static_assert(GS2M_NUM_STAGES == 10, "stage table");
 enum Stage { ST_PREPROCESS = 0, ST_UNUSED1, ST_SCAN, ST_EMIT, ST_TILE_SORT, ST_LISTS, ST_BLEND_FWD, ST_UNUSED7,
@@ -55,6 +56,23 @@
 std::atomic<int> g_spin_wait{1};
 std::atomic<int> g_debug{0};
 std::atomic<int> g_markers{0};
+std::atomic<int> g_speculative{1};
+
+uint32_t fit_instances(size_t capacity, uint32_t ucap, int tile_bits) {
+    thread_local size_t m_capacity = 0;
+    thread_local uint32_t m_ucap = 0, m_rcap = 0;
+    thread_local int m_bits = -1;
+    if (capacity == m_capacity && ucap == m_ucap && tile_bits == m_bits) return m_rcap;
+    auto fits = [&](size_t r) { return gs2m_carve_binning(nullptr, r, gs2m_binning_temp_bytes(r, tile_bits), ucap).total_bytes <= capacity; };
+    size_t lo = 0, hi = ((size_t)1 << 29) - 1;
+    if (fits(hi)) lo = hi;
+    while (hi - lo > 1) {
+        const size_t mid = lo + (hi - lo) / 2;
+        if (fits(mid)) lo = mid; else hi = mid;
+    }
+    m_capacity = capacity; m_ucap = ucap; m_bits = tile_bits; m_rcap = (uint32_t)lo;
+    return m_rcap;
+}
 
 const char* const kStageNames[ST_COUNT] = {"preprocess", "-", "scan", "emit", "tile_sort", "depth_order+quad_lists", "blend_fwd", "-", "blend_bwd", "gaussian_bwd"};
 
@@ -129,7 +147,7 @@
     return p->fallback ? p->fallback(bytes, p->fallback_user) : nullptr;
 }
 
-const char* gs2m_version(void) { return "gs2m_raster 0.5 (gfx950, round 5)"; }
+const char* gs2m_version(void) { return "gs2m_raster 0.6 (gfx950, speculative forward)"; }
 
 static int forward_impl(gs2m_alloc_fn geometry_alloc, void* geometry_user, gs2m_alloc_fn binning_alloc,
                         void* binning_user, gs2m_alloc_fn image_alloc, void* image_user, int P, int D, int M,
@@ -194,8 +212,57 @@
     land[GS2M_LAND_ROWS] = 0u;
     t_last_token = ((uint64_t)(dev_id + 1) << 40) | ((uint64_t)(generation & 0xFFFFFFFFu) << 8) | slot;
 
+    const int tile_bits = (int)higher_msb((uint32_t)tiles);
+    auto queue_from_emit = [&](const BinningState& b, size_t Rn, uint32_t Un, uint32_t crowded, const SpecCaps& spec, size_t Rguess) -> int {
+        if (Rn > 0) {
+            {
+                StageTimer t(ST_EMIT, s, &failed_stage);
+                ZeroJobs zj = {{nullptr, im.ranges_raw, nullptr}, {0, tiles * 2, 0}};
+                gs2m_radix_zero_region(b.temp, Rn, tile_bits, &zj.p[0], &zj.words[0]);
+                gs2m_launch_emit(P, width, height, tiles_x, tile_bits, g, b, Un, crowded, land_dev, zj, spec, s);
+            }
+            if (g_debug.load(std::memory_order_relaxed)) {
+                uint32_t total = 0;
+                HIP_TRY(hipStreamSynchronize(s));
+                HIP_TRY(hipMemcpy(&total, g.counters, sizeof(total), hipMemcpyDeviceToHost));
+                if (total != (uint32_t)Rn) return GS2M_ERR_STAGE(ST_EMIT);
+            }
+            {
+                StageTimer t(ST_TILE_SORT, s, &failed_stage);
+                HIP_TRY(gs2m_radix_sort_pairs(b.temp, b.temp_bytes, b.keys_unsorted, nullptr, b.sort_keyA, b.sort_valA, b.tile_keys, b.slot_sorted,
+                                              Rn, tile_bits, true, s, im.ranges_raw, g.tile_hist, spec.on ? g.counters : nullptr));
+            }
+        } else {
+            HIP_TRY(gs2m_zero_async(im.ranges_raw, tiles * 2 * sizeof(uint32_t), s));
+            land[GS2M_LAND_ROWS] = 1u;
+            if (land[GS2M_LAND_HUNITS] == 0xFFFFFFFFu) land[GS2M_LAND_HUNITS] = 0u;
+        }
+        DEBUG_CHECK();
+        {
+            StageTimer t(ST_LISTS, s, &failed_stage);
+            gs2m_launch_tile_sort(tiles, tiles_x, tiles_y, Rguess, b, im, g, s, spec.on != 0u);
+        }
+        {
+            StageTimer t(ST_BLEND_FWD, s, &failed_stage);
+            gs2m_launch_blend_fwd_q(width, height, tiles_x, tiles_y, feature_count, background, g, b, im, out_color, out_buffer, out_observe, s);
+        }
+        DEBUG_CHECK();
+        HIP_TRY(hipGetLastError());
+        return GS2M_OK;
+    };
+
+    gs2m_prealloc* const pre = binning_alloc == gs2m_prealloc_alloc ? static_cast<gs2m_prealloc*>(binning_user) : nullptr;
+    SpecCaps spec = {0u, 0u, 0u};
+    if (pre && pre->ptr && P > 0 && g_speculative.load() && !g_debug.load()) {
+        const uint32_t ucap = (uint32_t)(pre->units_capacity < ((size_t)1 << 22) - 1 ? pre->units_capacity : ((size_t)1 << 22) - 1);
+        const uint32_t rcap = fit_instances(pre->capacity, ucap, tile_bits);
+        if (rcap > 0u) spec = {1u, rcap, ucap};
+    }
+    const SpecCaps exact = {0u, 0u, 0u};
+
     int R = 0;
     uint32_t U = 0, crowded = GS2M_CROWDED_WAVE;
+    bool forced_fallback = false;
     if (P > 0) {
         {
             StageTimer t(ST_PREPROCESS, s, &failed_stage);
@@ -208,10 +275,15 @@
         if (prefiltered) gs2m_launch_prefiltered_check(P, means3D, viewmatrix, land_dev + GS2M_LAND_PREFILTERED, s);
         {
             StageTimer t(ST_SCAN, s, &failed_stage);
-            gs2m_launch_blockscan(P, g, land_dev, s);
+            gs2m_launch_blockscan(P, g, land_dev, spec, s);
         }
         HIP_TRY(hipGetLastError());
         DEBUG_CHECK();
+        if (spec.on) {
+            const BinningState b = gs2m_carve_binning(pre->ptr, spec.rcap, gs2m_binning_temp_bytes(spec.rcap, tile_bits), spec.ucap);
+            const int rc = queue_from_emit(b, spec.rcap, spec.ucap, GS2M_CROWDED_WAVE, spec, (size_t)spec.rcap / 5 * 4);
+            if (rc < 0) return rc;
+        }
         if (spin_wait) {
             const auto t0 = std::chrono::steady_clock::now();
             uint32_t spins = 0;
@@ -225,6 +297,16 @@
             HIP_TRY(hipStreamSynchronize(s));
             return GS2M_ERR_PREFILTERED;
         }
+        if (spec.on && !gs2m_spec_fails(land[GS2M_LAND_R], land[GS2M_LAND_HUNITS], spec.rcap, spec.ucap)) {
+            R = (int)land[GS2M_LAND_R];
+            U = land[GS2M_LAND_HUNITS];
+            const size_t Rn = R > 0 ? (size_t)R : 1;
+            pre->requested = gs2m_carve_binning(nullptr, Rn, gs2m_binning_temp_bytes(Rn, tile_bits), U).total_bytes;
+            pre->units = U;
+            t_last_carved = (long long)spec.rcap;
+            return R;
+        }
+        forced_fallback = spec.on != 0u;
         if (land[GS2M_LAND_R] >= (1u << 29)) return GS2M_ERR_UNSUPPORTED;
         R = (int)land[GS2M_LAND_R];
         U = land[GS2M_LAND_HUNITS];
@@ -233,7 +315,7 @@
             land[GS2M_LAND_R] = 0xFFFFFFFFu;
             land[GS2M_LAND_HUNITS] = 0xFFFFFFFFu;
             gs2m_launch_recount_heavy(P, g, s);
-            gs2m_launch_blockscan(P, g, land_dev, s);
+            gs2m_launch_blockscan(P, g, land_dev, exact, s);
             HIP_TRY(hipGetLastError());
             HIP_TRY(hipStreamSynchronize(s));
             if (land[GS2M_LAND_R] != (uint32_t)R) return GS2M_ERR_STAGE(ST_SCAN);
@@ -242,48 +324,24 @@
         if (U >= (1u << 22)) return GS2M_ERR_UNSUPPORTED;
     }
 
-    const int tile_bits = (int)higher_msb((uint32_t)tiles);
     const size_t Rn = R > 0 ? (size_t)R : 1;
     const size_t btemp = gs2m_binning_temp_bytes(Rn, tile_bits);
     BinningState bsz = gs2m_carve_binning(nullptr, Rn, btemp, U);
-    char* bbase = binning_alloc(bsz.total_bytes, binning_user);
+    char* bbase = nullptr;
+    if (forced_fallback) {
+        pre->requested = bsz.total_bytes;
+        pre->used_fallback = 1;
+        bbase = pre->fallback ? pre->fallback(bsz.total_bytes, pre->fallback_user) : nullptr;
+    } else {
+        bbase = binning_alloc(bsz.total_bytes, binning_user);
+    }
     if (!bbase) return GS2M_ERR_ALLOC;
+    if (pre) pre->units = U;
     BinningState b = gs2m_carve_binning(bbase, Rn, btemp, U);
-
-    if (R > 0) {
-        {
-            StageTimer t(ST_EMIT, s, &failed_stage);
-            ZeroJobs zj = {{nullptr, im.ranges_raw, nullptr}, {0, tiles * 2, 0}};
-            gs2m_radix_zero_region(b.temp, (size_t)R, tile_bits, &zj.p[0], &zj.words[0]);
-            gs2m_launch_emit(P, width, height, tiles_x, tile_bits, g, b, U, crowded, land_dev, zj, s);
-        }
-        if (g_debug.load(std::memory_order_relaxed)) {
-            uint32_t total = 0;
-            HIP_TRY(hipStreamSynchronize(s));
-            HIP_TRY(hipMemcpy(&total, g.counters, sizeof(total), hipMemcpyDeviceToHost));
-            if (total != (uint32_t)R) return GS2M_ERR_STAGE(ST_EMIT);
-        }
-        {
-            StageTimer t(ST_TILE_SORT, s, &failed_stage);
-            HIP_TRY(gs2m_radix_sort_pairs(b.temp, b.temp_bytes, b.keys_unsorted, nullptr, b.sort_keyA, b.sort_valA, b.tile_keys, b.slot_sorted,
-                                          (size_t)R, tile_bits, true, s, im.ranges_raw, g.tile_hist));
-        }
-    } else {
-        HIP_TRY(gs2m_zero_async(im.ranges_raw, tiles * 2 * sizeof(uint32_t), s));
-        land[GS2M_LAND_ROWS] = 1u;
-        if (land[GS2M_LAND_HUNITS] == 0xFFFFFFFFu) land[GS2M_LAND_HUNITS] = 0u;
-    }
-    DEBUG_CHECK();
-    {
-        StageTimer t(ST_LISTS, s, &failed_stage);
-        gs2m_launch_tile_sort(tiles, tiles_x, tiles_y, (size_t)(R > 0 ? R : 0), b, im, g, s);
-    }
-    {
-        StageTimer t(ST_BLEND_FWD, s, &failed_stage);
-        gs2m_launch_blend_fwd_q(width, height, tiles_x, tiles_y, feature_count, background, g, b, im, out_color, out_buffer, out_observe, s);
-    }
-    DEBUG_CHECK();
-    HIP_TRY(hipGetLastError());
+    t_last_carved = (long long)Rn;
+
+    const int rc = queue_from_emit(b, (size_t)(R > 0 ? R : 0), U, crowded, exact, (size_t)(R > 0 ? R : 0));
+    if (rc < 0) return rc;
     return R;
 }
 
@@ -311,7 +369,10 @@
 
     const int tiles_x = (width + GS2M_TILE - 1) / GS2M_TILE, tiles_y = (height + GS2M_TILE - 1) / GS2M_TILE;
     const size_t tiles = (size_t)tiles_x * tiles_y, N = (size_t)width * height;
-    const size_t Rn = R > 0 ? (size_t)R : 1;
+    const long long carve_hint = t_carve_hint;
+    t_carve_hint = -1;
+    if (carve_hint > 0 && (carve_hint < (long long)R || carve_hint >= (1ll << 29))) return GS2M_ERR_INVALID_ARG;
+    const size_t Rn = carve_hint > 0 ? (size_t)carve_hint : (R > 0 ? (size_t)R : 1);
     GeomState g = gs2m_carve_geom(geom_buffer, (size_t)P);
     BinningState b = gs2m_carve_binning(binning_buffer, Rn, gs2m_binning_temp_bytes(Rn, (int)higher_msb((uint32_t)tiles)), 0);
     ImageState im = gs2m_carve_image(image_buffer, N, tiles);
@@ -322,7 +383,7 @@
     t_rows_hint = -1;
     t_units_hint = -1;
     size_t nrows = 0;
-    if (hint >= 0 && (size_t)hint <= Rn * 10 + 256) {
+    if (hint >= 0 && (size_t)hint <= (size_t)(R > 0 ? R : 1) * 10 + 256) {
         nrows = (size_t)hint;
     } else if (R > 0) {
         uint32_t c[2] = {0u, 0u};
@@ -424,6 +485,11 @@
 int gs2m_set_tile_sort_policy(int policy) {
     if (policy < 0 || policy > 3) return GS2M_ERR_INVALID_ARG;
     gs2m_set_tile_sort_policy_impl(policy);
+    return GS2M_OK;
+}
+
+int gs2m_set_speculative_forward(int on) {
+    g_speculative = on ? 1 : 0;
     return GS2M_OK;
 }
 
@@ -539,6 +605,13 @@
     return GS2M_OK;
 }
 
+long long gs2m_raster_forward_carved(void) { return t_last_carved; }
+
+int gs2m_raster_backward_carve_hint(long long carved_instances) {
+    t_carve_hint = carved_instances;
+    return GS2M_OK;
+}
+
 int gs2m_debug_tile_sort(int tiles, const unsigned* ranges_raw, unsigned* ranges, const unsigned* slot_sorted, const unsigned* e_rec,
                          const unsigned* wave_rowbase, unsigned* point_list, unsigned* row_tmp, unsigned* qlist,
                          unsigned* qrow, unsigned* qcount, void* stream_) {
diff --git a/gs-2m_amd/csrc/binning.hip b/gs-2m_amd/csrc/binning.hip
--- a/gs-2m_amd/csrc/binning.hip
+++ b/gs-2m_amd/csrc/binning.hip
@@ -160,7 +160,7 @@
 
 __global__ void __launch_bounds__(1024) blockscan_kernel(const uint32_t* __restrict__ block_tt, const uint32_t* __restrict__ block_hu, size_t nblocks,
                                                          uint32_t* __restrict__ block_pref, uint32_t* __restrict__ block_hupref,
-                                                         uint32_t* __restrict__ counters, uint32_t* landing) {
+                                                         uint32_t* __restrict__ counters, uint32_t* landing, SpecCaps spec) {
     __shared__ uint32_t s_w[32];
     __shared__ unsigned long long s_part[32];
     unsigned long long t = 0, u = 0;
@@ -173,13 +173,15 @@
         counters[GS2M_CNT_HUNITS] = u32;
         counters[GS2M_CNT_SPAN_MID] = 0u;
         counters[GS2M_CNT_SPAN_LONG] = 0u;
+        counters[GS2M_CNT_SPEC_FAIL] = spec.on != 0u && gs2m_spec_fails(t, u, spec.rcap, spec.ucap) ? 1u : 0u;
     }
 }
 
 __global__ void __launch_bounds__(1024) rowscan_kernel(const uint32_t* __restrict__ wave_rows, size_t nwaves, uint32_t* __restrict__ wave_rowbase,
-                                                       uint32_t* __restrict__ counters, uint32_t* landing) {
+                                                       uint32_t* __restrict__ counters, uint32_t* landing, uint32_t spec) {
     __shared__ uint32_t s_w[16];
     __shared__ unsigned long long s_part[16];
+    if (spec != 0u && counters[GS2M_CNT_SPEC_FAIL] != 0u) return;
     const uint32_t heavy_rows = 4u * GS2M_UNIT * counters[GS2M_CNT_HUNITS];
     const unsigned long long total = heavy_rows + scan_1024_per_block(wave_rows, nwaves, s_w, s_part, [&](size_t w, uint32_t excl, uint32_t) { wave_rowbase[w] = heavy_rows + excl; });
     if (blockIdx.x == gridDim.x - 1 && threadIdx.x == 0) {
@@ -207,7 +209,7 @@
                                                    HeavyUnit* __restrict__ hrec,
                                                    uint32_t* __restrict__ gauss_rows, uint32_t* __restrict__ wave_rows,
                                                    uint32_t* __restrict__ counters, uint32_t* __restrict__ tile_hist, int npass, int4 hbits,
-                                                   int4 hshift, uint32_t crowded, ZeroJobs zero) {
+                                                   int4 hshift, uint32_t crowded, ZeroJobs zero, uint32_t spec) {
     __shared__ uint32_t s_th[4][256];
     __shared__ uint32_t s_pref[4][GS2M_WAVE];
     __shared__ uint32_t s_rmin[4][GS2M_WAVE];
@@ -221,6 +223,7 @@
     const int i = blockIdx.x * 256 + threadIdx.x;
     const int wave = threadIdx.x >> 6, lane = threadIdx.x & 63;
     gs2m_zero_jobs(zero, (size_t)i, (size_t)gridDim.x * 256);
+    if (spec != 0u && counters[GS2M_CNT_SPEC_FAIL] != 0u) return;
 #pragma unroll
     for (int p = 0; p < 4; p++) s_th[p][threadIdx.x] = 0u;
     const int hb[4] = {hbits.x, hbits.y, hbits.z, hbits.w}, hs[4] = {hshift.x, hshift.y, hshift.z, hshift.w};
@@ -315,11 +318,17 @@
     if (threadIdx.x == 0) block_hu[blockIdx.x] = s_hu[0] + s_hu[1] + s_hu[2] + s_hu[3];
 }
 
-__global__ void __launch_bounds__(256) emit_heavy_kernel(uint32_t units, int W, int H, int tiles_x, const uint2* __restrict__ rect, const float4* __restrict__ rec,
+__global__ void __launch_bounds__(256) emit_heavy_kernel(uint32_t units , int W, int H, int tiles_x, const uint2* __restrict__ rect, const float4* __restrict__ rec,
                                                          const uint32_t* __restrict__ depth_key, const uint32_t* __restrict__ gauss_rows,
                                                          uint32_t* __restrict__ keys_out, uint4* __restrict__ e_rec, HeavyUnit* __restrict__ hrec,
-                                                         uint32_t* __restrict__ tile_hist, int npass, int4 hbits, int4 hshift) {
+                                                         uint32_t* __restrict__ tile_hist, int npass, int4 hbits, int4 hshift,
+                                                         const uint32_t* __restrict__ counters, uint32_t spec) {
     __shared__ uint32_t s_th[4][256];
+    if (spec != 0u) {
+        if (counters[GS2M_CNT_SPEC_FAIL] != 0u) return;
+        units = counters[GS2M_CNT_HUNITS];
+        if (blockIdx.x * 4u >= units) return;
+    }
 #pragma unroll
     for (int p = 0; p < 4; p++) s_th[p][threadIdx.x] = 0u;
     gs2m_sync();
@@ -356,10 +365,10 @@
 
 }
 
-void gs2m_launch_blockscan(int P, const GeomState& g, uint32_t* landing, hipStream_t s) {
+void gs2m_launch_blockscan(int P, const GeomState& g, uint32_t* landing, const SpecCaps& spec, hipStream_t s) {
     const size_t nb = (size_t)(P + 255) / 256;
     blockscan_kernel<<<(unsigned)((nb + 1023) / 1024 > 0 ? (nb + 1023) / 1024 : 1), 1024, 0, s>>>(g.block_tt, g.block_hu, nb, g.block_pref, g.block_hupref, g.counters,
-                                                                                                  landing);
+                                                                                                  landing, spec);
 }
 
 void gs2m_launch_recount_heavy(int P, const GeomState& g, hipStream_t s) {
@@ -367,17 +376,18 @@
 }
 
 void gs2m_launch_emit(int P, int W, int H, int tiles_x, int tile_bits, const GeomState& g, const BinningState& b, uint32_t heavy_units, uint32_t crowded,
-                      uint32_t* landing, const ZeroJobs& zero, hipStream_t s) {
+                      uint32_t* landing, const ZeroJobs& zero, const SpecCaps& spec, hipStream_t s) {
     int npass = 0, bits[4], shift[4];
     gs2m_radix_plan(tile_bits, &npass, bits, shift);
     const int4 hbits = make_int4(bits[0], bits[1], bits[2], bits[3]), hshift = make_int4(shift[0], shift[1], shift[2], shift[3]);
     emit_kernel<<<(P + 255) / 256, 256, 0, s>>>(P, W, H, tiles_x, g.rect, g.block_pref, g.block_hupref, g.rec, g.depth_key, b.keys_unsorted, b.e_rec, b.hrec,
-                                                g.gauss_rows, g.wave_rows, g.counters, g.tile_hist, npass, hbits, hshift, crowded, zero);
+                                                g.gauss_rows, g.wave_rows, g.counters, g.tile_hist, npass, hbits, hshift, crowded, zero, spec.on);
+    if (spec.on) heavy_units = spec.ucap;
     if (heavy_units > 0u)
         emit_heavy_kernel<<<(heavy_units + 3u) / 4u, 256, 0, s>>>(heavy_units, W, H, tiles_x, g.rect, g.rec, g.depth_key, g.gauss_rows, b.keys_unsorted, b.e_rec,
-                                                                  b.hrec, g.tile_hist, npass, hbits, hshift);
+                                                                  b.hrec, g.tile_hist, npass, hbits, hshift, g.counters, spec.on);
     const size_t nw = (size_t)(P + 63) / 64;
-    rowscan_kernel<<<(unsigned)((nw + 1023) / 1024 > 0 ? (nw + 1023) / 1024 : 1), 1024, 0, s>>>(g.wave_rows, nw, g.wave_rowbase, g.counters, landing);
+    rowscan_kernel<<<(unsigned)((nw + 1023) / 1024 > 0 ? (nw + 1023) / 1024 : 1), 1024, 0, s>>>(g.wave_rows, nw, g.wave_rowbase, g.counters, landing, spec.on);
 }
 
 __global__ void zero_kernel(uint32_t* __restrict__ p, size_t words) {
diff --git a/gs-2m_amd/csrc/common.h b/gs-2m_amd/csrc/common.h
--- a/gs-2m_amd/csrc/common.h
+++ b/gs-2m_amd/csrc/common.h
@@ -178,7 +178,7 @@
 size_t gs2m_radix_temp_bytes(size_t n, int total_bits);
 hipError_t gs2m_radix_sort_pairs(void* temp, size_t temp_bytes, const uint32_t* kin, const uint32_t* vin, uint32_t* kA,
                                  uint32_t* vA, uint32_t* kB, uint32_t* vB, size_t n, int total_bits, bool prezeroed, hipStream_t s,
-                                 uint32_t* range_raw = nullptr, const uint32_t* ext_hist = nullptr);
+                                 uint32_t* range_raw = nullptr, const uint32_t* ext_hist = nullptr, const uint32_t* spec_counters = nullptr);
 #define GS2M_HIST_COPIES 8
 #define GS2M_HIST_COPY_WORDS 1024
 void gs2m_radix_plan(int total_bits, int* npass, int bits[4], int shift[4]);
@@ -192,6 +192,15 @@
 #define GS2M_CNT_HUNITS 3
 #define GS2M_CNT_SPAN_MID 4
 #define GS2M_CNT_SPAN_LONG 5
+#define GS2M_CNT_SPEC_FAIL 6
+struct SpecCaps {
+    uint32_t on;
+    uint32_t rcap;
+    uint32_t ucap;
+};
+__host__ __device__ inline bool gs2m_spec_fails(unsigned long long r, unsigned long long u, uint32_t rcap, uint32_t ucap) {
+    return r > rcap || u > ucap || u * 4ull * 64ull  > 6ull * r + 65536ull;
+}
 
 void gs2m_launch_preprocess(int P, int D, int M, const float* means3D, const float* scales, float scale_modifier,
                             const float* rotations, const float* opacities, const float* shs, const float* shs_rest,
@@ -199,13 +208,14 @@
                             const float* viewmatrix, const float* projmatrix, const float* cam_pos, int W, int H,
                             float tan_fovx, float tan_fovy, float focal_x, float focal_y, int tiles_x, int tiles_y,
                             int* radii, int* observe_zero, const GeomState& g, int shrink, const ZeroJobs& zero, hipStream_t s);
-void gs2m_launch_blockscan(int P, const GeomState& g, uint32_t* landing, hipStream_t s);
+void gs2m_launch_blockscan(int P, const GeomState& g, uint32_t* landing, const SpecCaps& spec, hipStream_t s);
 void gs2m_launch_emit(int P, int W, int H, int tiles_x, int tile_bits, const GeomState& g, const BinningState& b, uint32_t heavy_units,
-                      uint32_t crowded, uint32_t* landing, const ZeroJobs& zero, hipStream_t s);
+                      uint32_t crowded, uint32_t* landing, const ZeroJobs& zero, const SpecCaps& spec, hipStream_t s);
 void gs2m_launch_recount_heavy(int P, const GeomState& g, hipStream_t s);
 void gs2m_launch_heavy_reduce(float* rows, int rowf, const BinningState& b, const GeomState& g, long long heavy_units, hipStream_t s);
 void gs2m_set_tile_sort_policy_impl(int policy);
-void gs2m_launch_tile_sort(size_t tiles, int tiles_x, int tiles_y, size_t R, const BinningState& b, const ImageState& im, const GeomState& g, hipStream_t s);
+void gs2m_launch_tile_sort(size_t tiles, int tiles_x, int tiles_y, size_t R, const BinningState& b, const ImageState& im, const GeomState& g, hipStream_t s,
+                           bool R_on_device = false);
 hipError_t gs2m_zero_async(void* p, size_t bytes, hipStream_t s);
 
 void gs2m_launch_blend_fwd_q(int W, int H, int tiles_x, int tiles_y, int fc, const float* bg, const GeomState& g,
diff --git a/gs-2m_amd/csrc/radix_sort.hip b/gs-2m_amd/csrc/radix_sort.hip
--- a/gs-2m_amd/csrc/radix_sort.hip
+++ b/gs-2m_amd/csrc/radix_sort.hip
@@ -92,7 +92,8 @@
 __global__ void __launch_bounds__(RS_THREADS) rs_onesweep_kernel(
     const uint32_t* __restrict__ keys_in, const uint32_t* __restrict__ vals_in, uint32_t* __restrict__ keys_out,
     uint32_t* __restrict__ vals_out, uint32_t n, int shift, const uint32_t* __restrict__ ghist, uint32_t* ticket,
-    uint32_t* status , uint32_t* range_raw, int hist_copies ) {
+    uint32_t* status , uint32_t* range_raw, int hist_copies ,
+    const uint32_t* __restrict__ spec_counters ) {
     constexpr int BINS = 1 << BITS;
     __shared__ uint32_t s_cnt[4][BINS];
     __shared__ uint32_t s_gbase[256];
@@ -100,10 +101,15 @@
     __shared__ uint32_t s_tile;
     __shared__ uint32_t s_key[RS_TILE], s_val[RS_TILE];
     const int tid = threadIdx.x, wave = tid >> 6, lane = tid & 63;
+    if (spec_counters != nullptr) {
+        if (spec_counters[GS2M_CNT_SPEC_FAIL] != 0u) return;
+        n = spec_counters[1];
+    }
     if (tid == 0) s_tile = ticket != nullptr ? atomicAdd(ticket, 1u) : blockIdx.x;
     for (int i = tid; i < 4 * BINS; i += RS_THREADS) (&s_cnt[0][0])[i] = 0;
     gs2m_sync();
     const uint32_t tile = s_tile;
+    if ((unsigned long long)tile * RS_TILE >= n) return;
     const uint32_t tile_base = tile * RS_TILE;
     const uint32_t tile_count = min((uint32_t)RS_TILE, n - tile_base);
     const uint32_t segbase = tile_base + wave * (64 * RS_ITEMS);
@@ -246,11 +252,13 @@
 
 template <int BITS>
 void launch_pass(const uint32_t* ki, const uint32_t* vi, uint32_t* ko, uint32_t* vo, uint32_t n, int shift,
-                 const uint32_t* ghist, uint32_t* ticket, uint32_t* status, int tiles, hipStream_t s, uint32_t* range_raw, int hist_copies) {
+                 const uint32_t* ghist, uint32_t* ticket, uint32_t* status, int tiles, hipStream_t s, uint32_t* range_raw, int hist_copies,
+                 const uint32_t* spec_counters) {
     static const bool env_tickets = getenv("GS2M_SORT_TICKETS") && atoi(getenv("GS2M_SORT_TICKETS")) != 0;
     const bool force_tickets = env_tickets || g_sort_tickets.load(std::memory_order_relaxed) != 0;
     rs_onesweep_kernel<BITS><<<tiles, RS_THREADS, 0, s>>>(ki, vi, ko, vo, n, shift, ghist,
-                                                          (!force_tickets && tiles <= resident_tiles()) ? nullptr : ticket, status, range_raw, hist_copies);
+                                                          (!force_tickets && tiles <= resident_tiles()) ? nullptr : ticket, status, range_raw, hist_copies,
+                                                          spec_counters);
 }
 
 }
@@ -277,7 +285,7 @@
 
 hipError_t gs2m_radix_sort_pairs(void* temp, size_t temp_bytes, const uint32_t* kin, const uint32_t* vin, uint32_t* kA,
                                  uint32_t* vA, uint32_t* kB, uint32_t* vB, size_t n, int total_bits, bool prezeroed, hipStream_t s,
-                                 uint32_t* range_raw, const uint32_t* ext_hist) {
+                                 uint32_t* range_raw, const uint32_t* ext_hist, const uint32_t* spec_counters) {
     if (n == 0) return hipSuccess;
     const SortPlan p = make_plan(total_bits);
     const int tiles = (int)((n + RS_TILE - 1) / RS_TILE);
@@ -290,6 +298,7 @@
     hipError_t e = prezeroed ? hipSuccess : gs2m_zero_async(base, zero_bytes, s);
     if (e != hipSuccess) return e;
     const int workers = tiles < RS_HIST_WGS ? tiles : RS_HIST_WGS;
+    if (spec_counters != nullptr && ext_hist == nullptr) return hipErrorInvalidValue;
     if (ext_hist == nullptr)
         rs_hist_kernel<<<workers, RS_THREADS, 0, s>>>(kin, (uint32_t)n, p.npass, make_int4(p.bits[0], p.bits[1], p.bits[2], p.bits[3]),
                                                       make_int4(p.shift[0], p.shift[1], p.shift[2], p.shift[3]), ghist, tiles, workers);
@@ -302,10 +311,10 @@
         const int hc = ext_hist ? GS2M_HIST_COPIES : 1;
         uint32_t* const rr = i == p.npass - 1 ? range_raw : nullptr;
         switch (p.bits[i]) {
-#define RS_CASE(B) case B: launch_pass<B>(ki, vi, ko, vo, (uint32_t)n, p.shift[i], gh, tickets + i, st, tiles, s, rr, hc); break;
+#define RS_CASE(B) case B: launch_pass<B>(ki, vi, ko, vo, (uint32_t)n, p.shift[i], gh, tickets + i, st, tiles, s, rr, hc, spec_counters); break;
             RS_CASE(1) RS_CASE(2) RS_CASE(3) RS_CASE(4) RS_CASE(5) RS_CASE(6) RS_CASE(7) RS_CASE(8)
 #undef RS_CASE
-            default: launch_pass<1>(ki, vi, ko, vo, (uint32_t)n, 31, gh, tickets + i, st, tiles, s, rr, hc); break;
+            default: launch_pass<1>(ki, vi, ko, vo, (uint32_t)n, 31, gh, tickets + i, st, tiles, s, rr, hc, spec_counters); break;
         }
         ki = ko;
         vi = vo;
diff --git a/gs-2m_amd/csrc/tile_sort.hip b/gs-2m_amd/csrc/tile_sort.hip
--- a/gs-2m_amd/csrc/tile_sort.hip
+++ b/gs-2m_amd/csrc/tile_sort.hip
@@ -288,10 +288,12 @@
 __global__ void __launch_bounds__(64) __attribute__((amdgpu_waves_per_eu(4, 8)))
 tile_sort_wave16_kernel(const uint32_t* __restrict__ ranges_raw, const uint32_t* __restrict__ slot_sorted, const uint4* __restrict__ e_rec,
                         const uint32_t* __restrict__ wave_rowbase, uint32_t* __restrict__ point_list, uint2* __restrict__ qlist,
-                        uint32_t* __restrict__ qrow, uint32_t* __restrict__ qcount, int tiles_x, int tiles_y, const uint32_t* __restrict__ counters) {
+                        uint32_t* __restrict__ qrow, uint32_t* __restrict__ qcount, int tiles_x, int tiles_y, const uint32_t* __restrict__ counters,
+                        uint32_t own_above ) {
     constexpr int M16 = 64 * 16, W16 = M16 + M16 / 32;
     __shared__ uint32_t s_v[W16], s_r[W16];
     if (counters[GS2M_CNT_SPAN_MID] == 0u) return;
+    if (own_above != 0u && counters[1] <= own_above) return;
     const int lane = threadIdx.x;
     const int tile = tile_of_block(blockIdx.x, tiles_x, tiles_y);
     if (tile < 0) return;
@@ -594,10 +596,11 @@
 tile_sort_wg_kernel(const uint32_t* __restrict__ ranges_raw, uint2* __restrict__ ranges, const uint32_t* __restrict__ slot_sorted,
                     const uint4* __restrict__ e_rec, const uint32_t* __restrict__ wave_rowbase, uint32_t* __restrict__ point_list,
                     uint32_t* __restrict__ row_tmp, uint2* __restrict__ qlist, uint32_t* __restrict__ qrow, uint32_t* __restrict__ qcount,
-                    int tiles_x, int tiles_y, uint32_t nblocks, uint32_t* __restrict__ counters, int take_mid) {
+                    int tiles_x, int tiles_y, uint32_t nblocks, uint32_t* __restrict__ counters, int take_mid, uint32_t own_above) {
     constexpr int WORDS = WgCfg<MAXE>::kWords;
     __shared__ uint32_t s_all[WgCfg<MAXE>::kLds];
     if constexpr (MAXE >= 8) {
+        if (take_mid == 2) take_mid = counters[1] <= own_above ? 1 : 0;
         if (counters[GS2M_CNT_SPAN_LONG] == 0u && !(take_mid && counters[GS2M_CNT_SPAN_MID] != 0u)) return;
     }
     uint32_t* const s_v = s_all, * const s_r = s_all + WORDS, * const s_x = s_all + 2 * WORDS;
@@ -634,23 +637,24 @@
 void gs2m_set_tile_sort_policy_impl(int policy) { g_ts_policy = policy; }
 
 void gs2m_launch_tile_sort(size_t tiles, int tiles_x, int tiles_y, size_t R , const BinningState& b, const ImageState& im,
-                           const GeomState& g, hipStream_t s) {
+                           const GeomState& g, hipStream_t s, bool R_on_device) {
     if (tiles == 0) return;
     const unsigned grid = tile_grid(tiles_x, tiles_y);
     static const int env_policy = getenv("GS2M_TS_POLICY") ? atoi(getenv("GS2M_TS_POLICY")) : 0;
     const int set_policy = g_ts_policy.load(std::memory_order_relaxed), policy = set_policy != 0 ? set_policy : env_policy;
     const bool waves = policy == 2 || policy == 3 || (policy == 0 && tiles >= 2560);
     const bool mid_own_kernel = policy != 3 && (R == SIZE_MAX || R > (size_t)400 * tiles);
+    const uint32_t own_above = R_on_device && mid_own_kernel && (size_t)400 * tiles < 0xFFFFFFFFull ? (uint32_t)((size_t)400 * tiles) : 0u;
     const unsigned wg_grid = grid < 2048u ? grid : 2048u;
     if (waves) {
         tile_sort_wave_kernel<<<grid, 64, 0, s>>>(im.ranges_raw, im.ranges, b.slot_sorted, b.e_rec, g.wave_rowbase, b.point_list, b.qlist, b.qrow, im.qcount,
                                                   tiles_x, tiles_y, 512u, g.counters);
         if (mid_own_kernel)
-            tile_sort_wave16_kernel<<<grid, 64, 0, s>>>(im.ranges_raw, b.slot_sorted, b.e_rec, g.wave_rowbase, b.point_list, b.qlist, b.qrow, im.qcount, tiles_x, tiles_y, g.counters);
+            tile_sort_wave16_kernel<<<grid, 64, 0, s>>>(im.ranges_raw, b.slot_sorted, b.e_rec, g.wave_rowbase, b.point_list, b.qlist, b.qrow, im.qcount, tiles_x, tiles_y, g.counters, own_above);
     } else {
         tile_sort_wg_kernel<4><<<wg_grid, 256, 0, s>>>(im.ranges_raw, im.ranges, b.slot_sorted, b.e_rec, g.wave_rowbase, b.point_list, b.sort_valA, b.qlist, b.qrow,
-                                                       im.qcount, tiles_x, tiles_y, grid, g.counters, 0);
+                                                       im.qcount, tiles_x, tiles_y, grid, g.counters, 0, 0u);
     }
     tile_sort_wg_kernel<16><<<wg_grid < 768u ? wg_grid : 768u , 256, 0, s>>>(im.ranges_raw, nullptr, b.slot_sorted, b.e_rec, g.wave_rowbase, b.point_list, b.sort_valA,
-                                                                             b.qlist, b.qrow, im.qcount, tiles_x, tiles_y, grid, g.counters, waves && !mid_own_kernel ? 1 : 0);
-}
+                                                                             b.qlist, b.qrow, im.qcount, tiles_x, tiles_y, grid, g.counters, waves && !mid_own_kernel ? 1 : (waves && own_above != 0u ? 2 : 0), own_above);
+}
diff --git a/gs-2m_amd/diff_gaussian_rasterization/__init__.py b/gs-2m_amd/diff_gaussian_rasterization/__init__.py
--- a/gs-2m_amd/diff_gaussian_rasterization/__init__.py
+++ b/gs-2m_amd/diff_gaussian_rasterization/__init__.py
@@ -127,6 +127,7 @@
         self.owner = None
         self.recent_max = 0
         self.window = 0
+        self.units = 0
 
     @classmethod
     def acquire(cls, device, stream):
@@ -186,8 +187,10 @@
         geom, binning, img = _Alloc.three(device)
         cache, lease = _BinningCache.acquire(device, _native.stream_ptr(device)) if _cached_binning else (None, None)
         pre = None
-        if lease is not None and cache.tensor is not None:
-            pre = _native.Prealloc(cache.tensor.data_ptr(), cache.tensor.numel(), binning.cb, None, 0, 0)
+        if lease is not None:
+            t = cache.tensor
+            pre = _native.Prealloc(t.data_ptr() if t is not None else None, t.numel() if t is not None else 0, binning.cb, None, 0, 0,
+                                   cache.units, 0)
             if _CModule._prealloc_cb is None:
                 _CModule._prealloc_cb = C.cast(_native.lib().gs2m_prealloc_alloc, _native.ALLOC_FN)
             bin_cb, bin_user = _CModule._prealloc_cb, C.byref(pre)
@@ -219,6 +222,8 @@
             if lease is not None:
                 cache.tensor = torch.empty(int(bin_tensor.numel() * 1.25) + 4096, dtype=torch.uint8, device=device)
                 cache.recent_max, cache.window = 0, 0
+                units = int(pre.units)
+                cache.units = max(cache.units, units + units // 4 + (8 if units else 0))
                 lease.ended = True
         return rendered, out_color, radii, observe, out_buffer, geom.take(), bin_tensor, img.take()
 
@@ -334,6 +339,7 @@
         num_rendered, color, radii, observe, buffer, geomBuffer, binningBuffer, imgBuffer = _C.rasterize_gaussians(
             *args, sh_rest=shs_rest, _cached_binning=True, _lease_out=lease)
         ctx.forward_token = _native.lib().gs2m_raster_forward_token()
+        ctx.carved = _native.lib().gs2m_raster_forward_carved()
         ctx.binning_lease = lease[0] if lease else None
         if lease:
             lease[0].attach(ctx)
@@ -365,6 +371,7 @@
         dense_rows = L.gs2m_raster_dense_rows(ctx.forward_token)
         if dense_rows >= 0:
             L.gs2m_raster_backward_rows_hint(dense_rows)
+        L.gs2m_raster_backward_carve_hint(ctx.carved)
         res = _C.rasterize_gaussians_backward(*args, sh_rest=shs_rest, unused_input_grads=False, want_sh_grad=not color_dead)
         (grad_means2D, grad_colors_precomp, grad_opacities, grad_means3D, grad_cov3Ds_precomp, grad_sh, grad_scales,
          grad_rotations, grad_features) = res[:9]
diff --git a/gs-2m_amd/gs2m_native.py b/gs-2m_amd/gs2m_native.py
--- a/gs-2m_amd/gs2m_native.py
+++ b/gs-2m_amd/gs2m_native.py
@@ -11,7 +11,7 @@
 
 class Prealloc(C.Structure):
     _fields_ = [("ptr", C.c_void_p), ("capacity", C.c_size_t), ("fallback", ALLOC_FN), ("fallback_user", C.c_void_p),
-                ("used_fallback", C.c_int), ("requested", C.c_size_t)]
+                ("used_fallback", C.c_int), ("requested", C.c_size_t), ("units_capacity", C.c_size_t), ("units", C.c_size_t)]
 
 
 class Layout(C.Structure):
@@ -52,6 +52,9 @@
     "gs2m_set_sort_tickets": (i, [i]),
     "gs2m_set_tile_sort_policy": (i, [i]),
     "gs2m_prealloc_alloc": (p, [C.c_size_t, p]),
+    "gs2m_set_speculative_forward": (i, [i]),
+    "gs2m_raster_forward_carved": (ll, []),
+    "gs2m_raster_backward_carve_hint": (i, [ll]),
     "gs2m_set_debug": (i, [i]),
     "gs2m_set_markers": (i, [i]),
     "gs2m_stage_name": (C.c_char_p, [i]),
@@ -255,7 +258,7 @@
 def reset_modes():
     L = lib()
     L.gs2m_set_reference_binning(0); L.gs2m_set_spin_wait(1); L.gs2m_set_debug(0); L.gs2m_set_sort_tickets(0); L.gs2m_set_tile_sort_policy(0)
-    L.gs2m_set_markers(0); L.gs2m_profile_mode(0)
+    L.gs2m_set_markers(0); L.gs2m_profile_mode(0); L.gs2m_set_speculative_forward(1)
 
 
 def debug_layout(P, R, W, H):
@@ -270,6 +273,10 @@
 
 def set_tile_sort_policy(policy):
     check(lib().gs2m_set_tile_sort_policy(int(policy)), "gs2m_set_tile_sort_policy")
+
+
+def set_speculative_forward(on):
+    check(lib().gs2m_set_speculative_forward(int(bool(on))), "gs2m_set_speculative_forward")
 
 
 def set_spin_wait(on):
diff --git a/include/gs2m_raster.h b/include/gs2m_raster.h
--- a/include/gs2m_raster.h
+++ b/include/gs2m_raster.h
@@ -185,8 +185,14 @@
     void* fallback_user;
     int used_fallback;
     size_t requested;
+    size_t units_capacity;
+    size_t units;
 } gs2m_prealloc;
 char* gs2m_prealloc_alloc(size_t bytes, void* user);
+
+int gs2m_set_speculative_forward(int on);
+long long gs2m_raster_forward_carved(void);
+int gs2m_raster_backward_carve_hint(long long carved_instances);
 
 int gs2m_set_debug(int on);
 int gs2m_set_markers(int on);
```

Measured after the change: 862.2 views/s, median of 6. 1.01x the previous value.
